# astra-vision/PaSCo

Hardware: AMD Instinct MI355X
Metric: scenes/sec (256x256x32, ~10% occ) PaSCo MIMO-3 (higher is better)
Workload: dtype f32 (conv products as 3 x f16 split MFMA, fp32 accumulate)

## Files before the change

pasco_amd/build.py:

```python
from __future__ import annotations

import os
import subprocess
import sys
from concurrent.futures import ThreadPoolExecutor

CSRC = os.path.join(os.path.dirname(os.path.abspath(__file__)), "csrc")
LIB_PATH = os.path.join(CSRC, "libpascohip.so")
SOURCES = ["coords.hip", "conv.hip", "conv_f16x3.hip", "conv_dma.hip", "conv_lin.hip", "conv_wide.hip", "conv_grid.hip", "conv_win.hip", "conv_wop.hip", "rows.hip", "attn.hip", "input.hip", "panop.hip", "eval.hip", "frame.hip", "label.hip"]
HEADERS = ["ph_common.h", "conv_h2_common.h", os.path.join("..", "..", "include", "pasco_hip.h"),
           os.path.join("..", "..", "include", "pasco_eval.h"),
           os.path.join("..", "..", "include", "pasco_frame.h"),
           os.path.join("..", "..", "include", "pasco_label.h")]
HIPCC = os.environ.get("HIPCC", "/opt/rocm/bin/hipcc")
FLAGS = ["--offload-arch=gfx950", "-O3", "-std=c++17", "-fPIC", "-Wall", "-Wno-unused-function"]


def _stale(target: str, deps: list[str]) -> bool:
    if not os.path.exists(target):
        return True
    t = os.path.getmtime(target)
    return any(os.path.getmtime(d) > t for d in deps if os.path.exists(d))


DEV_LIB_PATH = os.path.join(CSRC, "libpascohip_dev.so")


def build_hip(force: bool = False, verbose: bool = True, dev: bool = False) -> str:
    srcs = [s for s in SOURCES if os.path.exists(os.path.join(CSRC, s))]
    hdrs = [os.path.join(CSRC, h) for h in HEADERS]
    objs = []
    jobs = []
    lib_path = DEV_LIB_PATH if dev else LIB_PATH
    for s in srcs:
        src = os.path.join(CSRC, s)
        obj = os.path.join(CSRC, s.replace(".hip", ".dev.o" if dev else ".o"))
        objs.append(obj)
        if force or _stale(obj, [src] + hdrs):
            jobs.append([HIPCC, *FLAGS, *(["-DPH_DEV"] if dev else []), "-c", src, "-o", obj])

    def run(cmd):
        if verbose:
            print("[build]", " ".join(cmd), flush=True)
        r = subprocess.run(cmd, capture_output=True, text=True)
        if r.returncode != 0:
            sys.stderr.write(r.stdout + r.stderr)
            raise RuntimeError("hipcc failed: " + " ".join(cmd))
        if verbose and r.stderr.strip():
            sys.stderr.write(r.stderr)

    if jobs:
        with ThreadPoolExecutor(max_workers=min(4, len(jobs))) as ex:
            list(ex.map(run, jobs))
    if force or jobs or _stale(lib_path, objs):
        run([HIPCC, "--offload-arch=gfx950", "-shared", "-fPIC", "-o", lib_path, *objs])
    return lib_path


if __name__ == "__main__":
    print(build_hip(force="--force" in sys.argv, dev="--dev" in sys.argv))
```

pasco_amd/csrc/coords.hip:

```cpp
#include <stdarg.h>

#include "ph_common.h"

static thread_local char g_err[512] = "";

void ph_set_error(const char *fmt, ...) {
  va_list ap;
  va_start(ap, fmt);
  vsnprintf(g_err, sizeof(g_err), fmt, ap);
  va_end(ap);
}

extern "C" int ph_abi_version(void) { return PH_ABI_VERSION; }
extern "C" int ph_conv_desc_size(void) { return (int)sizeof(ph_conv_desc); }
extern "C" const char *ph_last_error(void) { return g_err; }

constexpr int CP_THREADS = 256;
constexpr int CP_ROUNDS = 8;
constexpr int CP_TILE = CP_THREADS * CP_ROUNDS;

extern "C" int64_t ph_workspace_bytes(int64_t n) {
  if (n < 0) n = 0;
  int64_t nb = n / CP_TILE + 2;
  return 9 * n + (int64_t)PH_MAX_KVOL * nb * 4 + 4096;
}

template <class Pred>
__global__ void __launch_bounds__(CP_THREADS)
    k_compact_count(Pred pred, int64_t n, int32_t *__restrict__ block_counts) {
  const int seg = blockIdx.y;
  const int nb = gridDim.x;
  const int64_t base = (int64_t)blockIdx.x * CP_TILE;
  int cnt = 0;
#pragma unroll
  for (int r = 0; r < CP_ROUNDS; ++r) {
    int64_t i = base + r * CP_THREADS + threadIdx.x;
    bool p = (i < n) && pred(seg, i);
    cnt += __popcll(__ballot(p));
  }
  __shared__ int wcnt[CP_THREADS / PH_WAVE];
  const int wave = threadIdx.x >> 6, lane = threadIdx.x & 63;
  if (lane == 0) wcnt[wave] = cnt;
  __syncthreads();
  if (threadIdx.x == 0) block_counts[(int64_t)seg * nb + blockIdx.x] = wcnt[0] + wcnt[1] + wcnt[2] + wcnt[3];
}

__global__ void __launch_bounds__(256)
    k_compact_scan(int32_t *__restrict__ block_counts, int nb, int32_t *__restrict__ totals) {
  const int seg = blockIdx.x;
  int32_t *c = block_counts + (int64_t)seg * nb;
  __shared__ int wsum[4];
  const int lane = threadIdx.x & 63, wave = threadIdx.x >> 6;
  int carry = 0;
  for (int base = 0; base < nb; base += 256) {
    int i = base + threadIdx.x;
    int v = (i < nb) ? c[i] : 0;
    int x = v;
#pragma unroll
    for (int d = 1; d < 64; d <<= 1) {
      int y = __shfl_up(x, d);
      if (lane >= d) x += y;
    }
    if (lane == 63) wsum[wave] = x;
    __syncthreads();
    int woff = 0;
    for (int w = 0; w < wave; ++w) woff += wsum[w];
    int tot = wsum[0] + wsum[1] + wsum[2] + wsum[3];
    if (i < nb) c[i] = carry + woff + x - v;
    carry += tot;
    __syncthreads();
  }
  if (threadIdx.x == 0) totals[seg] = carry;
}

template <class Pred, class Emit>
__global__ void __launch_bounds__(CP_THREADS)
    k_compact_scatter(Pred pred, Emit emit, int64_t n, const int32_t *__restrict__ block_offsets) {
  const int seg = blockIdx.y;
  const int nb = gridDim.x;
  const int64_t base = (int64_t)blockIdx.x * CP_TILE;
  __shared__ int wcnt[CP_THREADS / PH_WAVE];
  const int wave = threadIdx.x >> 6, lane = threadIdx.x & 63;
  int running = block_offsets[(int64_t)seg * nb + blockIdx.x];
#pragma unroll 1
  for (int r = 0; r < CP_ROUNDS; ++r) {
    int64_t i = base + r * CP_THREADS + threadIdx.x;
    bool p = (i < n) && pred(seg, i);
    unsigned long long b = __ballot(p);
    int wtot = __popcll(b);
    int wpre = __popcll(b & ((1ull << lane) - 1ull));
    if (lane == 0) wcnt[wave] = wtot;
    __syncthreads();
    int woff = 0;
    for (int w = 0; w < wave; ++w) woff += wcnt[w];
    int tot = wcnt[0] + wcnt[1] + wcnt[2] + wcnt[3];
    if (i < n) emit(seg, i, p ? running + woff + wpre : -1);
    running += tot;
    __syncthreads();
  }
}

template <class Pred, class Emit>
static int compact_run(Pred pred, Emit emit, int64_t n, int segs, int32_t *totals, void *ws,
                       int64_t ws_bytes, hipStream_t st) {
  int64_t nb = (n + CP_TILE - 1) / CP_TILE;
  if (nb < 1) nb = 1;
  PH_REQUIRE(ws_bytes >= (int64_t)segs * nb * 4, "compaction workspace too small (%lld < %lld)",
             (long long)ws_bytes, (long long)(segs * nb * 4));
  int32_t *block_counts = (int32_t *)ws;
  dim3 grid((unsigned)nb, (unsigned)segs);
  hipLaunchKernelGGL(k_compact_count<Pred>, grid, dim3(CP_THREADS), 0, st, pred, n, block_counts);
  PH_LAUNCH_CHECK();
  hipLaunchKernelGGL(k_compact_scan, dim3(segs), dim3(256), 0, st, block_counts, (int)nb, totals);
  PH_LAUNCH_CHECK();
  hipLaunchKernelGGL((k_compact_scatter<Pred, Emit>), grid, dim3(CP_THREADS), 0, st, pred, emit, n,
                     block_counts);
  PH_LAUNCH_CHECK();
  return 0;
}

struct PredFlag {
  const uint8_t *flags;
  __device__ bool operator()(int, int64_t i) const { return flags[i] != 0; }
};
struct EmitRows {
  int32_t *keep_rows;
  int32_t *rank_of;
  __device__ void operator()(int, int64_t i, int rank) const {
    if (rank >= 0) keep_rows[rank] = (int32_t)i;
    if (rank_of) rank_of[i] = rank;
  }
};

int ph_compact_flags(const uint8_t *flags, int64_t n, int32_t *keep_rows, int32_t *rank_of,
                     int32_t *n_keep, void *ws, int64_t ws_bytes, hipStream_t st) {
  return compact_run(PredFlag{flags}, EmitRows{keep_rows, rank_of}, n, 1, n_keep, ws, ws_bytes, st);
}

extern "C" int ph_mask_compact(const uint8_t *mask, int64_t n, int32_t *keep_rows, int32_t *n_keep,
                               void *ws, int64_t ws_bytes, ph_stream_t stream) {
  PH_REQUIRE(n >= 0 && n < 0x7FFFFFFF, "mask_compact: bad n");
  if (n == 0) {
    PH_CHECK_HIP(hipMemsetAsync(n_keep, 0, 4, ph_stream(stream)));
    return 0;
  }
  return ph_compact_flags(mask, n, keep_rows, nullptr, n_keep, ws, ws_bytes, ph_stream(stream));
}

__global__ void __launch_bounds__(256)
    k_insert(const int4 *__restrict__ coords, int64_t n, unsigned long long *__restrict__ tkeys,
             int32_t *__restrict__ tvals, uint64_t mask, int32_t *__restrict__ row_slot, int32_t *__restrict__ status) {
  int64_t i = (int64_t)blockIdx.x * blockDim.x + threadIdx.x;
  if (i >= n) return;
  int4 c = coords[i];
  if (!ph_packable(c.x, c.y, c.z, c.w)) {
    if (status != nullptr) atomicOr(status, 2);
    if (row_slot) row_slot[i] = -1;
    return;
  }
  uint64_t key = ph_pack(c.x, c.y, c.z, c.w);
  uint64_t slot = ph_hash(key) & mask;
  for (;;) {
    unsigned long long prev = atomicCAS(&tkeys[slot], (unsigned long long)PH_EMPTY_KEY,
                                        (unsigned long long)key);
    if (prev == PH_EMPTY_KEY || prev == key) break;
    slot = (slot + 1) & mask;
  }
  atomicMin((unsigned int *)&tvals[slot], (unsigned int)i);
  if (row_slot) row_slot[i] = (int32_t)slot;
}

struct PredFirst {
  const int32_t *tvals;
  const int32_t *row_slot;
  __device__ bool operator()(int, int64_t i) const {
    const int32_t s = row_slot[i];
    return s >= 0 && tvals[s] == (int32_t)i;
  }
};

__global__ void __launch_bounds__(256)
    k_assign_rank(int64_t n, const int32_t *__restrict__ rank_of,
                  const int32_t *__restrict__ row_slot, int32_t *__restrict__ tvals) {
  int64_t i = (int64_t)blockIdx.x * blockDim.x + threadIdx.x;
  if (i >= n) return;
  int r = rank_of[i];
  if (r >= 0) tvals[row_slot[i]] = r;
}

__global__ void __launch_bounds__(256)
    k_row2uniq(int64_t n, const int32_t *__restrict__ row_slot, const int32_t *__restrict__ tvals,
               int32_t *__restrict__ row2uniq) {
  int64_t i = (int64_t)blockIdx.x * blockDim.x + threadIdx.x;
  if (i >= n) return;
  const int32_t s = row_slot[i];
  row2uniq[i] = s >= 0 ? tvals[s] : -1;
}

static inline unsigned nblk(int64_t n, int t) { return (unsigned)((n + t - 1) / t); }

extern "C" int ph_map_insert(const int32_t *coords, int64_t n, uint64_t *tkeys, int32_t *tvals,
                             int64_t cap, int32_t *row2uniq, int32_t *uniq_rows, int32_t *n_uniq,
                             void *ws, int64_t ws_bytes, int32_t *status, ph_stream_t stream) {
  hipStream_t st = ph_stream(stream);
  PH_REQUIRE(n >= 0 && n < 0x3FFFFFFF, "map_insert: bad n=%lld", (long long)n);
  PH_REQUIRE(ph_is_pow2(cap) && cap >= 2 * n && cap >= 2, "map_insert: cap=%lld must be pow2 >= 2n",
             (long long)cap);
  if ((const char *)tvals == (const char *)tkeys + (size_t)cap * 8) {
    PH_CHECK_HIP(hipMemsetAsync(tkeys, 0xFF, (size_t)cap * 12, st));
  } else {
    PH_CHECK_HIP(hipMemsetAsync(tkeys, 0xFF, (size_t)cap * 8, st));
    PH_CHECK_HIP(hipMemsetAsync(tvals, 0xFF, (size_t)cap * 4, st));
  }
  if (n == 0) {
    if (n_uniq) PH_CHECK_HIP(hipMemsetAsync(n_uniq, 0, 4, st));
    return 0;
  }
  const uint64_t mask = (uint64_t)cap - 1;
  if (uniq_rows == nullptr) {
    hipLaunchKernelGGL(k_insert, dim3(nblk(n, 256)), dim3(256), 0, st, (const int4 *)coords, n,
                       (unsigned long long *)tkeys, tvals, mask, (int32_t *)nullptr, status);
    PH_LAUNCH_CHECK();
    return 0;
  }
  PH_REQUIRE(row2uniq && n_uniq, "map_insert: row2uniq / n_uniq required with uniq_rows");
  PH_REQUIRE(ws_bytes >= ph_workspace_bytes(n), "map_insert: workspace too small");
  int32_t *row_slot = (int32_t *)ws;
  int32_t *rank_of = row_slot + n;
  char *rest = (char *)(rank_of + n);
  int64_t rest_bytes = ws_bytes - 8 * n;
  hipLaunchKernelGGL(k_insert, dim3(nblk(n, 256)), dim3(256), 0, st, (const int4 *)coords, n,
                     (unsigned long long *)tkeys, tvals, mask, row_slot, status);
  PH_LAUNCH_CHECK();
  int rc = compact_run(PredFirst{tvals, row_slot}, EmitRows{uniq_rows, rank_of}, n, 1, n_uniq, rest,
                       rest_bytes, st);
  if (rc) return rc;
  hipLaunchKernelGGL(k_assign_rank, dim3(nblk(n, 256)), dim3(256), 0, st, n, rank_of, row_slot, tvals);
  PH_LAUNCH_CHECK();
  hipLaunchKernelGGL(k_row2uniq, dim3(nblk(n, 256)), dim3(256), 0, st, n, row_slot, tvals, row2uniq);
  PH_LAUNCH_CHECK();
  return 0;
}

__global__ void __launch_bounds__(256)
    k_find(const int4 *__restrict__ q, int64_t n, const uint64_t *__restrict__ tkeys,
           const int32_t *__restrict__ tvals, uint64_t mask, int32_t *__restrict__ out) {
  int64_t i = (int64_t)blockIdx.x * blockDim.x + threadIdx.x;
  if (i >= n) return;
  int4 c = q[i];
  out[i] = ph_packable(c.x, c.y, c.z, c.w) ? ph_find(tkeys, tvals, mask, ph_pack(c.x, c.y, c.z, c.w)) : -1;
}

extern "C" int ph_map_find(const int32_t *query, int64_t n, const uint64_t *tkeys,
                           const int32_t *tvals, int64_t cap, int32_t *out_rows,
                           ph_stream_t stream) {
  PH_REQUIRE(ph_is_pow2(cap), "map_find: cap must be pow2");
  if (n == 0) return 0;
  hipLaunchKernelGGL(k_find, dim3(nblk(n, 256)), dim3(256), 0, ph_stream(stream),
                     (const int4 *)query, n, tkeys, tvals, (uint64_t)cap - 1, out_rows);
  PH_LAUNCH_CHECK();
  return 0;
}

__device__ __forceinline__ int floor_to(int v, int ts) {
  int q = v / ts;
  if ((v % ts) != 0 && ((v < 0) != (ts < 0))) --q;
  return q * ts;
}

__global__ void __launch_bounds__(256)
    k_coords_floor(const int4 *__restrict__ in, int64_t n, int ts, int4 *__restrict__ out) {
  int64_t i = (int64_t)blockIdx.x * blockDim.x + threadIdx.x;
  if (i >= n) return;
  int4 c = in[i];
  out[i] = make_int4(c.x, floor_to(c.y, ts), floor_to(c.z, ts), floor_to(c.w, ts));
}

extern "C" int ph_coords_floor(const int32_t *coords, int64_t n, int32_t ts, int32_t *out,
                               ph_stream_t stream) {
  PH_REQUIRE(ts > 0, "coords_floor: ts must be > 0");
  if (n == 0) return 0;
  hipLaunchKernelGGL(k_coords_floor, dim3(nblk(n, 256)), dim3(256), 0, ph_stream(stream),
                     (const int4 *)coords, n, ts, (int4 *)out);
  PH_LAUNCH_CHECK();
  return 0;
}

__global__ void __launch_bounds__(256)
    k_coords_expand(const int4 *__restrict__ in, int64_t n, int ts, int4 *__restrict__ out) {
  int64_t t = (int64_t)blockIdx.x * blockDim.x + threadIdx.x;
  if (t >= n * 8) return;
  int64_t i = t >> 3;
  int k = (int)(t & 7);
  int4 c = in[i];
  out[t] = make_int4(c.x, c.y + (k & 1) * ts, c.z + ((k >> 1) & 1) * ts, c.w + ((k >> 2) & 1) * ts);
}

extern "C" int ph_coords_expand(const int32_t *coords, int64_t n, int32_t ts_out, int32_t *out,
                                ph_stream_t stream) {
  PH_REQUIRE(ts_out > 0, "coords_expand: ts_out must be > 0");
  if (n == 0) return 0;
  hipLaunchKernelGGL(k_coords_expand, dim3(nblk(n * 8, 256)), dim3(256), 0, ph_stream(stream),
                     (const int4 *)coords, n, ts_out, (int4 *)out);
  PH_LAUNCH_CHECK();
  return 0;
}

struct NbrOffsets {
  int32_t d[PH_MAX_KVOL][3];
};

__global__ void __launch_bounds__(256)
    k_nbr_build(const int4 *__restrict__ out_coords, int64_t n_out,
                const uint64_t *__restrict__ tkeys, const int32_t *__restrict__ tvals,
                uint64_t mask, NbrOffsets off, int32_t *__restrict__ nbr) {
  const int k = blockIdx.y;
  int64_t o = (int64_t)blockIdx.x * blockDim.x + threadIdx.x;
  if (o >= n_out) return;
  int4 c = out_coords[o];
  const int x = c.y + off.d[k][0], y = c.z + off.d[k][1], z = c.w + off.d[k][2];
  nbr[(int64_t)k * n_out + o] = ph_packable(c.x, x, y, z) ? ph_find(tkeys, tvals, mask, ph_pack(c.x, x, y, z)) : -1;
}

extern "C" int ph_nbr_build(const int32_t *out_coords, int64_t n_out, const uint64_t *in_tkeys,
                            const int32_t *in_tvals, int64_t in_cap, const int32_t *h_offsets,
                            int32_t kvol, int32_t *nbr, ph_stream_t stream) {
  PH_REQUIRE(kvol >= 1 && kvol <= PH_MAX_KVOL, "nbr_build: kvol=%d out of range", kvol);
  PH_REQUIRE(ph_is_pow2(in_cap), "nbr_build: cap must be pow2");
  if (n_out == 0) return 0;
  NbrOffsets off;
  memset(&off, 0, sizeof(off));
  memcpy(off.d, h_offsets, sizeof(int32_t) * 3 * kvol);
  dim3 grid(nblk(n_out, 256), (unsigned)kvol);
  hipLaunchKernelGGL(k_nbr_build, grid, dim3(256), 0, ph_stream(stream), (const int4 *)out_coords,
                     n_out, in_tkeys, in_tvals, (uint64_t)in_cap - 1, off, nbr);
  PH_LAUNCH_CHECK();
  return 0;
}

__global__ void __launch_bounds__(256)
    k_nbr_build_same(const int4 *__restrict__ coords, int64_t n, const uint64_t *__restrict__ tkeys,
                     const int32_t *__restrict__ tvals, uint64_t mask, NbrOffsets off, int kvol, int32_t *__restrict__ nbr) {
  const int k = blockIdx.y;
  int64_t o = (int64_t)blockIdx.x * blockDim.x + threadIdx.x;
  if (o >= n) return;
  if (k == kvol / 2) {
    nbr[(int64_t)k * n + o] = (int32_t)o;
    return;
  }
  int4 c = coords[o];
  const int x = c.y + off.d[k][0], y = c.z + off.d[k][1], z = c.w + off.d[k][2];
  const int j = ph_packable(c.x, x, y, z) ? ph_find(tkeys, tvals, mask, ph_pack(c.x, x, y, z)) : -1;
  nbr[(int64_t)k * n + o] = j;
  if (j >= 0) nbr[(int64_t)(kvol - 1 - k) * n + j] = (int32_t)o;
}

extern "C" int ph_nbr_build_same(const int32_t *coords, int64_t n, const uint64_t *tkeys, const int32_t *tvals, int64_t cap,
                                 const int32_t *h_offsets, int32_t kvol, int32_t *nbr, ph_stream_t stream) {
  PH_REQUIRE(kvol >= 1 && kvol <= PH_MAX_KVOL && (kvol & 1), "nbr_build_same: odd kernel volume <= %d expected, got %d", PH_MAX_KVOL, kvol);
  PH_REQUIRE(ph_is_pow2(cap), "nbr_build_same: cap must be pow2");
  for (int k = 0; k < kvol; ++k)
    for (int a = 0; a < 3; ++a)
      PH_REQUIRE(h_offsets[3 * k + a] == -h_offsets[3 * (kvol - 1 - k) + a], "nbr_build_same: offsets are not symmetric");
  if (n == 0) return 0;
  hipStream_t st = ph_stream(stream);
  NbrOffsets off;
  memset(&off, 0, sizeof(off));
  memcpy(off.d, h_offsets, sizeof(int32_t) * 3 * kvol);
  const int half = kvol / 2;
  if (half > 0)
    PH_CHECK_HIP(hipMemsetAsync(nbr + (int64_t)(half + 1) * n, 0xFF, (size_t)half * (size_t)n * 4, st));
  dim3 grid(nblk(n, 256), (unsigned)(half + 1));
  hipLaunchKernelGGL(k_nbr_build_same, grid, dim3(256), 0, st, (const int4 *)coords, n, tkeys, tvals, (uint64_t)cap - 1, off,
                     kvol, nbr);
  PH_LAUNCH_CHECK();
  return 0;
}

struct PredNbr {
  const int32_t *nbr;
  int64_t n_out;
  __device__ bool operator()(int seg, int64_t i) const { return nbr[(int64_t)seg * n_out + i] >= 0; }
};
struct EmitPairs {
  const int32_t *nbr;
  int64_t n_out;
  int32_t *pairs_in;
  int32_t *pairs_out;
  __device__ void operator()(int seg, int64_t i, int rank) const {
    if (rank < 0) return;
    int64_t base = (int64_t)seg * n_out;
    pairs_in[base + rank] = nbr[base + i];
    pairs_out[base + rank] = (int32_t)i;
  }
};

extern "C" int ph_kmap_compact(const int32_t *nbr, int32_t kvol, int64_t n_out, int32_t *pairs_in,
                               int32_t *pairs_out, int32_t *counts, void *ws, int64_t ws_bytes,
                               ph_stream_t stream) {
  PH_REQUIRE(kvol >= 1 && kvol <= PH_MAX_KVOL, "kmap_compact: kvol=%d out of range", kvol);
  if (n_out == 0) {
    PH_CHECK_HIP(hipMemsetAsync(counts, 0, 4 * kvol, ph_stream(stream)));
    return 0;
  }
  return compact_run(PredNbr{nbr, n_out}, EmitPairs{nbr, n_out, pairs_in, pairs_out}, n_out, kvol,
                     counts, ws, ws_bytes, ph_stream(stream));
}


__global__ void __launch_bounds__(256)
    k_rowlist_pack(const int32_t *__restrict__ pairs_in, const int32_t *__restrict__ pairs_out, const int32_t *__restrict__ counts,
                   int kvol, int64_t n_out, int32_t *__restrict__ rl_in, int32_t *__restrict__ rl_out,
                   int32_t *__restrict__ tile_k, int64_t cap, int64_t tcap, int32_t *__restrict__ status) {
  __shared__ int64_t off[PH_MAX_KVOL + 1];
  if (threadIdx.x == 0) {
    int64_t o = 0, pairs = 0;
    for (int k = 0; k < kvol; ++k) {
      off[k] = o;
      o += ((int64_t)counts[k] + 127) / 128 * 128;
      pairs += counts[k];
    }
    off[kvol] = o;
    if (status != nullptr && blockIdx.x == 0 && pairs != n_out) atomicOr(status, 32);
  }
  __syncthreads();
  const int64_t stride = (int64_t)gridDim.x * blockDim.x;
  for (int64_t i = (int64_t)blockIdx.x * blockDim.x + threadIdx.x; i < cap; i += stride) {
    int k = 0;
    while (k < kvol && i >= off[k + 1]) ++k;
    int vi = -1, vo = -1;
    if (k < kvol) {
      const int64_t j = i - off[k];
      if (j < counts[k]) {
        vi = pairs_in[(int64_t)k * n_out + j];
        vo = pairs_out[(int64_t)k * n_out + j];
      }
    }
    rl_in[i] = vi;
    rl_out[i] = vo;
    if ((i & 127) == 0 && (i >> 7) < tcap) tile_k[i >> 7] = k < kvol ? k : -1;
  }
  for (int64_t t = cap / 128 + (int64_t)blockIdx.x * blockDim.x + threadIdx.x; t < tcap; t += stride) tile_k[t] = -1;
}

extern "C" int ph_rowlist_pack(const int32_t *pairs_in, const int32_t *pairs_out, const int32_t *counts, int32_t kvol,
                               int64_t n_out, int32_t *rl_in, int32_t *rl_out, int32_t *tile_k, int64_t cap, int64_t tcap,
                               int32_t *status, ph_stream_t stream) {
  PH_REQUIRE(kvol >= 1 && kvol <= PH_MAX_KVOL, "rowlist_pack: kvol=%d out of range", kvol);
  PH_REQUIRE(cap % 128 == 0 && cap >= n_out + (int64_t)kvol * 127 - (kvol * 127) % 128 && tcap * 128 >= cap,
             "rowlist_pack: list capacity %lld too small for %lld rows and %d offsets", (long long)cap, (long long)n_out, kvol);
  if (cap == 0) return 0;
  int64_t blocks = (cap + 255) / 256;
  if (blocks > 4096) blocks = 4096;
  hipLaunchKernelGGL(k_rowlist_pack, dim3((unsigned)blocks), dim3(256), 0, ph_stream(stream), pairs_in, pairs_out, counts, kvol,
                     n_out, rl_in, rl_out, tile_k, cap, tcap, status);
  PH_LAUNCH_CHECK();
  return 0;
}
```

pasco_amd/csrc/rows.hip:

```cpp
#include "ph_common.h"

static inline unsigned nblk(int64_t n, int t) { return (unsigned)((n + t - 1) / t); }

template <typename T>
__global__ void __launch_bounds__(256)
    k_gather_rows(const T *__restrict__ src, int c, const int32_t *__restrict__ rows, int64_t n_out,
                  T *__restrict__ dst) {
  int64_t t = (int64_t)blockIdx.x * blockDim.x + threadIdx.x;
  if (t >= n_out * c) return;
  int64_t j = t / c;
  int ch = (int)(t - j * c);
  int r = rows[j];
  T v;
  memset(&v, 0, sizeof(T));
  if (r >= 0) v = src[(int64_t)r * c + ch];
  dst[t] = v;
}

extern "C" int ph_gather_rows(const void *src, int32_t c, const int32_t *rows, int64_t n_out,
                              void *dst, ph_stream_t stream) {
  PH_REQUIRE(c > 0, "gather_rows: c must be > 0");
  if (n_out == 0) return 0;
  hipStream_t st = ph_stream(stream);
  if (c % 4 == 0 && (((uintptr_t)src | (uintptr_t)dst) & 15) == 0) {
    int c4 = c / 4;
    hipLaunchKernelGGL(k_gather_rows<float4>, dim3(nblk(n_out * c4, 256)), dim3(256), 0, st,
                       (const float4 *)src, c4, rows, n_out, (float4 *)dst);
  } else {
    hipLaunchKernelGGL(k_gather_rows<float>, dim3(nblk(n_out * c, 256)), dim3(256), 0, st,
                       (const float *)src, c, rows, n_out, (float *)dst);
  }
  PH_LAUNCH_CHECK();
  return 0;
}

__global__ void __launch_bounds__(256)
    k_scatter_add_rows(const float *__restrict__ src, int c, const int32_t *__restrict__ rows,
                       int64_t n_src, float *__restrict__ dst) {
  int64_t t = (int64_t)blockIdx.x * blockDim.x + threadIdx.x;
  if (t >= n_src * c) return;
  int64_t i = t / c;
  int ch = (int)(t - i * c);
  int r = rows[i];
  if (r >= 0) dst[(int64_t)r * c + ch] += src[t];
}

extern "C" int ph_scatter_add_rows(const float *src, int32_t c, const int32_t *rows, int64_t n_src,
                                   float *dst, ph_stream_t stream) {
  PH_REQUIRE(c > 0, "scatter_add_rows: c must be > 0");
  if (n_src == 0) return 0;
  hipLaunchKernelGGL(k_scatter_add_rows, dim3(nblk(n_src * c, 256)), dim3(256), 0,
                     ph_stream(stream), src, c, rows, n_src, dst);
  PH_LAUNCH_CHECK();
  return 0;
}

struct KeepSrcs {
  const void *p[8];
};
__global__ void __launch_bounds__(256)
    k_keep_mask(KeepSrcs srcs, int n_src, int kind, const int4 *__restrict__ coords, int64_t n, const int32_t *__restrict__ lo,
                const int32_t *__restrict__ hi, uint8_t *__restrict__ out, int32_t *__restrict__ any) {
  const int64_t r = (int64_t)blockIdx.x * blockDim.x + threadIdx.x;
  bool k = n_src == 0;
  if (r < n) {
    for (int i = 0; i < n_src; ++i)
      k = k || (kind == 1 ? reinterpret_cast<const int32_t *>(srcs.p[i])[r] >= 0 : reinterpret_cast<const uint8_t *>(srcs.p[i])[r] != 0);
  }
  if (any != nullptr && __ballot(k) != 0ull && (threadIdx.x & 63) == 0) {
    if (__hip_atomic_load(any, __ATOMIC_RELAXED, __HIP_MEMORY_SCOPE_AGENT) == 0) atomicOr(any, 1);
  }
  if (r >= n) return;
  bool inside = true;
  if (lo != nullptr) {
    const int4 c = coords[r];
    inside = c.y >= lo[0] && c.z >= lo[1] && c.w >= lo[2] && c.y <= hi[0] && c.z <= hi[1] && c.w <= hi[2];
  }
  out[r] = (k && inside) ? 1 : 0;
}
__global__ void __launch_bounds__(256)
    k_keep_fallback(const int4 *__restrict__ coords, int64_t n, int64_t fallback, const int32_t *__restrict__ lo,
                    const int32_t *__restrict__ hi, uint8_t *__restrict__ out, const int32_t *__restrict__ any) {
  if (*any != 0) return;
  const int64_t r = (int64_t)blockIdx.x * blockDim.x + threadIdx.x;
  if (r >= n || r >= fallback) return;
  bool inside = true;
  if (lo != nullptr) {
    const int4 c = coords[r];
    inside = c.y >= lo[0] && c.z >= lo[1] && c.w >= lo[2] && c.y <= hi[0] && c.z <= hi[1] && c.w <= hi[2];
  }
  out[r] = inside ? 1 : 0;
}

extern "C" int ph_keep_mask(const void *const *srcs, int32_t n_src, int32_t kind, const int32_t *coords, int64_t n,
                            const int32_t *lo, const int32_t *hi, int64_t fallback_rows, uint8_t *out, int32_t *any_word,
                            ph_stream_t stream) {
  PH_REQUIRE(n_src >= 0 && n_src <= 8 && (kind == 0 || kind == 1) && n >= 0 && fallback_rows >= 0, "keep_mask: bad arguments");
  PH_REQUIRE((lo == nullptr) == (hi == nullptr) && (lo == nullptr || coords != nullptr), "keep_mask: bounds need lo, hi and coords");
  PH_REQUIRE(fallback_rows == 0 || any_word != nullptr, "keep_mask: the fallback needs the scratch word");
  if (n == 0) return 0;
  KeepSrcs ks;
  for (int i = 0; i < 8; ++i) ks.p[i] = i < n_src ? srcs[i] : nullptr;
  hipStream_t st = ph_stream(stream);
  int32_t *any = fallback_rows > 0 ? any_word : nullptr;
  if (any) PH_CHECK_HIP(hipMemsetAsync(any, 0, sizeof(int32_t), st));
  hipLaunchKernelGGL(k_keep_mask, dim3(nblk(n, 256)), dim3(256), 0, st, ks, n_src, kind, (const int4 *)coords, n, lo, hi, out, any);
  PH_LAUNCH_CHECK();
  if (any) {
    const int64_t m = n < fallback_rows ? n : fallback_rows;
    hipLaunchKernelGGL(k_keep_fallback, dim3(nblk(m, 256)), dim3(256), 0, st, (const int4 *)coords, n, fallback_rows, lo, hi, out,
                       any);
    PH_LAUNCH_CHECK();
  }
  return 0;
}

__global__ void __launch_bounds__(256)
    k_maxpool(const float *__restrict__ in, int c, const int32_t *__restrict__ nbr, int kvol,
              int64_t n_out, float *__restrict__ out) {
  int64_t t = (int64_t)blockIdx.x * blockDim.x + threadIdx.x;
  if (t >= n_out * c) return;
  int64_t o = t / c;
  int ch = (int)(t - o * c);
  float m = 0.f;
  bool any = false;
  for (int k = 0; k < kvol; ++k) {
    int r = nbr[(int64_t)k * n_out + o];
    if (r >= 0) {
      float v = in[(int64_t)r * c + ch];
      m = any ? fmaxf(m, v) : v;
      any = true;
    }
  }
  out[t] = m;
}

extern "C" int ph_maxpool_fwd(const float *in, int32_t c, const int32_t *nbr, int32_t kvol,
                              int64_t n_out, float *out, ph_stream_t stream) {
  PH_REQUIRE(c > 0 && kvol >= 1 && kvol <= PH_MAX_KVOL, "maxpool_fwd: bad shape");
  if (n_out == 0) return 0;
  hipLaunchKernelGGL(k_maxpool, dim3(nblk(n_out * c, 256)), dim3(256), 0, ph_stream(stream), in, c,
                     nbr, kvol, n_out, out);
  PH_LAUNCH_CHECK();
  return 0;
}

struct Dims4 {
  int b, x, y, z;
};

__device__ __forceinline__ int floor_div(int v, int ts) {
  int q = v / ts;
  if ((v % ts) != 0 && ((v < 0) != (ts < 0))) --q;
  return q;
}

__global__ void __launch_bounds__(256)
    k_to_dense(const float *__restrict__ feats, const int4 *__restrict__ coords, int64_t n, int c,
               int mx, int my, int mz, int ts, Dims4 d, float *__restrict__ dense) {
  int64_t t = (int64_t)blockIdx.x * blockDim.x + threadIdx.x;
  if (t >= n * c) return;
  int64_t i = t / c;
  int ch = (int)(t - i * c);
  int4 p = coords[i];
  int x = floor_div(p.y - mx, ts), y = floor_div(p.z - my, ts), z = floor_div(p.w - mz, ts);
  if (x < 0) x += d.x;
  if (y < 0) y += d.y;
  if (z < 0) z += d.z;
  if (p.x < 0 || p.x >= d.b || x < 0 || x >= d.x || y < 0 || y >= d.y || z < 0 || z >= d.z) return;
  int64_t site = ((int64_t)x * d.y + y) * d.z + z;
  dense[((int64_t)p.x * c + ch) * ((int64_t)d.x * d.y * d.z) + site] = feats[t];
}

extern "C" int ph_to_dense(const float *feats, const int32_t *coords, int64_t n, int32_t c,
                           const int32_t *h_min3, int32_t ts, const int32_t *h_dims4, float *dense,
                           ph_stream_t stream) {
  PH_REQUIRE(c > 0 && ts > 0, "to_dense: bad c/ts");
  if (n == 0) return 0;
  Dims4 d{h_dims4[0], h_dims4[1], h_dims4[2], h_dims4[3]};
  hipLaunchKernelGGL(k_to_dense, dim3(nblk(n * c, 256)), dim3(256), 0, ph_stream(stream), feats,
                     (const int4 *)coords, n, c, h_min3[0], h_min3[1], h_min3[2], ts, d, dense);
  PH_LAUNCH_CHECK();
  return 0;
}

__global__ void __launch_bounds__(256)
    k_site_flags(const float *__restrict__ dense, int c, int64_t nsite_per_b, int64_t nsites,
                 uint8_t *__restrict__ flags) {
  int64_t s = (int64_t)blockIdx.x * blockDim.x + threadIdx.x;
  if (s >= nsites) return;
  int64_t b = s / nsite_per_b;
  int64_t site = s - b * nsite_per_b;
  const float *p = dense + b * c * nsite_per_b + site;
  bool any = false;
  for (int ch = 0; ch < c; ++ch) any |= (p[(int64_t)ch * nsite_per_b] != 0.f);
  flags[s] = any ? 1 : 0;
}

__global__ void __launch_bounds__(256)
    k_sites_to_coords(const int32_t *__restrict__ keep_rows, const int32_t *__restrict__ n_rows,
                      Dims4 d, int4 *__restrict__ out_coords) {
  int64_t j = (int64_t)blockIdx.x * blockDim.x + threadIdx.x;
  if (j >= *n_rows) return;
  int64_t s = keep_rows[j];
  int z = (int)(s % d.z);
  s /= d.z;
  int y = (int)(s % d.y);
  s /= d.y;
  int x = (int)(s % d.x);
  s /= d.x;
  out_coords[j] = make_int4((int)s, x, y, z);
}

extern "C" int ph_to_sparse_coords(const float *dense, int32_t c, const int32_t *h_dims4,
                                   int32_t *out_coords, int32_t *n_rows, void *ws,
                                   int64_t ws_bytes, ph_stream_t stream) {
  Dims4 d{h_dims4[0], h_dims4[1], h_dims4[2], h_dims4[3]};
  int64_t per_b = (int64_t)d.x * d.y * d.z;
  int64_t nsites = per_b * d.b;
  PH_REQUIRE(c > 0 && nsites < 0x7FFFFF00, "to_sparse_coords: bad shape");
  hipStream_t st = ph_stream(stream);
  if (nsites == 0) {
    PH_CHECK_HIP(hipMemsetAsync(n_rows, 0, 4, st));
    return 0;
  }
  PH_REQUIRE(ws_bytes >= ph_workspace_bytes(nsites), "to_sparse_coords: workspace too small");
  uint8_t *flags = (uint8_t *)ws;
  int64_t fpad = (nsites + 15) & ~(int64_t)15;
  int32_t *keep_rows = (int32_t *)(flags + fpad);
  char *rest = (char *)(keep_rows + nsites);
  int64_t rest_bytes = ws_bytes - fpad - 4 * nsites;
  hipLaunchKernelGGL(k_site_flags, dim3(nblk(nsites, 256)), dim3(256), 0, st, dense, c, per_b, nsites,
                     flags);
  PH_LAUNCH_CHECK();
  int rc = ph_compact_flags(flags, nsites, keep_rows, nullptr, n_rows, rest, rest_bytes, st);
  if (rc) return rc;
  hipLaunchKernelGGL(k_sites_to_coords, dim3(nblk(nsites, 256)), dim3(256), 0, st, keep_rows, n_rows, d,
                     (int4 *)out_coords);
  PH_LAUNCH_CHECK();
  return 0;
}

__global__ void __launch_bounds__(256)
    k_dense_gather(const float *__restrict__ dense, int c, Dims4 d, const int4 *__restrict__ sc,
                   int64_t n, float *__restrict__ feats) {
  int64_t t = (int64_t)blockIdx.x * blockDim.x + threadIdx.x;
  if (t >= n * c) return;
  int64_t i = t / c;
  int ch = (int)(t - i * c);
  int4 p = sc[i];
  float v = 0.f;
  if (p.x >= 0 && p.x < d.b && p.y >= 0 && p.y < d.x && p.z >= 0 && p.z < d.y && p.w >= 0 && p.w < d.z) {
    int64_t per_b = (int64_t)d.x * d.y * d.z;
    int64_t site = ((int64_t)p.y * d.y + p.z) * d.z + p.w;
    v = dense[((int64_t)p.x * c + ch) * per_b + site];
  }
  feats[t] = v;
}

extern "C" int ph_dense_gather(const float *dense, int32_t c, const int32_t *h_dims4,
                               const int32_t *site_coords, int64_t n, float *feats,
                               ph_stream_t stream) {
  PH_REQUIRE(c > 0, "dense_gather: bad c");
  if (n == 0) return 0;
  Dims4 d{h_dims4[0], h_dims4[1], h_dims4[2], h_dims4[3]};
  hipLaunchKernelGGL(k_dense_gather, dim3(nblk(n * c, 256)), dim3(256), 0, ph_stream(stream), dense, c,
                     d, (const int4 *)site_coords, n, feats);
  PH_LAUNCH_CHECK();
  return 0;
}

__global__ void __launch_bounds__(256) k_sine_pe(const int32_t *__restrict__ coords, int64_t n, int cstride, int coff, int f,
                                                  const float *__restrict__ dim_t, float scale,
                                                  const float *__restrict__ table, int tab_lo, int tab_n,
                                                  float *__restrict__ out) {
  const int64_t t = (int64_t)blockIdx.x * blockDim.x + threadIdx.x;
  const int w = 3 * f;
  if (t >= n * w) return;
  const int64_t row = t / w;
  const int col = (int)(t - row * w);
  const int axis = col / f;
  const int j = col - axis * f;
  const int half = f >> 1;
  const int ci = coords[row * cstride + coff + axis];
  const unsigned ti = (unsigned)(ci - tab_lo);
  float v;
  if (table != nullptr && ti < (unsigned)tab_n) {
    v = table[(int64_t)ti * f + j];
  } else {
    float c = (float)ci;
    c = c / (c + 1e-6f) * scale;
    if (j < half) v = sinf(c / dim_t[2 * j]);
    else v = cosf(c / dim_t[2 * (j - half) + 1]);
  }
  out[t] = v;
}

extern "C" int ph_sine_pe(const int32_t *coords, int64_t n, int32_t cstride, int32_t coff, int32_t f,
                          const float *dim_t, float scale, const float *table, int32_t tab_lo, int32_t tab_n,
                          float *out, ph_stream_t stream) {
  PH_REQUIRE(n >= 0 && f > 0 && f % 2 == 0 && cstride >= 3 && coff >= 0 && coff + 3 <= cstride, "sine_pe: bad shape");
  PH_REQUIRE(table == nullptr || tab_n > 0, "sine_pe: empty table");
  if (n == 0) return 0;
  PH_REQUIRE(coords && dim_t && out, "sine_pe: null buffer");
  hipLaunchKernelGGL(k_sine_pe, dim3(nblk(n * 3 * f, 256)), dim3(256), 0, ph_stream(stream), coords, n, cstride, coff, f,
                     dim_t, scale, table, tab_lo, tab_n, out);
  PH_LAUNCH_CHECK();
  return 0;
}


template <int C, bool VEC>
__global__ void __launch_bounds__(256) k_sem_ensemble(ph_sem_ens_desc d) {
  const int64_t s = (int64_t)blockIdx.x * blockDim.x + threadIdx.x;
  if (s >= d.n_sites) return;
  float mean[C];
#pragma unroll
  for (int ch = 0; ch < C; ++ch) mean[ch] = 0.f;
  for (int i = 0; i < d.m; ++i) {
    float p[C];
    const int r = d.rows[i][s];
    if (r >= 0) {
      const float *x = d.logits[i] + (int64_t)r * C;
      if (VEC) {
#pragma unroll
        for (int q = 0; q < C / 4; ++q) {
          const float4 v = reinterpret_cast<const float4 *>(x)[q];
          p[4 * q] = v.x; p[4 * q + 1] = v.y; p[4 * q + 2] = v.z; p[4 * q + 3] = v.w;
        }
      } else {
#pragma unroll
        for (int ch = 0; ch < C; ++ch) p[ch] = x[ch];
      }
      float mx = p[0];
#pragma unroll
      for (int ch = 1; ch < C; ++ch) mx = fmaxf(mx, p[ch]);
      float sum = 0.f;
#pragma unroll
      for (int ch = 0; ch < C; ++ch) {
        p[ch] = expf(p[ch] - mx);
        sum += p[ch];
      }
#pragma unroll
      for (int ch = 0; ch < C; ++ch) p[ch] = p[ch] / sum;
    } else {
#pragma unroll
      for (int ch = 0; ch < C; ++ch) p[ch] = ch == 0 ? 1.f : 0.f;
    }
    float best = p[0];
#pragma unroll
    for (int ch = 0; ch < C; ++ch) {
      mean[ch] += p[ch];
      best = fmaxf(best, p[ch]);
    }
    float *o = d.out[i] + s * C;
    if (VEC) {
#pragma unroll
      for (int q = 0; q < C / 4; ++q) reinterpret_cast<float4 *>(o)[q] = make_float4(p[4 * q], p[4 * q + 1], p[4 * q + 2], p[4 * q + 3]);
    } else {
#pragma unroll
      for (int ch = 0; ch < C; ++ch) o[ch] = p[ch];
    }
    if (d.conf[i]) d.conf[i][s] = best;
  }
  const float inv_m = (float)d.m;
  float best = 0.f;
#pragma unroll
  for (int ch = 0; ch < C; ++ch) {
    mean[ch] = mean[ch] / inv_m;
    best = ch == 0 ? mean[ch] : fmaxf(best, mean[ch]);
  }
  float *o = d.out[d.m] + s * C;
  if (VEC) {
#pragma unroll
    for (int q = 0; q < C / 4; ++q) reinterpret_cast<float4 *>(o)[q] = make_float4(mean[4 * q], mean[4 * q + 1], mean[4 * q + 2], mean[4 * q + 3]);
  } else {
#pragma unroll
    for (int ch = 0; ch < C; ++ch) o[ch] = mean[ch];
  }
  if (d.conf[d.m]) d.conf[d.m][s] = best;
}

extern "C" int ph_sem_ensemble(const ph_sem_ens_desc *desc, ph_stream_t stream) {
  PH_REQUIRE(desc != nullptr && desc->m >= 1 && desc->m <= 8, "sem_ensemble: 1 <= m <= 8");
  PH_REQUIRE(desc->c == 20 || desc->c == 19, "sem_ensemble: serves 20 (SemanticKITTI) or 19 (SSCBench-KITTI360) classes, got %d", desc->c);
  if (desc->n_sites == 0) return 0;
  for (int i = 0; i < desc->m; ++i) PH_REQUIRE(desc->logits[i] && desc->rows[i] && desc->out[i], "sem_ensemble: null buffer");
  PH_REQUIRE(desc->out[desc->m] != nullptr, "sem_ensemble: null mean buffer");
  hipStream_t st = ph_stream(stream);
  const dim3 grid((unsigned)((desc->n_sites + 255) / 256));
  bool al = true;
  for (int i = 0; i <= desc->m; ++i) al = al && (((uintptr_t)desc->out[i]) & 15) == 0;
  for (int i = 0; i < desc->m; ++i) al = al && (((uintptr_t)desc->logits[i]) & 15) == 0;
  if (desc->c == 20 && al)
    hipLaunchKernelGGL((k_sem_ensemble<20, true>), grid, dim3(256), 0, st, *desc);
  else if (desc->c == 20)
    hipLaunchKernelGGL((k_sem_ensemble<20, false>), grid, dim3(256), 0, st, *desc);
  else
    hipLaunchKernelGGL((k_sem_ensemble<19, false>), grid, dim3(256), 0, st, *desc);
  PH_LAUNCH_CHECK();
  return 0;
}


__global__ void __launch_bounds__(256)
    k_ens_resample(const float *__restrict__ logits, int q, const int32_t *__restrict__ rows, const int32_t *__restrict__ sel,
                   int64_t u, float *__restrict__ out, uint8_t *__restrict__ flag) {
  const int lane = threadIdx.x & 63;
  const int64_t nwaves = (int64_t)gridDim.x * 4;
  for (int64_t s = (int64_t)blockIdx.x * 4 + (threadIdx.x >> 6); s < u; s += nwaves) {
    const int r = rows[sel[s]];
    float v0 = 0.f, v1 = 0.f;
    if (r >= 0) {
      const float *x = logits + (int64_t)r * q;
      if (lane < q) v0 = 1.f / (1.f + expf(-x[lane]));
      if (lane + 64 < q) v1 = 1.f / (1.f + expf(-x[lane + 64]));
    }
    float *o = out + s * q;
    if (lane < q) o[lane] = v0;
    if (lane + 64 < q) o[lane + 64] = v1;
    const unsigned long long any = __ballot(v0 != 0.f || v1 != 0.f);
    if (lane == 0) flag[s] = any != 0ull ? 1 : 0;
  }
}

__global__ void __launch_bounds__(256)
    k_ens_merge(float *__restrict__ anchor, const float *__restrict__ m, const int32_t *__restrict__ perm, int64_t u, int q,
                float fi) {
#pragma clang fp contract(off)
  const int lane = threadIdx.x & 63;
  const int p0 = lane < q ? perm[lane] : 0, p1 = lane + 64 < q ? perm[lane + 64] : 0;
  const int64_t nwaves = (int64_t)gridDim.x * 4;
  const float den = fi + 1.f;
  for (int64_t s = (int64_t)blockIdx.x * 4 + (threadIdx.x >> 6); s < u; s += nwaves) {
    float *a = anchor + s * q;
    const float *b = m + s * q;
    if (lane < q) {
      const float t = a[lane] * fi;
      a[lane] = (t + b[p0]) / den;
    }
    if (lane + 64 < q) {
      const float t = a[lane + 64] * fi;
      a[lane + 64] = (t + b[p1]) / den;
    }
  }
}

__global__ void __launch_bounds__(256)
    k_ens_finish(const float *__restrict__ anchor, int q, const int32_t *__restrict__ keep, int qk, const float *__restrict__ sem,
                 int c, const int32_t *__restrict__ sel, int64_t u, float *__restrict__ out, uint8_t *__restrict__ flag) {
  const int lane = threadIdx.x & 63;
  const int k0 = lane < qk ? keep[lane] : 0, k1 = lane + 64 < qk ? keep[lane + 64] : 0;
  const int64_t nwaves = (int64_t)gridDim.x * 4;
  for (int64_t s = (int64_t)blockIdx.x * 4 + (threadIdx.x >> 6); s < u; s += nwaves) {
    const float *sr = sem + (int64_t)sel[s] * c;
    const float p0 = sr[0];
    const bool larger = lane >= 1 && lane < c && sr[lane] > p0;
    const float nz = __ballot(larger) != 0ull ? 1.f : 0.f;
    const float *a = anchor + s * q;
    float v0 = 0.f, v1 = 0.f;
    if (lane < qk) v0 = a[k0] * nz;
    if (lane + 64 < qk) v1 = a[k1] * nz;
    float *o = out + s * qk;
    if (lane < qk) o[lane] = v0;
    if (lane + 64 < qk) o[lane + 64] = v1;
    const unsigned long long any = __ballot(v0 != 0.f || v1 != 0.f);
    if (lane == 0) flag[s] = any != 0ull ? 1 : 0;
  }
}

static unsigned ens_grid(int64_t u) {
  int64_t g = (u + 3) / 4;
  if (g > 16384) g = 16384;
  return (unsigned)(g < 1 ? 1 : g);
}

extern "C" int ph_ens_resample(const float *logits, int64_t n, int32_t q, const int32_t *rows, const int32_t *sel, int64_t u,
                               float *out, uint8_t *flag, ph_stream_t stream) {
  PH_REQUIRE(q >= 1 && q <= 128 && n >= 0 && u >= 0, "ens_resample: bad shape");
  if (u == 0) return 0;
  PH_REQUIRE(logits && rows && sel && out && flag, "ens_resample: null buffer");
  hipLaunchKernelGGL(k_ens_resample, dim3(ens_grid(u)), dim3(256), 0, ph_stream(stream), logits, q, rows, sel, u, out, flag);
  PH_LAUNCH_CHECK();
  return 0;
}

extern "C" int ph_ens_merge(float *anchor, const float *m, const int32_t *perm, int64_t u, int32_t q, int32_t i,
                            ph_stream_t stream) {
  PH_REQUIRE(q >= 1 && q <= 128 && u >= 0 && i >= 1, "ens_merge: bad shape");
  if (u == 0) return 0;
  PH_REQUIRE(anchor && m && perm, "ens_merge: null buffer");
  hipLaunchKernelGGL(k_ens_merge, dim3(ens_grid(u)), dim3(256), 0, ph_stream(stream), anchor, m, perm, u, q, (float)i);
  PH_LAUNCH_CHECK();
  return 0;
}

extern "C" int ph_ens_finish(const float *anchor, int64_t u, int32_t q, const int32_t *keep, int32_t qk, const float *sem,
                             int32_t c, const int32_t *sel, float *out, uint8_t *flag, ph_stream_t stream) {
  PH_REQUIRE(q >= 1 && q <= 128 && qk >= 0 && qk <= q && c >= 1 && c <= 64 && u >= 0, "ens_finish: bad shape");
  if (u == 0) return 0;
  PH_REQUIRE(anchor && sem && sel && flag && (qk == 0 || (keep && out)), "ens_finish: null buffer");
  hipLaunchKernelGGL(k_ens_finish, dim3(ens_grid(u)), dim3(256), 0, ph_stream(stream), anchor, q, keep, qk, sem, c, sel, u, out,
                     flag);
  PH_LAUNCH_CHECK();
  return 0;
}

__global__ void __launch_bounds__(256)
    k_project_canonical(const float *__restrict__ T, int X, int Y, int Z, double res, float mb0, float mb1, float mb2,
                        int4 *__restrict__ out) {
#pragma clang fp contract(off)
  const int64_t i = (int64_t)blockIdx.x * blockDim.x + threadIdx.x;
  const int64_t n = (int64_t)X * Y * Z;
  if (i >= n) return;
  const int z = (int)(i % Z), y = (int)((i / Z) % Y), x = (int)(i / ((int64_t)Y * Z));
  const float mb[3] = {mb0, mb1, mb2};
  const int c[3] = {x, y, z};
  float p[3];
#pragma unroll
  for (int a = 0; a < 3; ++a) {
    const double m = (double)c[a] * res;
    const double h = m + res / 2;
    p[a] = (float)(h + (double)mb[a]);
  }
  const float resf = (float)res, halff = (float)(res / 2);
  int q[3];
#pragma unroll
  for (int r = 0; r < 3; ++r) {
    const float t0 = T[r * 4 + 0] * p[0];
    const float t1 = T[r * 4 + 1] * p[1];
    float v = t0 + t1;
    const float t2 = T[r * 4 + 2] * p[2];
    v = v + t2;
    v = v + T[r * 4 + 3];
    v = v - mb[r];
    v = v - halff;
    v = v / resf;
    q[r] = (int)rintf(v);
  }
  out[i] = make_int4(0, q[0], q[1], q[2]);
}

extern "C" int ph_project_canonical(const float *T, int32_t X, int32_t Y, int32_t Z, double resolution, const float *h_min_bound,
                                    int32_t *out_coords, ph_stream_t stream) {
  PH_REQUIRE(X >= 1 && Y >= 1 && Z >= 1 && resolution > 0, "project_canonical: bad grid");
  PH_REQUIRE(T && h_min_bound && out_coords, "project_canonical: null buffer");
  const int64_t n = (int64_t)X * Y * Z;
  hipLaunchKernelGGL(k_project_canonical, dim3((unsigned)((n + 255) / 256)), dim3(256), 0, ph_stream(stream), T, X, Y, Z,
                     resolution, h_min_bound[0], h_min_bound[1], h_min_bound[2], (int4 *)out_coords);
  PH_LAUNCH_CHECK();
  return 0;
}
```

pasco_amd/graph/decoder.py:

```python
from __future__ import annotations

import os
from collections import defaultdict
from typing import Dict, List, Optional

import torch
import torch.nn as nn

from .. import me as ME
from . import fused
from .blocks import BasicGenerativeDeconvolutionBlock, ResidualBlock, SpatialDropout, run_sequential
from .fused import ACT_NONE, ACT_RELU


def _corner(v, coords: torch.Tensor) -> torch.Tensor:
    if torch.is_tensor(v):
        stream = torch.cuda.current_stream(coords.device).cuda_stream if coords.device.type == "cuda" else 0
        key = (coords.dtype, coords.device, stream, v._version)
        cache = getattr(v, "_ph_corner", None)
        if cache is not None and key in cache:
            return cache[key]
        out = v.to(device=coords.device, dtype=coords.dtype).reshape(1, 3)
        try:
            if cache is None or len(cache) > 8:
                cache = {}
                v._ph_corner = cache
            cache[key] = out
        except AttributeError:
            pass
        return out
    return torch.as_tensor(v, device=coords.device).to(coords.dtype).reshape(1, 3)


def inside_bounds(coords: torch.Tensor, lo, hi) -> torch.Tensor:
    lo, hi = _corner(lo, coords), _corner(hi, coords)
    xyz = coords[:, 1:]
    return ((xyz >= lo) & (xyz <= hi)).all(dim=1)


def box_mask(mgr, coords: torch.Tensor, lo, hi) -> torch.Tensor:
    if fused.fusion() and coords.dtype == torch.int32 and coords.dim() == 2 and coords.shape[1] == 4:
        try:
            be = mgr.backend()
        except Exception:
            be = None
        if be is not None and be.has("keep_mask") and os.environ.get("PASCO_KEEP_FUSED", "1") != "0":
            lo_t, hi_t = _corner(lo, coords).reshape(3).contiguous(), _corner(hi, coords).reshape(3).contiguous()
            return be.keep_mask([], coords.contiguous(), lo_t, hi_t)
    return inside_bounds(coords, lo, hi)


_FIRST_ROWS = {}


def _first_rows(n: int, device, k: int = 1000) -> torch.Tensor:
    stream = torch.cuda.current_stream(device).cuda_stream if torch.device(device).type == "cuda" else 0
    key = (n, str(device), k, stream)
    hit = _FIRST_ROWS.get(key)
    if hit is None:
        if len(_FIRST_ROWS) > 64:
            _FIRST_ROWS.clear()
        hit = torch.arange(n, device=device) < k
        _FIRST_ROWS[key] = hit
    return hit


def batch_sparse_tensor(tensors: List[ME.SparseTensor], n_max: Optional[int] = None):
    n_max = max([t.F.shape[0] for t in tensors] + ([n_max] if n_max is not None else []))
    f0, c0 = tensors[0].F, tensors[0].C
    bf = f0.new_empty((len(tensors), n_max, f0.shape[1]))
    bc = c0.new_empty((len(tensors), n_max, c0.shape[1]))
    for i, t in enumerate(tensors):
        n = t.F.shape[0]
        bf[i, :n] = t.F
        bc[i, :n] = t.C
        if n < n_max:
            bf[i, n:].zero_()
            bc[i, n:].zero_()
    return bf, bc


class DecoderBlock(nn.Module):
    def __init__(self, in_channels, out_channels, n_heads, compl_head_dim, heavy_decoder=True, dropout=0.0):
        super().__init__()
        self.upsample = BasicGenerativeDeconvolutionBlock(in_channels, out_channels, ks=2, stride=2)
        self.resize = nn.Sequential(
            ME.MinkowskiBatchNorm(out_channels + 3),
            ME.MinkowskiConvolution(out_channels + 3, out_channels, kernel_size=1, bias=True, dimension=3),
        )
        n_res = 7 if heavy_decoder else 3
        layers = [ResidualBlock(out_channels, out_channels) for _ in range(n_res)]
        if heavy_decoder:
            layers.append(SpatialDropout(p=dropout))
        self.process = nn.Sequential(*layers)
        self.n_heads = n_heads
        self.completion_heads = nn.ModuleDict({
            str(i): nn.Sequential(ME.MinkowskiConvolution(out_channels, compl_head_dim, kernel_size=1, bias=True,
                                                          dimension=3))
            for i in range(n_heads)})

    def forward(self, x: ME.SparseTensor, shortcut: ME.SparseTensor, global_min, global_max):
        mgr = x.coordinate_manager
        up = self.upsample.net[0]
        out_key = mgr.expand_pruned(x.coordinate_map_key, up.stride, lambda kids: box_mask(mgr, kids, global_min, global_max))
        nbr = mgr.kernel_map(x.coordinate_map_key, out_key, up.kernel_size, up.dilation, transposed=True)
        y_in = None
        if self._resize_applies(x, out_key):
            ukey, _, b2o = mgr.union(out_key, shortcut.coordinate_map_key)
            n_un, n_dec = mgr.size(ukey), mgr.size(out_key)
            buf = torch.empty((n_un, self.resize[1].out_channels), dtype=torch.float32, device=x.F.device)
            dec = self._resize_absorbed(x, out_key, nbr, out=buf[:n_dec])
            if dec is not None and dec.F.data_ptr() == buf.data_ptr():
                if n_un > n_dec:
                    buf[n_dec:].zero_()
                mgr.backend().scatter_add_rows(shortcut.F.contiguous(), b2o.contiguous(), buf)
                y_in = ME.SparseTensor(buf, coordinate_map_key=ukey, coordinate_manager=mgr)
        else:
            dec = None
        if y_in is None and dec is None:
            dec = self.upsample(x, out_key=out_key, nbr=nbr)
            ts = dec.tensor_stride[0]
            feats = torch.cat([dec.F, dec.C[:, 1:].float() / ts], dim=1)
            dec = ME.SparseTensor(feats, coordinate_map_key=out_key, coordinate_manager=mgr)
            dec = fused.conv(dec, self.resize[1], pro_bn=self.resize[0], pro_act=ACT_NONE)
        if y_in is None:
            y_in = dec + shortcut
        y = run_sequential(self.process, y_in)
        logits = [fused.conv(y, self.completion_heads[str(i)][0]) for i in range(self.n_heads)]
        return y, logits


    RESIZE_LO, RESIZE_ROWS = -1024, 5120

    def _resize_applies(self, x, out_key) -> bool:
        mgr = x.coordinate_manager
        conv = self.resize[1]
        c_in, c_out = conv.in_channels - 3, conv.out_channels
        be = mgr.backend()
        return bool(fused.fusion() and fused.conv_precision() == "f16x3" and fused._PRESPLIT and fused._kernel_device(x.F.device)
                    and mgr.size(out_key) >= fused.MIN_ROWS_LINEAR and c_in % 32 == 0 and be.split_supported(c_in, c_out)
                    and os.environ.get("PASCO_RESIZE_ABSORB", "1") != "0")

    def _resize_absorbed(self, x, out_key, nbr, out=None):
        mgr = x.coordinate_manager
        n_out = mgr.size(out_key)
        conv, bn = self.resize[1], self.resize[0]
        c_out = conv.out_channels
        c_in = conv.in_channels - 3
        be = mgr.backend()
        if not self._resize_applies(x, out_key):
            return None
        dec = self.upsample(x, out_key=out_key, nbr=nbr, emit_next=(None, ACT_NONE), split_only=True)
        if not isinstance(dec, fused.SplitRows):
            return self._resize_plain(dec, out_key)
        ts = out_key.tensor_stride[0]
        w = conv.kernel
        ver = (w._version, w.data_ptr(), conv.bias._version if conv.bias is not None else -1, ts) + tuple(
            (t._version, t.data_ptr()) for t in (bn.bn.running_mean, bn.bn.running_var, bn.bn.weight, bn.bn.bias) if t is not None)
        hit = self.__dict__.get("_ph_resize")
        if hit is None or hit[0] != ver:
            with torch.no_grad():
                s_, b_ = fused.fold_bn(bn)
                s64, b64, w64 = s_.double(), b_.double(), w.detach().reshape(c_in + 3, c_out).double()
                wf = (s64[:c_in, None] * w64[:c_in]).t().contiguous().float()
                bias = b64[:c_in] @ w64[:c_in]
                if conv.bias is not None:
                    bias = bias + conv.bias.detach().reshape(-1).double()
                idx = torch.arange(self.RESIZE_ROWS, device=w.device, dtype=torch.float64) + self.RESIZE_LO
                tab = torch.stack([((idx / ts) * s64[c_in + a] + b64[c_in + a])[:, None] * w64[c_in + a][None, :]
                                   for a in range(3)]).float().contiguous()
            hit = (ver, wf, bias.float().contiguous(), tab)
            fused.publish(tab)
            self.__dict__["_ph_resize"] = hit
        _, wf, bias, tab = hit
        coords = mgr.get_coordinates(out_key)
        out = fused.linear_rows(None, wf, bias, self, "resize", in_split=dec.split,
                                axis=(tab, coords.contiguous(), self.RESIZE_LO), out=out)
        return ME.SparseTensor(out, coordinate_map_key=out_key, coordinate_manager=mgr)

    def _resize_plain(self, dec, out_key):
        mgr = dec.coordinate_manager
        ts = dec.tensor_stride[0]
        feats = torch.cat([dec.F, dec.C[:, 1:].float() / ts], dim=1)
        dec = ME.SparseTensor(feats, coordinate_map_key=out_key, coordinate_manager=mgr)
        return fused.conv(dec, self.resize[1], pro_bn=self.resize[0], pro_act=ACT_NONE)


class DecoderGenerativeSepConvV2(nn.Module):
    def __init__(self, f, n_classes, transformer_predictor, n_infers, heavy_decoder=True, dropouts=(0.0, 0.0, 0.0)):
        super().__init__()
        dec_ch = list(f[::-1])
        self.n_infers = n_infers
        self.n_classes = n_classes
        self.transformer_predictor = transformer_predictor
        self.dec_blocks = nn.ModuleList()
        self.voxel_feats = nn.ModuleDict()
        for i in range(len(dec_ch) - 1):
            scale = 2 ** (len(dec_ch) - 2 - i)
            self.dec_blocks.append(DecoderBlock(dec_ch[i], dec_ch[i + 1], n_heads=n_infers, compl_head_dim=n_classes,
                                                heavy_decoder=heavy_decoder, dropout=dropouts[i]))
            c = dec_ch[i + 1]
            for j in range(n_infers):
                self.voxel_feats[f"scale{scale}_infer{j}"] = nn.Sequential(
                    ME.MinkowskiConvolution(c, c, kernel_size=3, bias=False, dimension=3),
                    ME.MinkowskiBatchNorm(c),
                    ME.MinkowskiReLU(),
                    ME.MinkowskiConvolution(c, c, kernel_size=3, bias=True, dimension=3),
                )
        self.pruning = ME.MinkowskiPruning()

    @staticmethod
    def _occupied(logits: ME.SparseTensor) -> torch.Tensor:
        return logits.F.argmax(dim=-1) != 0

    @staticmethod
    def _keep_sources(keep_override, scale, i, x, logits):
        if keep_override is not None:
            if hasattr(keep_override, "member_rows"):
                return keep_override.member_rows(scale, i, x.C)
            return keep_override.member(scale, i, x.C)
        return DecoderGenerativeSepConvV2._occupied(logits)

    @staticmethod
    def _fused_keep(x):
        if not fused.fusion() or x.C.dtype != torch.int32 or len(x.C.shape) != 2 or x.C.shape[1] != 4:
            return None
        try:
            be = x.coordinate_manager.backend()
        except Exception:
            return None
        return be if be.has("keep_mask") and os.environ.get("PASCO_KEEP_FUSED", "1") != "0" else None

    def _keep_completion(self, x, scale, sem_logits, keep_override):
        srcs = [self._keep_sources(keep_override, scale, i, x, sem_logits[i] if sem_logits is not None else None)
                for i in range(self.n_infers)]
        be = self._fused_keep(x)
        if be is not None and len(srcs) <= 8 and len({s.dtype for s in srcs}) == 1:
            return be.keep_mask([s.contiguous() for s in srcs])
        keeps = [s >= 0 if s.dtype == torch.int32 else s for s in srcs]
        keep = keeps[0]
        for k in keeps[1:]:
            keep = keep | k
        return keep

    def predict_panop(self, xs, sem_logits_at_scales, min_Cs, max_Cs, keep_override=None, subnets=None):
        xs_infers = defaultdict(list)
        sem_logits_pruneds = []

        def keep_mask(i, scale, x):
            logits = sem_logits_at_scales[scale][i]
            src = self._keep_sources(keep_override, scale, i, x, logits)
            be = self._fused_keep(x)
            if be is not None:
                lo, hi = _corner(min_Cs[i], x.C).reshape(3), _corner(max_Cs[i], x.C).reshape(3)
                return be.keep_mask([src.contiguous()], x.C.contiguous(), lo.contiguous(), hi.contiguous(), fallback_rows=1000)
            keep = src >= 0 if src.dtype == torch.int32 else src
            first = _first_rows(keep.shape[0], keep.device)
            keep = torch.where(keep.any(), keep, first)
            return keep & inside_bounds(x.C, min_Cs[i], max_Cs[i])

        pad_to = {s: None for s in xs}
        if subnets is not None:
            for scale, x in xs.items():
                pad_to[scale] = max(int(keep_mask(i, scale, x).sum()) for i in range(self.n_infers))
        todo = [(i, scale, x, keep_mask(i, scale, x)) for i in (range(self.n_infers) if subnets is None else subnets)
                for scale, x in xs.items()]
        mgrs = {id(x.coordinate_manager) for _, _, x, _ in todo}
        if len(mgrs) == 1 and todo:
            mgr = todo[0][2].coordinate_manager
            pruned = mgr.prune_batch([(x.coordinate_map_key, keep) for _, _, x, keep in todo])
        else:
            pruned = [x.coordinate_manager.prune(x.coordinate_map_key, keep) for _, _, x, keep in todo]
        infer_ids = list(range(self.n_infers) if subnets is None else subnets)
        n_rows = {(i, scale): x.coordinate_manager.size(out_key) for (i, scale, x, keep), (out_key, rows) in zip(todo, pruned)}
        batch_f, batch_c = {}, {}
        for scale, x in xs.items():
            n_max = max([n_rows[(i, scale)] for i in infer_ids] + ([pad_to[scale]] if pad_to[scale] is not None else []))
            batch_f[scale] = x.F.new_empty((len(infer_ids), n_max, x.F.shape[1]))
            batch_c[scale] = x.C.new_zeros((len(infer_ids), n_max, x.C.shape[1]))
        sem_F = None
        if 1 in xs:
            l0 = sem_logits_at_scales[1][infer_ids[0]].F
            sem_F = l0.new_empty((len(infer_ids), batch_f[1].shape[1], l0.shape[1]))
        for (i, scale, x, keep), (out_key, rows) in zip(todo, pruned):
            mgr = x.coordinate_manager
            be = mgr.backend()
            if scale == 1:
                logits = sem_logits_at_scales[scale][i]
                slot1, n1_ = infer_ids.index(i), n_rows[(i, scale)]
                dst = sem_F[slot1, :n1_]
                be.gather_rows(logits.F.contiguous(), rows, out=dst)
                if n1_ < sem_F.shape[1]:
                    sem_F[slot1, n1_:].zero_()
                sem_logits_pruneds.append(ME.SparseTensor(dst, coordinate_map_key=out_key, coordinate_manager=mgr))
            xi = fused.gathered_split(x, rows, out_key)
            if xi is None:
                xi = ME.SparseTensor(be.gather_rows(x.F.contiguous(), rows), coordinate_map_key=out_key, coordinate_manager=mgr)
            vf = self.voxel_feats[f"scale{scale}_infer{i}"]
            h = fused.conv(xi, vf[0], epi_bn=vf[1], epi_act=ACT_RELU, emit_next=(None, ACT_NONE), split_only=True)
            slot = infer_ids.index(i)
            n = n_rows[(i, scale)]
            y = fused.conv(h, vf[3], out=batch_f[scale][slot, :n])
            batch_c[scale][slot, :n] = y.C
            if n < batch_f[scale].shape[1]:
                batch_f[scale][slot, n:].zero_()
            xs_infers[scale].append(y)
        batched = {s: (batch_f[s], batch_c[s]) for s in xs_infers}
        batched["_meta"] = {"lens": {"fine": [int(t.F.shape[0]) for t in xs_infers[1]],
                                     "level": {s: [int(t.F.shape[0]) for t in v] for s, v in xs_infers.items()}}}
        if sem_F is None:
            sem_F, sem_C = batch_sparse_tensor(sem_logits_pruneds, pad_to[1])
        else:
            sem_C = batch_c[1]
        keep_pad = (sem_F != 0).any(-1) | (sem_C != 0).any(-1)
        panop = self.transformer_predictor(batched, (sem_F, sem_C), min_Cs, max_Cs, keep_pad, subnets=subnets,
                                           sem_tensors=sem_logits_pruneds)
        return panop, sem_logits_pruneds

    def forward(self, x, features, global_min_coords, global_max_coords, min_Cs, max_Cs,
                is_predict_panop=True, keep_override=None, subnets=None):
        assert not self.training, "inference only"
        skips = features[::-1]
        sem_logits_at_scales: Dict[int, list] = {}
        xs: Dict[int, ME.SparseTensor] = {}
        for i, block in enumerate(self.dec_blocks):
            scale = 2 ** (len(self.dec_blocks) - 1 - i)
            x, sem_logits = block(x, skips[i], global_min_coords, global_max_coords)
            keep = self._keep_completion(x, scale, sem_logits, keep_override)
            mgr = x.coordinate_manager
            out_key, rows = mgr.prune(x.coordinate_map_key, keep)
            be = mgr.backend()
            x = ME.SparseTensor(be.gather_rows(x.F, rows), coordinate_map_key=out_key, coordinate_manager=mgr)
            sem_logits = [ME.SparseTensor(be.gather_rows(l.F, rows), coordinate_map_key=out_key,
                                          coordinate_manager=mgr) for l in sem_logits]
            xs[scale] = x
            sem_logits_at_scales[scale] = sem_logits
        ret = {"sem_logits_at_scales": sem_logits_at_scales}
        if is_predict_panop:
            panop, pruned = self.predict_panop(xs, sem_logits_at_scales, min_Cs, max_Cs, keep_override, subnets)
            ret["panop_predictions"] = panop
            ret["sem_logits_pruneds"] = pruned
        return ret
```

pasco_amd/graph/fused.py:

```python
from __future__ import annotations

import contextlib
import os
import threading
from typing import Optional, Tuple

import torch
import torch.nn as nn

from ..me import SparseTensor
from ..me.backend import ACT_LEAKY, ACT_NONE, ACT_RELU
from ..me.modules import MinkowskiBatchNorm, _ConvBase

_CONV_PRECISION = "f16x3"
_PRESPLIT = True
_FUSION = True
MIN_ROWS_LINEAR = 16384
MIN_ROWS_WINDOWS = 16384
_WINDOWS_WIDE = os.environ.get("PASCO_CONV_WIN", "1") == "2"


def _kernel_device(device) -> bool:
    if device.type == "cuda":
        return True
    from ..me import backend
    cb = backend._checker_backend
    return cb is not None and cb.checker_split


def set_conv_precision(mode: str) -> None:
    global _CONV_PRECISION, _PRESPLIT
    assert mode in ("f32", "f16x3", "f16x3-inline")
    _PRESPLIT = mode != "f16x3-inline"
    _CONV_PRECISION = "f32" if mode == "f32" else "f16x3"


_TLS = threading.local()


def conv_precision() -> str:
    return getattr(_TLS, "precision", None) or _CONV_PRECISION


@contextlib.contextmanager
def precision_override(mode: str):
    assert mode in ("f32", "f16x3")
    prev = getattr(_TLS, "precision", None)
    _TLS.precision = mode
    try:
        yield
    finally:
        _TLS.precision = prev


def optimistic() -> bool:
    return bool(getattr(_TLS, "optimistic", False))


def optimistic_word(device):
    if not optimistic():
        return None
    from ..me.backend import backend_for
    try:
        return backend_for(device).optimistic_word(device)
    except RuntimeError:
        return None


@contextlib.contextmanager
def optimistic_override(on: bool):
    prev = getattr(_TLS, "optimistic", None)
    _TLS.optimistic = bool(on)
    try:
        yield
    finally:
        _TLS.optimistic = prev


def set_fusion(on: bool) -> None:
    global _FUSION
    _FUSION = bool(on)


def fusion() -> bool:
    return _FUSION


def _act_rows(F: torch.Tensor, act: int, slope: float) -> torch.Tensor:
    if act == ACT_RELU:
        return torch.relu(F)
    if act == ACT_LEAKY:
        return torch.nn.functional.leaky_relu(F, slope)
    return F


def _module_act(y: SparseTensor, act: int, slope: float) -> SparseTensor:
    if act == ACT_NONE:
        return y
    from ..me.modules import MinkowskiLeakyReLU, MinkowskiReLU
    mod = MinkowskiReLU() if act == ACT_RELU else MinkowskiLeakyReLU(slope)
    return mod(y)


def _conv_unfused(x, mod, pro_bn, pro_act, epi_bn, epi_act, epi2_bn, residual, res_act, slope, out_key, nbr):
    mgr = x.coordinate_manager
    same = lambda t, feats: SparseTensor(feats, coordinate_map_key=t.coordinate_map_key, coordinate_manager=mgr)
    bn_of = lambda bn, t: bn(t) if isinstance(bn, MinkowskiBatchNorm) else same(t, bn(t.F))
    y = x
    if pro_bn is not None:
        y = bn_of(pro_bn, y)
    y = _module_act(y, pro_act, slope)
    if out_key is None:
        y = mod(y)
    else:
        raw, pending = y.take_prologue()
        y = SparseTensor(mod.conv_rows(mgr.backend(), raw, nbr, mgr.size(out_key), mgr=mgr, prologue=pending),
                         coordinate_map_key=out_key, coordinate_manager=mgr)
    if epi_bn is not None:
        y = bn_of(epi_bn, y)
    y = _module_act(y, epi_act, slope)
    if epi2_bn is not None:
        y = bn_of(epi2_bn, y)
    if residual is not None:
        y = same(y, y.F + residual)
    return _module_act(y, res_act, slope)


def publish(t):
    dev = t.device if torch.is_tensor(t) else t
    if dev.type == "cuda" and not torch.cuda.is_current_stream_capturing():
        torch.cuda.current_stream(dev).synchronize()
    return t


def _split_of(w, be):
    return be.split_weight_rows(w) if _PRESPLIT else be.split_weight_f16(w)


def split_weight(mod, be):
    w = mod.kernel
    ver = (w._version, w.device, _PRESPLIT)
    hit = getattr(mod, "_ph_split", None)
    if hit is None or hit[0] != ver:
        hit = (ver, _split_of(w, be))
        publish(w.device)
        object.__setattr__(mod, "_ph_split", hit)
    return hit[1]


def split_input(x: SparseTensor, be, ps, pb, pro_act, slope):
    F = x.F if x.F.is_contiguous() else x.F.contiguous()
    key = _split_key(F, ps, pb, pro_act, slope)
    cache = x.__dict__.setdefault("_ph_in_split", {})
    hit = cache.get(key)
    if hit is None:
        hit = be.split_rows(F, pro_scale=ps, pro_shift=pb, pro_act=pro_act, slope=slope)
        cache[key] = hit
    return hit


def gathered_split(x: SparseTensor, rows: torch.Tensor, out_key):
    mgr = x.coordinate_manager
    be = mgr.backend()
    c = x.F.shape[1]
    if not (_FUSION and _PRESPLIT and conv_precision() == "f16x3" and be.split_supported(c, c) and x.F.shape[0] > 0):
        return None
    op = split_input(x, be, None, None, ACT_NONE, 0.01)
    n, cpad = op.shape[0], op.shape[1] * 32
    got = be.gather_rows(op.view(torch.float32).view(n, cpad), rows)
    return SplitRows(got.view(torch.float16).view(got.shape[0], cpad // 32, 2, 32), c, out_key, mgr)


def split_rows_2d(x2d: torch.Tensor):
    if not (_FUSION and _kernel_device(x2d.device) and conv_precision() == "f16x3" and _PRESPLIT and x2d.shape[1] % 8 == 0):
        return None
    from ..me.backend import backend_for
    return backend_for(x2d.device).split_rows(x2d.contiguous())


def linear_rows(x2d: Optional[torch.Tensor], weight: torch.Tensor, bias, cache_owner, cache_key: str,
                min_rows: Optional[int] = None, in_split=None, residual: Optional[torch.Tensor] = None,
                emit: bool = False, want_out: bool = True, axis=None, out: Optional[torch.Tensor] = None):
    cout, cin = weight.shape
    n = x2d.shape[0] if x2d is not None else in_split.shape[0]
    dev = x2d.device if x2d is not None else in_split.device
    be = None
    min_rows = MIN_ROWS_LINEAR if min_rows is None else min_rows
    if _FUSION and _kernel_device(dev) and n >= min_rows and conv_precision() == "f16x3":
        from ..me.backend import backend_for
        be = backend_for(dev)
        if not be.split_supported(cin, cout):
            be = None
    if be is None:
        assert x2d is not None, "linear_rows: a pre-split operand needs the split path"
        y = torch.nn.functional.linear(x2d, weight, bias)
        y = y if residual is None else y + residual
        if axis is not None:
            y = y + axis_rows(axis)
        if out is not None:
            out.copy_(y)
            y = out
        return (y, None) if emit else y
    ver = (weight._version, weight.device, weight.data_ptr(), _PRESPLIT)
    hit = cache_owner.__dict__.get("_ph_lin_" + cache_key)
    if hit is None or hit[0] != ver:
        wt = weight.detach().t().contiguous()
        hit = (ver, wt, _split_of(wt, be), bias.detach().contiguous() if bias is not None else None)
        publish(wt)
        cache_owner.__dict__["_ph_lin_" + cache_key] = hit
    _, wt, split, b = hit
    do_emit = emit and _PRESPLIT and cout % 32 == 0
    out = be.conv_fwd(None if (x2d is None) else x2d.contiguous(), wt, None, n,
                      xshape=(n, cin) if x2d is None else None, bias=b, split=split,
                      in_split=in_split if _PRESPLIT else None,
                      residual=None if residual is None else residual.contiguous(),
                      emit_split=(None, None, ACT_NONE) if do_emit else None, want_out=want_out or not do_emit,
                      axis=axis, out=out)
    if not emit:
        return out
    return out if do_emit else (out, None)


def axis_rows(axis) -> torch.Tensor:
    tab, coords, lo = axis
    idx = (coords[:, 1:4].long() - lo).clamp(0, tab.shape[1] - 1)
    return tab[0][idx[:, 0]] + tab[1][idx[:, 1]] + tab[2][idx[:, 2]]


def linear_bn_act(x2d: Optional[torch.Tensor], lin: nn.Linear, *, pro_bn=None, epi_bn=None, epi_act: int = ACT_NONE,
                  min_rows: Optional[int] = None, in_split=None, emit: bool = False, emit_into: Optional[torch.Tensor] = None,
                  out: Optional[torch.Tensor] = None):
    cin, cout = lin.in_features, lin.out_features
    n = x2d.shape[0] if x2d is not None else in_split.shape[0]
    dev = x2d.device if x2d is not None else in_split.device
    min_rows = MIN_ROWS_LINEAR if min_rows is None else min_rows
    if not (_FUSION and _kernel_device(dev) and n >= min_rows):
        assert x2d is not None
        y = x2d if pro_bn is None else pro_bn(x2d)
        y = lin(y)
        y = y if epi_bn is None else epi_bn(y)
        y = torch.relu(y) if epi_act == ACT_RELU else y
        return (y, None) if emit else y
    from ..me.backend import backend_for
    be = backend_for(dev)
    ps = pb = es = eb = None
    if pro_bn is not None:
        ps, pb = fold_bn(pro_bn)
    if epi_bn is not None:
        es, eb = fold_bn(epi_bn)
    w = lin.weight
    ver = (w._version, w.device, w.data_ptr(), _PRESPLIT, conv_precision())
    hit = lin.__dict__.get("_ph_lin_w")
    if hit is None or hit[0] != ver:
        wt = w.detach().t().contiguous()
        split = _split_of(wt, be) if (conv_precision() == "f16x3" and be.split_supported(cin, cout)) else None
        hit = (ver, wt, split, lin.bias.detach().contiguous() if lin.bias is not None else None)
        publish(wt)
        lin.__dict__["_ph_lin_w"] = hit
    _, wt, split, b = hit
    do_emit = emit and split is not None and _PRESPLIT and cout % 32 == 0
    assert x2d is not None or (split is not None and _PRESPLIT), "a pre-split operand needs the split path"
    out = be.conv_fwd(None if x2d is None else x2d.contiguous(), wt, None, n, xshape=(n, cin) if x2d is None else None,
                      bias=b, pro_scale=ps, pro_shift=pb, epi_scale=es, epi_shift=eb, epi_act=epi_act, split=split,
                      in_split=in_split if (split is not None and _PRESPLIT) else None,
                      emit_split=(None, None, ACT_NONE) if do_emit else None, want_out=not do_emit,
                      in_split_has_prologue=True, out_split=emit_into if do_emit else None, out=None if do_emit else out)
    if not emit:
        return out
    return out if do_emit else (out, None)


def prepare_batched_weights(w: torch.Tensor):
    from ..me.backend import backend_for
    be = backend_for(w.device)
    B, Q, D = w.shape
    w = w.detach()
    e = 13 - torch.frexp(w.abs().amax())[1]
    e = e.to(torch.int32).clamp(-100, 100)
    up = ((e + 127) << 23).view(torch.float32)
    down = ((127 - e) << 23).view(torch.float32)
    w_split = be.split_rows((w * up).reshape(B * Q, D).contiguous(), exp2=0)
    unscale = (torch.ones(Q, device=w.device) * down).contiguous()
    return w_split, unscale


def batched_rows_matmul(x: Optional[torch.Tensor], w: Optional[torch.Tensor], x_split: torch.Tensor, shape=None,
                        prepared=None, bias=None, axis=None) -> torch.Tensor:
    from ..me.backend import backend_for
    dev = x_split.device
    be = backend_for(dev)
    B, P, D = x.shape if x is not None else shape
    w_split, unscale = prepared if prepared is not None else prepare_batched_weights(w)
    Q = unscale.numel()
    out = torch.empty((B, P, Q), dtype=torch.float32, device=dev)
    xs = x_split.reshape(B, P, -1)
    ws = w_split.reshape(B, Q, -1)
    for b in range(B):
        be.conv_fwd(None, None, None, P, xshape=(P, D), wshape=(1, D, Q), split=(ws[b], 1.0), in_split=xs[b],
                    epi_scale=unscale, out=out[b], epi2_shift=None if bias is None else bias[b],
                    axis=None if axis is None else (axis[0][b], axis[1][b], axis[2]))
    return out


def fold_bn(bn) -> Tuple[torch.Tensor, torch.Tensor]:
    m = bn.bn if isinstance(bn, MinkowskiBatchNorm) else bn
    assert isinstance(m, nn.modules.batchnorm._BatchNorm)
    assert not m.training, "fused graph serves inference (module.eval()) only"
    bufs, pars = m._buffers, m._parameters
    rm, rv, w, b = bufs["running_mean"], bufs["running_var"], pars.get("weight"), pars.get("bias")
    ver = (rm._version, rv._version, w._version if w is not None else -1, b._version if b is not None else -1, rm.device)
    hit = m.__dict__.get("_ph_folded")
    if hit is not None and hit[0] == ver:
        return hit[1], hit[2]
    with torch.no_grad():
        inv = torch.rsqrt(m.running_var.float() + m.eps)
        scale = inv * (m.weight.float() if m.weight is not None else 1.0)
        shift = (m.bias.float() if m.bias is not None else 0.0) - m.running_mean.float() * scale
        scale, shift = scale.contiguous(), shift.contiguous()
    publish(scale)
    m._ph_folded = (ver, scale, shift)
    return scale, shift


class SplitRows:

    def __init__(self, split: torch.Tensor, channels: int, coordinate_map_key, coordinate_manager):
        self.split = split
        self.channels = channels
        self.coordinate_map_key = coordinate_map_key
        self.coordinate_manager = coordinate_manager


def _split_key(F, ps, pb, pro_act, slope):
    return (F.data_ptr(), F._version, None if ps is None else ps.data_ptr(), None if pb is None else pb.data_ptr(),
            pro_act, float(slope) if pro_act == ACT_LEAKY else 0.0)


def conv(x: SparseTensor, mod: _ConvBase, *, pro_bn=None, pro_act: int = ACT_NONE, epi_bn=None,
         epi_act: int = ACT_NONE, epi2_bn=None, residual: Optional[torch.Tensor] = None,
         res_act: int = ACT_NONE, slope: float = 0.01, out_key=None, nbr=None, emit_next=None,
         split_only: bool = False, one_pair: bool = False, out: Optional[torch.Tensor] = None):
    mgr = x.coordinate_manager
    if not _FUSION:
        assert not isinstance(x, SplitRows)
        y = _conv_unfused(x, mod, pro_bn, pro_act, epi_bn, epi_act, epi2_bn, residual, res_act, slope, out_key, nbr)
        if out is not None:
            out.copy_(y.F)
            y = SparseTensor(out, coordinate_map_key=y.coordinate_map_key, coordinate_manager=mgr)
        return y
    if out_key is None:
        out_key, nbr = mod._maps(x)
    n_out = mgr.size(out_key)
    ps = pb = es = eb = e2s = e2b = None
    if pro_bn is not None:
        ps, pb = fold_bn(pro_bn)
    if epi_bn is not None:
        es, eb = fold_bn(epi_bn)
    if epi2_bn is not None:
        e2s, e2b = fold_bn(epi2_bn)
    bias = mod.bias.detach().reshape(-1) if mod.bias is not None else None
    be = mgr.backend()
    split = in_split = None
    x_rows = None
    if isinstance(x, SplitRows):
        assert pro_bn is None and pro_act == ACT_NONE, "a pre-split input already carries its prologue"
        split, in_split = split_weight(mod, be), x.split
        xshape = (in_split.shape[0], x.channels)
    else:
        x_rows = x.F if x.F.is_contiguous() else x.F.contiguous()
        xshape = None
        if conv_precision() == "f16x3" and be.split_supported(mod.in_channels, mod.out_channels):
            split = split_weight(mod, be)
            if _PRESPLIT and n_out > 0:
                in_split = split_input(x, be, ps, pb, pro_act, slope)
    emit = None
    if emit_next is not None and in_split is not None and mod.out_channels % 32 == 0:
        nbn, nact = emit_next
        ns, nb = fold_bn(nbn) if nbn is not None else (None, None)
        emit = (ns, nb, nact)
    only = split_only and emit is not None and n_out > 0
    win = None
    if in_split is not None and nbr is not None and nbr.shape[0] == 27 and n_out >= MIN_ROWS_WINDOWS and \
            be.device_type == "cuda" and (33 <= mod.out_channels <= 64 or _WINDOWS_WIDE):
        win = mgr.kernel_windows(nbr)
    rowlist = None
    if one_pair and in_split is not None and nbr is not None and nbr.shape[0] <= 8 and n_out >= MIN_ROWS_LINEAR and \
            be.device_type == "cuda" and os.environ.get("PASCO_CONV_RL", "1") != "0":
        rowlist = mgr.kernel_rowlist(nbr)
    if out is not None:
        assert not only and out.is_contiguous() and tuple(out.shape) == (n_out, mod.out_channels) and out.dtype == torch.float32
    out = be.conv_fwd(
        x_rows, mod.kernel.detach(), nbr, n_out, xshape=xshape, bias=bias,
        pro_scale=ps, pro_shift=pb, pro_act=pro_act, epi_scale=es, epi_shift=eb, epi_act=epi_act,
        epi2_scale=e2s, epi2_shift=e2b, residual=residual, res_act=res_act, slope=slope, split=split,
        in_split=in_split, emit_split=emit, want_out=not only, win=win, in_split_has_prologue=True, rowlist=rowlist,
        out=out if n_out > 0 else None)
    if emit is None:
        return SparseTensor(out, coordinate_map_key=out_key, coordinate_manager=mgr)
    out, out_split = out
    if only:
        assert emit[0] is None and emit[1] is None and emit[2] == ACT_NONE, "split_only serves a plain next operand"
        return SplitRows(out_split, mod.out_channels, out_key, mgr)
    y = SparseTensor(out, coordinate_map_key=out_key, coordinate_manager=mgr)
    y.__dict__.setdefault("_ph_in_split", {})[_split_key(y.F, emit[0], emit[1], emit[2], slope)] = out_split
    return y


__all__ = ["fold_bn", "conv", "set_conv_precision", "conv_precision", "precision_override", "optimistic", "optimistic_override", "set_fusion", "fusion", "linear_rows", "split_rows_2d", "gathered_split", "batched_rows_matmul", "prepare_batched_weights", "linear_bn_act", "ACT_NONE", "ACT_RELU", "ACT_LEAKY"]
```

pasco_amd/me/backend.py:

```python
from __future__ import annotations

import contextlib
import ctypes as C
import os
import threading
from typing import Dict, Optional

import torch

_HERE = os.path.dirname(os.path.abspath(__file__))
HIP_LIB_PATH = os.path.join(os.path.dirname(_HERE), "csrc", "libpascohip.so")

ACT_NONE, ACT_RELU, ACT_LEAKY = 0, 1, 2
ABI_VERSION = 5


class StatusError(RuntimeError):

    def __init__(self, bits: int, message: str):
        super().__init__(message)
        self.bits = bits


class F16RangeError(StatusError):
    """ONLY bit 0 was raised: an activation left the f16 range of the split-precision convolutions.  The result of the
    step is unusable, the exact-fp32 path (fused.set_conv_precision("f32")) serves the same graph."""
MAX_KVOL = 64
SPLIT_ACT_EXP2 = 5

_vp = C.c_void_p
_i64 = C.c_int64
_i32 = C.c_int32


class ConvDesc(C.Structure):

    _fields_ = [
        ("in_", _vp), ("weight", _vp), ("nbr", _vp), ("out", _vp),
        ("n_in", _i64), ("n_out", _i64),
        ("cin", _i32), ("cout", _i32), ("kvol", _i32), ("pro_act", _i32),
        ("pro_scale", _vp), ("pro_shift", _vp), ("bias", _vp),
        ("epi_scale", _vp), ("epi_shift", _vp),
        ("epi_act", _i32), ("epi_slope", C.c_float),
        ("residual", _vp), ("res_act", _i32), ("split_exp2", _i32),
        ("epi2_scale", _vp), ("epi2_shift", _vp),
        ("mma_mode", _i32), ("w_unscale", C.c_float), ("w_f16_hi", _vp), ("w_f16_lo", _vp),
        ("splitk_ws", _vp), ("splitk_ws_bytes", _i64), ("status", _vp),
        ("in_split", _vp), ("w_split", _vp),
        ("out_split", _vp), ("osp_scale", _vp), ("osp_shift", _vp), ("osp_act", _i32), ("route", _i32),
        ("win_rows", _vp), ("win_cnt", _vp), ("win_slots", _vp), ("win_stats", _vp),
        ("axis_table", _vp), ("axis_coords", _vp), ("axis_lo", _i32), ("axis_rows", _i32),
        ("rl_in", _vp), ("rl_out", _vp), ("rl_tile_k", _vp), ("rl_rows", _i64), ("rl_tiles", _i32),
        ("exact_if", _vp), ("w_frag", _vp),
        ("grid_dims", _i32 * 4), ("grid_kernel", _i32 * 3), ("reserved3", _i32),
    ]


class SemEnsDesc(C.Structure):

    _fields_ = [("m", _i32), ("c", _i32), ("n_sites", _i64), ("logits", _vp * 8), ("rows", _vp * 8),
                ("out", _vp * 9), ("conf", _vp * 9)]


_SIGNATURES = {
    "abi_version": [],
    "conv_desc_size": [],
    "last_error": [],
    "workspace_bytes": [_i64],
    "map_insert": [_vp, _i64, _vp, _vp, _i64, _vp, _vp, _vp, _vp, _i64, _vp, _vp],
    "map_find": [_vp, _i64, _vp, _vp, _i64, _vp, _vp],
    "coords_floor": [_vp, _i64, _i32, _vp, _vp],
    "coords_expand": [_vp, _i64, _i32, _vp, _vp],
    "nbr_build": [_vp, _i64, _vp, _vp, _i64, _vp, _i32, _vp, _vp],
    "nbr_build_same": [_vp, _i64, _vp, _vp, _i64, _vp, _i32, _vp, _vp],
    "kmap_compact": [_vp, _i32, _i64, _vp, _vp, _vp, _vp, _i64, _vp],
    "rowlist_pack": [_vp, _vp, _vp, _i32, _i64, _vp, _vp, _vp, _i64, _i64, _vp, _vp],
    "conv_fwd": [C.POINTER(ConvDesc), _vp],
    "conv_last_config": [_vp],
    "win_build": [_vp, _i32, _i64, _vp, _vp, _vp, _vp, _vp],
    "sem_ensemble": [C.POINTER(SemEnsDesc), _vp],
    "split_rows": [_vp, _i64, _i32, _vp, _vp, _i32, C.c_float, _i32, _vp, _vp, _vp],
    "maxpool_fwd": [_vp, _i32, _vp, _i32, _i64, _vp, _vp],
    "mask_compact": [_vp, _i64, _vp, _vp, _vp, _i64, _vp],
    "gather_rows": [_vp, _i32, _vp, _i64, _vp, _vp],
    "scatter_add_rows": [_vp, _i32, _vp, _i64, _vp, _vp],
    "to_dense": [_vp, _vp, _i64, _i32, _vp, _i32, _vp, _vp, _vp],
    "to_sparse_coords": [_vp, _i32, _vp, _vp, _vp, _vp, _i64, _vp],
    "dense_gather": [_vp, _i32, _vp, _vp, _i64, _vp, _vp],
    "sine_pe": [_vp, _i64, _i32, _i32, _i32, _vp, C.c_float, _vp, _i32, _i32, _vp, _vp],
    "attn_workspace_bytes": [_i64, _i32, _i32, _i32, _i32],
    "attn_mask_pack": [_vp, _i64, _i32, _i32, _i32, _vp, _vp, _vp],
    "bits_orpool": [_vp, _vp, _i32, _i64, _vp, _vp],
    "bits_or_reduce": [_vp, _i64, _i32, _vp, _vp],
    "attn_cross_fwd": [_vp, _vp, _vp, _vp, _vp, _vp, _i64, _i32, _i32, _i32, _i32, _vp, _i64, _vp],
    "bits_block_or": [_vp, _i64, _i64, _i32, _vp, _vp, _i64, _vp, _vp, _vp, _vp, _vp, _vp],
    "project_canonical": [_vp, _i32, _i32, _i32, C.c_double, _vp, _vp, _vp],
    "ens_resample": [_vp, _i64, _i32, _vp, _vp, _i64, _vp, _vp, _vp],
    "ens_merge": [_vp, _vp, _vp, _i64, _i32, _i32, _vp],
    "ens_finish": [_vp, _i64, _i32, _vp, _i32, _vp, _i32, _vp, _vp, _vp, _vp],
    "attn_cross_split": [_vp, _vp, _vp, _i32, _vp, _vp, _vp, _i64, _i32, _i32, _i32, _i32, _vp, _i64, _vp, _vp],
    "attn_cross_feat": [_vp, _vp, _vp, _i32, _i32, _vp, _vp, _vp, _i64, _i32, _i32, _i32, _vp, _i64, _vp, _vp],
    "pos_aug": [_vp, _i64, _vp, _i32, _i32, _i32, _vp, _vp, _vp],
    "keep_mask": [_vp, _i32, _i32, _vp, _i64, _vp, _vp, _i64, _vp, _vp, _vp],
    "points_bounds": [_vp, _i64, _vp, _vp],
    "points_mark": [_vp, _i64, _vp, _vp, _vp, _vp, _vp],
    "mask_compact_rank": [_vp, _i64, _vp, _vp, _vp, _vp, _i64, _vp],
    "points_link": [_vp, _i64, _vp, _i32, _vp, _vp, _vp, _vp, _vp, _vp],
    "cells_max": [_vp, _i32, _vp, _vp, _i64, _i32, _vp, _vp, _vp, _vp, _vp, _vp, _vp],
    "panop_queries": [_vp, _i32, _i32, C.c_float, _vp, _vp, _vp],
    "panop_argmax": [_vp, _i64, _i32, _vp, C.c_float, _vp, _vp, _vp, _vp, _vp, _vp],
    "panop_write": [_i64, _vp, _vp, _vp, _vp, _vp, _vp, _vp, C.c_double, C.c_uint64, _vp, _vp, _vp, _vp, _vp, _vp, _vp],
}
_RESTYPES = {"last_error": C.c_char_p, "workspace_bytes": _i64, "attn_workspace_bytes": _i64}
_OPTIONAL = {}

EXPORTED_SYMBOLS = tuple(_SIGNATURES.keys())


def _ptr(t: Optional[torch.Tensor]) -> Optional[int]:
    if t is None:
        return None
    return t.data_ptr()


STATUS_MAGNITUDE = 0x40
ROUTE_WIN_ALWAYS, ROUTE_WIN_NEVER, ROUTE_WIDE_ALWAYS, ROUTE_WIDE_NEVER, ROUTE_LIN_NEVER, ROUTE_GRID_NEVER = 0x1, 0x2, 0x4, 0x8, 0x10, 0x20


class CBackend:

    def __init__(self, path: str, prefix: str, device_type: str):
        if not os.path.exists(path):
            raise RuntimeError(
                f"{path} not found - build it first (python -m pasco_amd.build); "
                "pasco_amd has no CPU fallback")
        self.path = path
        self.prefix = prefix
        self.device_type = device_type
        self._serves_cuda = device_type == "cuda"
        self.lib = C.CDLL(path)
        self.fn: Dict[str, object] = {}
        ver = getattr(self.lib, prefix + "abi_version", None)
        v = int(ver()) if ver is not None else -1
        if v != ABI_VERSION:
            raise RuntimeError(f"{path}: C-ABI version {v}, this binding expects {ABI_VERSION} - rebuild the library "
                               "(python -m pasco_amd.build --force; oracle: python -m oracle.build)")
        dsz = getattr(self.lib, prefix + "conv_desc_size", None)
        if dsz is None or int(dsz()) != C.sizeof(ConvDesc):
            raise RuntimeError(f"{path}: sizeof(ph_conv_desc) = {None if dsz is None else int(dsz())}, the binding's mirror has "
                               f"{C.sizeof(ConvDesc)} bytes - rebuild the library against include/pasco_hip.h")
        for name, argtypes in _SIGNATURES.items():
            f = getattr(self.lib, prefix + name)
            f.argtypes = argtypes
            f.restype = _RESTYPES.get(name, C.c_int)
            self.fn[name] = f
        for name, argtypes in _OPTIONAL.items():
            f = getattr(self.lib, prefix + name, None)
            if f is not None:
                f.argtypes = argtypes
                f.restype = C.c_int
                self.fn[name] = f
        self._ws: Dict[torch.device, torch.Tensor] = {}
        self._status_ptrs: Dict[tuple, int] = {}
        self._tls = threading.local()
        self.checker_split = False

    def routing(self, bits: int):
        import contextlib

        @contextlib.contextmanager
        def cm():
            old = getattr(self._tls, "route", 0)
            self._tls.route = int(bits)
            try:
                yield self
            finally:
                self._tls.route = old
        return cm()

    def set_route(self, bits: int) -> int:
        old = getattr(self._tls, "route", 0)
        self._tls.route = int(bits)
        return old

    def has(self, name: str) -> bool:
        return name in self.fn

    def _check(self, rc: int, name: str):
        if rc != 0:
            msg = self.fn["last_error"]()
            raise RuntimeError(f"{self.prefix}{name} failed ({rc}): {msg.decode() if msg else ''}")

    def stream(self, device: torch.device) -> Optional[int]:
        if device.type == "cuda":
            idx = device.index
            if idx is None:
                idx = torch.cuda.current_device()
            return _raw_stream(idx)
        return None

    def _stream_key(self, device: torch.device):
        if device.type == "cuda" and device.index is None:
            device = torch.device("cuda", torch.cuda.current_device())
        return (device, self.stream(device) or 0)

    def release_stream(self, stream) -> int:
        handle = int(getattr(stream, "cuda_stream", stream) or 0)
        dev = getattr(stream, "device", None)
        if dev is None and torch.cuda.is_available():
            dev = torch.device("cuda", torch.cuda.current_device())
        drop = [k for k in self._ws
                if isinstance(k, tuple) and len(k) == 3 and isinstance(k[0], str) and isinstance(k[1], torch.device)
                and k[2] == handle and (dev is None or k[1] == dev)]
        for k in drop:
            del self._ws[k]
        for k in [k for k in self._status_ptrs if k[2] == handle and (dev is None or k[1] == dev.index)]:
            del self._status_ptrs[k]
        return len(drop)

    def workspace(self, n: int, device: torch.device) -> torch.Tensor:
        need = int(self.fn["workspace_bytes"](int(n)))
        key = ("ws",) + self._stream_key(device)
        ws = self._ws.get(key)
        if ws is None or ws.numel() < need:
            ws = torch.empty(max(need, 1 << 20), dtype=torch.uint8, device=device)
            self._ws[key] = ws
        return ws

    def _chk(self, t: torch.Tensor, dtype, name: str):
        if t.dtype is dtype and t.is_cuda == self._serves_cuda and t.is_contiguous():
            return
        if t.dtype != dtype:
            raise TypeError(f"{name}: expected {dtype}, got {t.dtype}")
        if not t.is_contiguous():
            raise ValueError(f"{name}: tensor must be contiguous")
        if t.device.type != self.device_type:
            raise ValueError(f"{name}: tensor on {t.device}, backend serves {self.device_type}")

    @staticmethod
    def table_capacity(n: int) -> int:
        cap = 16
        while cap < 2 * n:
            cap <<= 1
        return cap

    def map_insert(self, coords: torch.Tensor, dedup: bool = True):
        tkeys, tvals, row2uniq, uniq_rows, n_uniq = self.map_insert_launch(coords, dedup)
        if not dedup:
            return tkeys, tvals, None, None, coords.shape[0]
        nu = int(n_uniq.item())
        return tkeys, tvals, row2uniq, uniq_rows[:nu], nu

    def map_insert_launch(self, coords: torch.Tensor, dedup: bool = True, n_uniq: Optional[torch.Tensor] = None):
        self._chk(coords, torch.int32, "coords")
        n = coords.shape[0]
        dev = coords.device
        cap = self.table_capacity(n)
        table = torch.empty(cap + cap // 2, dtype=torch.int64, device=dev)
        tkeys = table[:cap]
        tvals = table[cap:].view(torch.int32)
        ws = torch.empty(int(self.fn["workspace_bytes"](int(n))), dtype=torch.uint8, device=dev)
        if dedup:
            m = max(n, 1)
            m4 = (m + 3) // 4 * 4
            rows2 = torch.empty(2 * m4 + 1, dtype=torch.int32, device=dev)
            row2uniq, uniq_rows = rows2[:m], rows2[m4:m4 + m]
            if n_uniq is None:
                n_uniq = rows2[2 * m4:]
            rc = self.fn["map_insert"](_ptr(coords), n, _ptr(tkeys), _ptr(tvals), cap, _ptr(row2uniq),
                                       _ptr(uniq_rows), n_uniq.data_ptr(), _ptr(ws), ws.numel(), self.status_ptr(dev),
                                       self.stream(dev))
            self._check(rc, "map_insert")
            return tkeys, tvals, row2uniq[:n], uniq_rows, n_uniq
        rc = self.fn["map_insert"](_ptr(coords), n, _ptr(tkeys), _ptr(tvals), cap, None, None, None,
                                   _ptr(ws), ws.numel(), self.status_ptr(dev), self.stream(dev))
        self._check(rc, "map_insert")
        return tkeys, tvals, None, None, None

    def map_find(self, query: torch.Tensor, tkeys: torch.Tensor, tvals: torch.Tensor) -> torch.Tensor:
        self._chk(query, torch.int32, "query")
        n = query.shape[0]
        out = torch.empty(n, dtype=torch.int32, device=query.device)
        rc = self.fn["map_find"](_ptr(query), n, _ptr(tkeys), _ptr(tvals), tkeys.numel(), _ptr(out),
                                 self.stream(query.device))
        self._check(rc, "map_find")
        return out

    def coords_floor(self, coords: torch.Tensor, ts: int) -> torch.Tensor:
        self._chk(coords, torch.int32, "coords")
        out = torch.empty_like(coords)
        rc = self.fn["coords_floor"](_ptr(coords), coords.shape[0], int(ts), _ptr(out),
                                     self.stream(coords.device))
        self._check(rc, "coords_floor")
        return out

    def coords_expand(self, coords: torch.Tensor, ts_out: int) -> torch.Tensor:
        self._chk(coords, torch.int32, "coords")
        n = coords.shape[0]
        out = torch.empty((n * 8, 4), dtype=torch.int32, device=coords.device)
        rc = self.fn["coords_expand"](_ptr(coords), n, int(ts_out), _ptr(out), self.stream(coords.device))
        self._check(rc, "coords_expand")
        return out

    def nbr_build(self, out_coords: torch.Tensor, tkeys: torch.Tensor, tvals: torch.Tensor,
                  offsets, same_map: bool = False) -> torch.Tensor:
        self._chk(out_coords, torch.int32, "out_coords")
        kvol = len(offsets)
        if not 1 <= kvol <= MAX_KVOL:
            raise ValueError(f"kernel volume {kvol} not supported (max {MAX_KVOL})")
        n_out = out_coords.shape[0]
        flat = (_i32 * (3 * kvol))(*[int(v) for o in offsets for v in o])
        nbr = torch.empty((kvol, n_out), dtype=torch.int32, device=out_coords.device)
        name = "nbr_build_same" if same_map else "nbr_build"
        rc = self.fn[name](_ptr(out_coords), n_out, _ptr(tkeys), _ptr(tvals), tkeys.numel(),
                           C.cast(flat, _vp), kvol, _ptr(nbr), self.stream(out_coords.device))
        self._check(rc, name)
        return nbr

    def rowlist_build(self, nbr: torch.Tensor) -> dict:
        self._chk(nbr, torch.int32, "nbr")
        kvol, n_out = nbr.shape
        pin, pout, counts = self.kmap_compact(nbr)
        cap = (n_out + kvol * 127 + 127) // 128 * 128
        tcap = cap // 128
        dev = nbr.device
        rl_in = torch.empty(cap, dtype=torch.int32, device=dev)
        rl_out = torch.empty(cap, dtype=torch.int32, device=dev)
        tile_k = torch.empty(tcap, dtype=torch.int32, device=dev)
        rc = self.fn["rowlist_pack"](_ptr(pin), _ptr(pout), _ptr(counts), kvol, n_out, _ptr(rl_in), _ptr(rl_out), _ptr(tile_k),
                                     cap, tcap, self.status_ptr(dev), self.stream(dev))
        self._check(rc, "rowlist_pack")
        return {"in": rl_in, "out": rl_out, "tile_k": tile_k}

    def win_build(self, nbr: torch.Tensor) -> dict:
        self._chk(nbr, torch.int32, "nbr")
        kvol, n_out = nbr.shape
        if kvol != 27:
            raise ValueError("win_build serves 3x3x3 kernel maps")
        dev = nbr.device
        t = (n_out + 127) // 128
        win = {"rows": torch.empty((max(t, 1), 27 * 128), dtype=torch.int32, device=dev),
               "cnt": torch.empty(max(t, 1), dtype=torch.int32, device=dev) if n_out > 0 else torch.zeros(1, dtype=torch.int32, device=dev),
               "slots": torch.empty((max(t, 1), 27, 128), dtype=torch.int16, device=dev),
               "stats": torch.empty(4, dtype=torch.int32, device=dev) if n_out > 0 else torch.zeros(4, dtype=torch.int32, device=dev),
               "n_out": n_out}
        rc = self.fn["win_build"](_ptr(nbr), kvol, n_out, _ptr(win["rows"]), _ptr(win["cnt"]), _ptr(win["slots"]),
                                  _ptr(win["stats"]), self.stream(dev))
        self._check(rc, "win_build")
        return win

    def kmap_compact(self, nbr: torch.Tensor):
        self._chk(nbr, torch.int32, "nbr")
        kvol, n_out = nbr.shape
        dev = nbr.device
        pin = torch.empty_like(nbr)
        pout = torch.empty_like(nbr)
        counts = torch.empty(kvol, dtype=torch.int32, device=dev)
        ws = self.workspace(n_out, dev)
        rc = self.fn["kmap_compact"](_ptr(nbr), kvol, n_out, _ptr(pin), _ptr(pout), _ptr(counts),
                                     _ptr(ws), ws.numel(), self.stream(dev))
        self._check(rc, "kmap_compact")
        return pin, pout, counts

    def conv_fwd(self, x: Optional[torch.Tensor], weight: Optional[torch.Tensor], nbr: Optional[torch.Tensor],
                 n_out: int, *, wshape=None, xshape=None, bias=None, pro_scale=None, pro_shift=None, pro_act=ACT_NONE, epi_scale=None,
                 epi_shift=None, epi_act=ACT_NONE, slope=0.01, residual=None, res_act=ACT_NONE,
                 epi2_scale=None, epi2_shift=None, split=None, in_split: Optional[torch.Tensor] = None,
                 emit_split=None, want_out: bool = True,
                 out: Optional[torch.Tensor] = None, win=None, in_split_has_prologue: bool = False, axis=None,
                 rowlist=None, out_split: Optional[torch.Tensor] = None, status: Optional[torch.Tensor] = None,
                 exact_if: Optional[torch.Tensor] = None, grid=None):
        if x is None:
            if xshape is None or in_split is None or split is None or len(split) != 2 or not self.split_capable():
                raise ValueError("conv: x=None needs xshape, in_split and a mode-2 split on the device backend")
            if pro_scale is not None or pro_shift is not None or pro_act != ACT_NONE:
                raise ValueError("conv: a pre-split input already carries its prologue")
            x = torch.empty((xshape[0], xshape[1]), dtype=torch.float32, device="meta")
            dev = in_split.device
        else:
            self._chk(x, torch.float32, "in")
            dev = x.device
        if weight is None:
            if wshape is None or split is None or len(split) != 2 or not self.split_capable():
                raise ValueError("conv: weight=None needs wshape and a mode-2 split on the device backend")
            kvol, cin, cout = wshape
        else:
            self._chk(weight, torch.float32, "weight")
            if weight.dim() == 2:
                kvol, (cin, cout) = 1, weight.shape
            else:
                kvol, cin, cout = weight.shape
        if x.shape[1] != cin:
            raise ValueError(f"conv: input has {x.shape[1]} channels, kernel expects {cin}")
        if nbr is not None:
            self._chk(nbr, torch.int32, "nbr")
            if tuple(nbr.shape) != (kvol, n_out):
                raise ValueError(f"conv: nbr shape {tuple(nbr.shape)} != {(kvol, n_out)}")
        emit = emit_split is not None and split is not None and len(split) == 2 and cout % 32 == 0
        if emit_split is not None and not emit:
            raise ValueError("conv: emit_split needs a mode-2 split and cout % 32 == 0")
        if out is None and (want_out or not emit):
            out = torch.empty((n_out, cout), dtype=torch.float32, device=dev)
        if emit and out_split is not None:
            if out_split.dtype != torch.float16 or not out_split.is_contiguous() or out_split.numel() != n_out * 2 * cout:
                raise ValueError("conv: out_split must be contiguous f16 [n_out, cout / 32, 2, 32]")
        else:
            out_split = torch.empty((n_out, cout // 32, 2, 32), dtype=torch.float16, device=dev) if emit else None
        if n_out == 0:
            return (out, out_split) if emit else out
        d = ConvDesc()
        d.route = getattr(self._tls, "route", 0)
        if emit:
            osc, osh, oact = emit_split
            for name, t in (("osp_scale", osc), ("osp_shift", osh)):
                if t is not None:
                    self._chk(t, torch.float32, name)
                    if t.numel() != cout:
                        raise ValueError(f"conv: {name} has {t.numel()} entries, expected {cout}")
            d.out_split, d.osp_scale, d.osp_shift, d.osp_act = _ptr(out_split), _ptr(osc), _ptr(osh), int(oact)
        d.in_, d.weight, d.nbr, d.out = (None if x.is_meta else _ptr(x)), _ptr(weight), _ptr(nbr), _ptr(out)
        d.n_in, d.n_out, d.cin, d.cout, d.kvol = x.shape[0], n_out, cin, cout, kvol
        d.pro_act, d.epi_act, d.res_act, d.epi_slope = pro_act, epi_act, res_act, float(slope)
        for name, t, c in (("pro_scale", pro_scale, cin), ("pro_shift", pro_shift, cin),
                           ("bias", bias, cout), ("epi_scale", epi_scale, cout),
                           ("epi_shift", epi_shift, cout), ("epi2_scale", epi2_scale, cout),
                           ("epi2_shift", epi2_shift, cout)):
            if t is not None:
                self._chk(t, torch.float32, name)
                if t.numel() != c:
                    raise ValueError(f"conv: {name} has {t.numel()} entries, expected {c}")
            setattr(d, name, _ptr(t))
        if residual is not None:
            self._chk(residual, torch.float32, "residual")
            if tuple(residual.shape) != (n_out, cout):
                raise ValueError("conv: residual shape mismatch")
        d.residual = _ptr(residual)
        if axis is not None:
            tab, acoords, lo = axis
            self._chk(tab, torch.float32, "axis table")
            self._chk(acoords, torch.int32, "axis coords")
            if tab.dim() != 3 or tab.shape[0] != 3 or tab.shape[2] != cout or tuple(acoords.shape) != (n_out, 4):
                raise ValueError("conv: axis = (table [3, T, cout], coords [n_out, 4], lo)")
            if self.device_type == "cuda" and (split is None or len(split) != 2):
                raise ValueError("conv: the axis-table residual is served by the pre-split (mode 2) path")
            d.axis_table, d.axis_coords, d.axis_lo, d.axis_rows = _ptr(tab), _ptr(acoords), int(lo), int(tab.shape[1])
        if split is not None:
            if len(split) == 2:
                w_split, unscale = split
                if in_split is None:
                    in_split = self.split_rows(x, pro_scale=pro_scale, pro_shift=pro_shift, pro_act=pro_act, slope=slope)
                elif not x.is_meta and (pro_scale is not None or pro_shift is not None or pro_act != ACT_NONE) and \
                        not in_split_has_prologue:
                    raise ValueError("conv: in_split given together with a prologue - pass in_split_has_prologue=True if "
                                     "the operand was built with split_rows(x, pro_scale=..., pro_shift=..., pro_act=...), "
                                     "else drop in_split")
                cpad = (cin + 31) // 32 * 32
                if in_split.dtype != torch.float16 or in_split.numel() != x.shape[0] * 2 * cpad:
                    raise ValueError("conv: in_split does not match the input rows")
                if w_split.numel() != kvol * cout * 2 * cpad:
                    raise ValueError("conv: w_split does not match the kernel")
                d.mma_mode, d.in_split, d.w_split = 2, _ptr(in_split), _ptr(w_split)
                if grid is not None and nbr is not None:
                    gd, gk = grid
                    if len(gd) != 4 or len(gk) != 3 or gd[0] * gd[1] * gd[2] * gd[3] != n_out or x.shape[0] != n_out or \
                            gk[0] * gk[1] * gk[2] != kvol or any(k % 2 == 0 for k in gk):
                        raise ValueError("conv: grid = ((B, X, Y, Z), (kx, ky, kz)) must describe the whole map (odd kernel sizes)")
                    for q in range(4):
                        d.grid_dims[q] = int(gd[q])
                    for q in range(3):
                        d.grid_kernel[q] = int(gk[q])
                if rowlist is not None and nbr is not None:
                    d.rl_in, d.rl_out, d.rl_tile_k = _ptr(rowlist["in"]), _ptr(rowlist["out"]), _ptr(rowlist["tile_k"])
                    d.rl_rows, d.rl_tiles = int(rowlist["in"].numel()), int(rowlist["tile_k"].numel())
                if win is not None and kvol == 27 and nbr is not None:
                    d.win_rows, d.win_cnt, d.win_slots, d.win_stats = (_ptr(win["rows"]), _ptr(win["cnt"]),
                                                                       _ptr(win["slots"]), _ptr(win["stats"]))
                    if 32 < cout <= 64 and self._serves_cuda:
                        d.w_frag = _ptr(self.weight_fragments(w_split, kvol, cout, cpad))
            else:
                w_hi, w_lo, unscale = split
                d.mma_mode, d.w_f16_hi, d.w_f16_lo = 1, _ptr(w_hi), _ptr(w_lo)
            d.split_exp2 = SPLIT_ACT_EXP2
            d.w_unscale = float(unscale) * 2.0 ** (-SPLIT_ACT_EXP2)
            d.status = self.status_ptr(dev) if status is None else status.data_ptr()
            if kvol > 1 or n_out * cout <= (1 << 23):
                need = 12 * n_out * cout * 4 if n_out * cout <= (1 << 23) else 512 * 128 * 128 * 4
                key = ("splitk",) + self._stream_key(dev)
                sk = self._ws.get(key)
                if sk is None or sk.numel() < need:
                    sk = torch.empty(need, dtype=torch.uint8, device=dev)
                    self._ws[key] = sk
                d.splitk_ws, d.splitk_ws_bytes = _ptr(sk), sk.numel()
        if exact_if is not None:
            if split is not None:
                raise ValueError("conv: exact_if guards an exact fp32 launch (no split)")
            d.exact_if = exact_if.data_ptr()
        rc = self.fn["conv_fwd"](C.byref(d), self.stream(dev))
        self._check(rc, "conv_fwd")
        return (out, out_split) if emit else out

    @staticmethod
    def grid_offsets(kernel_size) -> list:
        kx, ky, kz = (int(k) for k in kernel_size)
        return [(x, y, z) for z in range(-(kz // 2), kz // 2 + 1) for x in range(-(kx // 2), kx // 2 + 1)
                for y in range(-(ky // 2), ky // 2 + 1)]

    def conv_last_config(self) -> dict:
        buf = (_i32 * 8)()
        self._check(self.fn["conv_last_config"](C.cast(buf, _vp)), "conv_last_config")
        names = ("mma_mode", "bm", "bn", "kc", "ksplit", "emit", "kernel", "waves")
        return dict(zip(names, [int(v) for v in buf]))

    def status_word(self, device) -> torch.Tensor:
        return self._status_pair(device)[0:1]

    def status_ptr(self, device) -> int:
        pinned = getattr(self._tls, "status_pin", None)
        if pinned is not None:
            return pinned.data_ptr()
        idx = device.index
        if idx is None and device.type == "cuda":
            idx = torch.cuda.current_device()
        k = (device.type, idx, _raw_stream(idx) if device.type == "cuda" else 0)
        hit = self._status_ptrs.get(k)
        if hit is None:
            hit = self._status_pair(device).data_ptr()
            self._status_ptrs[k] = hit
        return hit

    def optimistic_word(self, device) -> torch.Tensor:
        return self._status_pair(device)[1:2]

    def _status_pair(self, device) -> torch.Tensor:
        pinned = getattr(self._tls, "status_pin", None)
        if pinned is not None:
            return pinned
        key = ("status",) + self._stream_key(torch.device(device))
        t = self._ws.get(key)
        if t is None:
            t = torch.zeros(2, dtype=torch.int32, device=device)
            self._ws[key] = t
        return t

    @contextlib.contextmanager
    def pin_status(self, device):
        prev = getattr(self._tls, "status_pin", None)
        self._tls.status_pin = None
        self._tls.status_pin = self._status_pair(device)
        try:
            yield
        finally:
            self._tls.status_pin = prev

    STATUS_TEXT = {
        1: "an activation outside the f16 range in a split-precision convolution / attention operand (rerun with "
           "pasco_amd.graph.fused.set_conv_precision('f32'); PascoNet.forward does so by itself)",
        2: "a coordinate outside the packable range (batch index 0..1023, coordinates -131072..131071, not all four at their "
           "maximum) was inserted into a coordinate map; the row was left out of the map",
        32: "a kernel map handed over as one-pair-per-output-row (fused.conv(..., one_pair=True): row lists of a generative "
            "transposed convolution) has another number of pairs than rows: output rows would stay unwritten (PASCO_CONV_RL=0)",
        16: "an optimistic shortcut of the graph did not hold (a fast path taken without the host read that would justify it: "
            "attention-mask block lookups with a coordinate outside its subnet's box, kept rows that are not the leading rows, "
            "an all-zero bottleneck site); PASCO_OPTIMISTIC=0 takes the checked paths; PascoNet.forward redoes the step by itself",
        8: "the fused input stage met a merged row that is entirely zero or a point outside its box (ME.to_sparse drops such a "
           "row: the stage has to run on its general path, PASCO_INPUT_FUSED=0; PascoNet.forward redoes it by itself)",
        4: "a coordinate outside the rows of a per-axis table residual (ph_conv_desc.axis_table) was clamped to the table's "
           "edge; the materialised forms are selected with PASCO_RESIZE_ABSORB=0 PASCO_PE_TABLE=0 PASCO_HEAD_ABSORB=0",
    }

    def check_status(self, device) -> None:
        t = self._ws.get(("status",) + self._stream_key(torch.device(device)))
        if t is None:
            return
        snap = t.clone()
        t.zero_()
        v, opt = snap.tolist()
        v &= ~STATUS_MAGNITUDE
        if opt != 0:
            v |= 16
        if v == 0:
            return
        msgs = [self.STATUS_TEXT[b] for b in (1, 2, 4, 8, 16, 32) if v & b]
        if v & ~63:
            msgs.append(f"unknown status bits {v & ~63:#x}")
        text = f"pasco_amd: device status {v:#x}: " + "; ".join(msgs)
        raise (F16RangeError if v == 1 else StatusError)(v, text)

    @staticmethod
    def split_weight_f16(weight: torch.Tensor, exponent=None):
        w = weight.detach().float()
        if w.dim() == 2:
            w = w[None]
        if exponent is not None:
            e = int(exponent)
        else:
            wmax = float(w.abs().max())
            e = 0 if wmax == 0.0 else 13 - int(torch.frexp(torch.tensor(wmax))[1])
        scaled = (w * float(2.0 ** e)).transpose(1, 2).contiguous()
        hi = scaled.to(torch.float16)
        lo = (scaled - hi.float()).to(torch.float16)
        return hi.contiguous(), lo.contiguous(), float(2.0 ** (-e))

    def split_rows(self, x: torch.Tensor, *, pro_scale=None, pro_shift=None, pro_act=ACT_NONE, slope=0.01,
                   out: Optional[torch.Tensor] = None, exp2: Optional[int] = None,
                   status: Optional[torch.Tensor] = None) -> torch.Tensor:
        exp2 = SPLIT_ACT_EXP2 if exp2 is None else int(exp2)
        self._chk(x, torch.float32, "in")
        n, c = x.shape
        if c % 8 != 0:
            raise ValueError("split_rows: needs c % 8 == 0")
        cpad = (c + 31) // 32 * 32
        if out is None:
            out = torch.empty((n, cpad // 32, 2, 32), dtype=torch.float16, device=x.device)
        for name, t in (("pro_scale", pro_scale), ("pro_shift", pro_shift)):
            if t is not None:
                self._chk(t, torch.float32, name)
                if t.numel() != c:
                    raise ValueError(f"split_rows: {name} has {t.numel()} entries, expected {c}")
        rc = self.fn["split_rows"](_ptr(x), n, c, _ptr(pro_scale), _ptr(pro_shift), pro_act, float(slope), exp2, _ptr(out),
                                   self.status_ptr(x.device) if status is None else status.data_ptr(), self.stream(x.device))
        self._check(rc, "split_rows")
        return out

    def split_weight_rows(self, weight: torch.Tensor, exponent=None):
        w = weight.detach().float()
        if w.dim() == 2:
            w = w[None]
        if exponent is not None:
            e = int(exponent)
        else:
            wmax = float(w.abs().max())
            e = 0 if wmax == 0.0 else 13 - int(torch.frexp(torch.tensor(wmax))[1])
        k, cin, cout = w.shape
        rows = (w * float(2.0 ** e)).transpose(1, 2).contiguous().view(k * cout, cin)
        return self.split_rows(rows, exp2=0), float(2.0 ** (-e))

    @staticmethod
    def weight_fragments(w_split: torch.Tensor, kvol: int, cout: int, cpad: int) -> torch.Tensor:
        hit = getattr(w_split, "_ph_wfrag", None)
        if hit is not None and hit[0] == (kvol, cout, cpad):
            return hit[1]
        g = cpad // 32
        ws = w_split.view(kvol, cout, g, 2, 2, 2, 8)
        rows = torch.arange(64, device=w_split.device).clamp_(max=cout - 1)
        ws = ws.index_select(1, rows).view(kvol, 2, 32, g, 2, 2, 2, 8)
        frag = ws.permute(0, 3, 5, 1, 4, 6, 2, 7).contiguous()
        frag = frag.view(kvol, 2 * g, 2, 2, 64, 8)
        try:
            w_split._ph_wfrag = ((kvol, cout, cpad), frag)
        except AttributeError:
            pass
        return frag

    def split_capable(self) -> bool:
        return self.device_type == "cuda" or self.checker_split

    def split_supported(self, cin: int, cout: int) -> bool:
        return self.split_capable() and cin % 8 == 0 and cout % 4 == 0

    def maxpool_fwd(self, x: torch.Tensor, nbr: torch.Tensor) -> torch.Tensor:
        self._chk(x, torch.float32, "in")
        self._chk(nbr, torch.int32, "nbr")
        kvol, n_out = nbr.shape
        out = torch.empty((n_out, x.shape[1]), dtype=torch.float32, device=x.device)
        rc = self.fn["maxpool_fwd"](_ptr(x), x.shape[1], _ptr(nbr), kvol, n_out, _ptr(out),
                                    self.stream(x.device))
        self._check(rc, "maxpool_fwd")
        return out

    def mask_compact(self, mask: torch.Tensor) -> torch.Tensor:
        if mask.dtype == torch.bool:
            mask = mask.view(torch.uint8)
        self._chk(mask, torch.uint8, "mask")
        n = mask.shape[0]
        dev = mask.device
        buf = torch.empty(max(n, 1) + 1, dtype=torch.int32, device=dev)
        keep, cnt = buf[:-1], buf[-1:]
        ws = self.workspace(n, dev)
        rc = self.fn["mask_compact"](_ptr(mask), n, _ptr(keep), cnt.data_ptr(), _ptr(ws), ws.numel(),
                                     self.stream(dev))
        self._check(rc, "mask_compact")
        return keep[: int(cnt.item())]

    MAX_INPUT_SITES = 1 << 27

    def pooled_merge(self, h: torch.Tensor, xyz: torch.Tensor, starts, bounds=None):
        self._chk(h, torch.float32, "h")
        self._chk(xyz, torch.int64, "xyz")
        n, c = h.shape
        m = len(starts) - 1
        if not (c % 4 == 0 and 1 <= m <= 8 and tuple(xyz.shape) == (n, 3)):
            raise ValueError("pooled_merge: h [P, C] with C % 4 == 0, xyz int64 [P, 3], at most 8 subnets")
        dev = h.device
        st = self.stream(dev)
        if bounds is None:
            b6 = torch.empty(6, dtype=torch.int32, device=dev)
            self._check(self.fn["points_bounds"](_ptr(xyz), n, _ptr(b6), st), "points_bounds")
            b6 = b6.tolist()
            lo, hi = b6[:3], b6[3:]
        else:
            lo, hi = [int(v) for v in bounds[0]], [int(v) for v in bounds[1]]
        dims = [hi[a] - lo[a] + 1 for a in range(3)]
        nsites = dims[0] * dims[1] * dims[2]
        if n == 0 or min(dims) <= 0 or nsites > self.MAX_INPUT_SITES:
            return None
        hlo, hdim = (_i32 * 3)(*lo), (_i32 * 3)(*dims)
        hst = (_i64 * (m + 1))(*[int(v) for v in starts])
        flags = torch.zeros(nsites, dtype=torch.uint8, device=dev)
        status = self.status_ptr(dev)
        self._check(self.fn["points_mark"](_ptr(xyz), n, C.cast(hlo, _vp), C.cast(hdim, _vp), _ptr(flags), status, st),
                    "points_mark")
        sites = torch.empty(min(n, nsites), dtype=torch.int32, device=dev)
        rank = torch.empty(nsites, dtype=torch.int32, device=dev)
        cnt = torch.empty(1, dtype=torch.int32, device=dev)
        ws = self.workspace(nsites, dev)
        self._check(self.fn["mask_compact_rank"](_ptr(flags), nsites, _ptr(sites), _ptr(rank), _ptr(cnt), _ptr(ws), ws.numel(),
                                                 st), "mask_compact_rank")
        v = int(cnt.item())
        head = torch.full((max(v * m, 1),), -1, dtype=torch.int32, device=dev)
        nxt = torch.empty(n, dtype=torch.int32, device=dev)
        self._check(self.fn["points_link"](_ptr(xyz), n, C.cast(hst, _vp), m, C.cast(hlo, _vp), C.cast(hdim, _vp), _ptr(rank),
                                           _ptr(head), _ptr(nxt), st), "points_link")
        out = torch.empty((v, m * c), dtype=torch.float32, device=dev)
        coords = torch.empty((v, 4), dtype=torch.int32, device=dev)
        self._check(self.fn["cells_max"](_ptr(h), c, _ptr(head), _ptr(nxt), v, m, _ptr(sites), C.cast(hlo, _vp), C.cast(hdim, _vp),
                                         _ptr(out), _ptr(coords), status, st), "cells_max")
        return coords, out

    def mask_compact_many(self, masks) -> list:
        masks = [m.view(torch.uint8) if m.dtype == torch.bool else m for m in masks]
        if not masks:
            return []
        dev = masks[0].device
        cnts = torch.empty(len(masks), dtype=torch.int32, device=dev)
        keeps = []
        for j, mask in enumerate(masks):
            self._chk(mask, torch.uint8, "mask")
            n = mask.shape[0]
            keep = torch.empty(max(n, 1), dtype=torch.int32, device=dev)
            ws = torch.empty(int(self.fn["workspace_bytes"](int(n))), dtype=torch.uint8, device=dev)
            rc = self.fn["mask_compact"](_ptr(mask), n, _ptr(keep), cnts[j:j + 1].data_ptr(), _ptr(ws), ws.numel(),
                                         self.stream(dev))
            self._check(rc, "mask_compact")
            keeps.append(keep)
        return [k[:c] for k, c in zip(keeps, cnts.tolist())]

    def gather_rows(self, src: torch.Tensor, rows: torch.Tensor, out: Optional[torch.Tensor] = None) -> torch.Tensor:
        if src.element_size() != 4:
            raise TypeError("gather_rows serves 4-byte element types")
        if not src.is_contiguous():
            raise ValueError("gather_rows: src must be contiguous")
        self._chk(rows, torch.int32, "rows")
        c = src.shape[1]
        if out is None:
            out = torch.empty((rows.shape[0], c), dtype=src.dtype, device=src.device)
        elif out.shape != (rows.shape[0], c) or out.dtype != src.dtype or not out.is_contiguous() or out.device != src.device:
            raise ValueError("gather_rows: out must be contiguous [M, C] of src's dtype")
        rc = self.fn["gather_rows"](_ptr(src), c, _ptr(rows), rows.shape[0], _ptr(out),
                                    self.stream(src.device))
        self._check(rc, "gather_rows")
        return out

    def scatter_add_rows(self, src: torch.Tensor, rows: torch.Tensor, dst: torch.Tensor) -> torch.Tensor:
        self._chk(src, torch.float32, "src")
        self._chk(dst, torch.float32, "dst")
        self._chk(rows, torch.int32, "rows")
        rc = self.fn["scatter_add_rows"](_ptr(src), src.shape[1], _ptr(rows), src.shape[0], _ptr(dst),
                                         self.stream(src.device))
        self._check(rc, "scatter_add_rows")
        return dst

    def sem_ensemble(self, logits, rows, want_conf: bool = True):
        m = len(logits)
        c = logits[0].shape[1]
        n = rows[0].shape[0]
        dev = logits[0].device
        d = SemEnsDesc()
        d.m, d.c, d.n_sites = m, c, n
        outs = [torch.empty((n, c), dtype=torch.float32, device=dev) for _ in range(m + 1)]
        confs = [torch.empty(n, dtype=torch.float32, device=dev) for _ in range(m + 1)] if want_conf else None
        for i in range(m):
            self._chk(logits[i], torch.float32, "logits")
            self._chk(rows[i], torch.int32, "rows")
            if logits[i].shape[1] != c or rows[i].shape[0] != n:
                raise ValueError("sem_ensemble: shape mismatch between subnets")
            d.logits[i], d.rows[i] = _ptr(logits[i]), _ptr(rows[i])
        for i in range(m + 1):
            d.out[i] = _ptr(outs[i])
            d.conf[i] = _ptr(confs[i]) if want_conf else None
        rc = self.fn["sem_ensemble"](C.byref(d), self.stream(dev))
        self._check(rc, "sem_ensemble")
        return outs, confs

    def to_dense(self, feats, coords, min3, ts: int, dims4) -> torch.Tensor:
        self._chk(feats, torch.float32, "feats")
        self._chk(coords, torch.int32, "coords")
        c = feats.shape[1]
        b, x, y, z = [int(v) for v in dims4]
        dense = torch.zeros((b, c, x, y, z), dtype=torch.float32, device=feats.device)
        hmin = (_i32 * 3)(*[int(v) for v in min3])
        hdim = (_i32 * 4)(b, x, y, z)
        rc = self.fn["to_dense"](_ptr(feats), _ptr(coords), feats.shape[0], c, C.cast(hmin, _vp), int(ts),
                                 C.cast(hdim, _vp), _ptr(dense), self.stream(feats.device))
        self._check(rc, "to_dense")
        return dense

    def to_sparse(self, dense: torch.Tensor):
        self._chk(dense, torch.float32, "dense")
        b, c, x, y, z = dense.shape
        dev = dense.device
        nsites = b * x * y * z
        coords = torch.empty((max(nsites, 1), 4), dtype=torch.int32, device=dev)
        cnt = torch.empty(1, dtype=torch.int32, device=dev)
        ws = self.workspace(nsites, dev)
        hdim = (_i32 * 4)(b, x, y, z)
        rc = self.fn["to_sparse_coords"](_ptr(dense), c, C.cast(hdim, _vp), _ptr(coords), _ptr(cnt),
                                         _ptr(ws), ws.numel(), self.stream(dev))
        self._check(rc, "to_sparse_coords")
        n = int(cnt.item())
        coords = coords[:n].contiguous()
        feats = self.dense_gather(dense, coords)
        return coords, feats

    def dense_gather(self, dense: torch.Tensor, site_coords: torch.Tensor) -> torch.Tensor:
        self._chk(dense, torch.float32, "dense")
        self._chk(site_coords, torch.int32, "site_coords")
        b, c, x, y, z = dense.shape
        n = site_coords.shape[0]
        feats = torch.empty((n, c), dtype=torch.float32, device=dense.device)
        hdim = (_i32 * 4)(b, x, y, z)
        rc = self.fn["dense_gather"](_ptr(dense), c, C.cast(hdim, _vp), _ptr(site_coords), n, _ptr(feats),
                                     self.stream(dense.device))
        self._check(rc, "dense_gather")
        return feats


    def keep_mask(self, srcs, coords: Optional[torch.Tensor] = None, lo: Optional[torch.Tensor] = None,
                  hi: Optional[torch.Tensor] = None, fallback_rows: int = 0) -> torch.Tensor:
        srcs = list(srcs)
        if not srcs:
            if coords is None or lo is None:
                raise ValueError("keep_mask: no source and no box")
            kind, n, dev = 0, coords.shape[0], coords.device
        else:
            kind = 1 if srcs[0].dtype == torch.int32 else 0
            n = srcs[0].shape[0]
            dev = srcs[0].device
        for t in srcs:
            if t.shape != (n,) or not t.is_contiguous() or (t.dtype == torch.int32) != (kind == 1) or \
                    (kind == 0 and t.dtype not in (torch.bool, torch.uint8)):
                raise ValueError("keep_mask: sources must be contiguous [n] tensors, all int32 or all bool / uint8")
        if (lo is None) != (hi is None):
            raise ValueError("keep_mask: give both corners or neither")
        if lo is not None:
            self._chk(coords, torch.int32, "coords")
            self._chk(lo, torch.int32, "lo")
            self._chk(hi, torch.int32, "hi")
            if coords.shape != (n, 4) or lo.numel() != 3 or hi.numel() != 3:
                raise ValueError("keep_mask: coords [n, 4], corners [3]")
        out = torch.empty((n,), dtype=torch.bool, device=dev)
        ptrs = (_vp * len(srcs))(*[_ptr(t) for t in srcs])
        word = None
        if fallback_rows > 0:
            key = ("keep_any",) + self._stream_key(dev)
            word = self._ws.get(key)
            if word is None:
                word = torch.zeros(1, dtype=torch.int32, device=dev)
                self._ws[key] = word
        rc = self.fn["keep_mask"](C.cast(ptrs, _vp), len(srcs), kind, _ptr(coords) if lo is not None else None, n, _ptr(lo),
                                  _ptr(hi), int(fallback_rows), _ptr(out), _ptr(word), self.stream(dev))
        self._check(rc, "keep_mask")
        return out

    def attn_mask_pack(self, vals: torch.Tensor, b: int, n: int, positive_only: bool = False, want_any: bool = True):
        self._chk(vals, torch.float32, "vals")
        qn = vals.shape[1]
        assert vals.shape[0] == b * n
        bits = torch.empty((b, n, 4), dtype=torch.int32, device=vals.device)
        any_ = torch.empty((b, 4), dtype=torch.int32, device=vals.device) if want_any else None
        rc = self.fn["attn_mask_pack"](_ptr(vals), n, b, qn, 1 if positive_only else 0, _ptr(bits), _ptr(any_),
                                       self.stream(vals.device))
        self._check(rc, "attn_mask_pack")
        return bits, any_

    def bits_orpool(self, bits: torch.Tensor, nbr: torch.Tensor) -> torch.Tensor:
        self._chk(bits, torch.int32, "bits")
        self._chk(nbr, torch.int32, "nbr")
        kvol, n_out = nbr.shape
        out = torch.empty((n_out, 4), dtype=torch.int32, device=bits.device)
        rc = self.fn["bits_orpool"](_ptr(bits), _ptr(nbr), kvol, n_out, _ptr(out), self.stream(bits.device))
        self._check(rc, "bits_orpool")
        return out

    def bits_block_or(self, level_coords: torch.Tensor, n_per_b: int, s: int, tkeys, tvals, bits: torch.Tensor, lo=None,
                      hi=None, want_range: bool = False, range_word: Optional[torch.Tensor] = None):
        self._chk(level_coords, torch.int32, "level_coords")
        self._chk(bits, torch.int32, "bits")
        m = level_coords.shape[0]
        out = torch.empty((m, 4), dtype=torch.int32, device=bits.device)
        rng = torch.zeros(1, dtype=torch.int32, device=bits.device) if want_range else range_word
        if rng is not None:
            self._chk(lo, torch.int32, "lo")
            self._chk(hi, torch.int32, "hi")
        rc = self.fn["bits_block_or"](_ptr(level_coords), m, int(n_per_b), int(s), _ptr(tkeys), _ptr(tvals), tkeys.numel(),
                                      _ptr(bits), _ptr(lo), _ptr(hi), _ptr(out), _ptr(rng), self.stream(bits.device))
        self._check(rc, "bits_block_or")
        return (out, rng) if want_range else out

    def bits_or_reduce(self, bits: torch.Tensor) -> torch.Tensor:
        self._chk(bits, torch.int32, "bits")
        b, n, _ = bits.shape
        out = torch.empty((b, 4), dtype=torch.int32, device=bits.device)
        rc = self.fn["bits_or_reduce"](_ptr(bits), n, b, _ptr(out), self.stream(bits.device))
        self._check(rc, "bits_or_reduce")
        return out

    def sine_pe(self, coords: torch.Tensor, dim_t: torch.Tensor, scale: float, coff: int = 0,
                table: Optional[torch.Tensor] = None, tab_lo: int = 0) -> torch.Tensor:
        self._chk(coords, torch.int32, "coords")
        self._chk(dim_t, torch.float32, "dim_t")
        n, cstride = coords.shape
        f = dim_t.numel()
        tab_n = 0
        if table is not None:
            self._chk(table, torch.float32, "table")
            if table.dim() != 2 or table.shape[1] != f:
                raise ValueError("sine_pe: table must be [T, f]")
            tab_n = table.shape[0]
        out = torch.empty((n, 3 * f), dtype=torch.float32, device=coords.device)
        rc = self.fn["sine_pe"](_ptr(coords), n, cstride, coff, f, _ptr(dim_t), float(scale), _ptr(table), int(tab_lo),
                                tab_n, _ptr(out), self.stream(coords.device))
        self._check(rc, "sine_pe")
        return out

    def sine_pe_table(self, dim_t: torch.Tensor, scale: float, lo: int, hi: int) -> torch.Tensor:
        v = torch.arange(lo, hi, dtype=torch.int32, device=dim_t.device)
        c = torch.stack([v, v, v], dim=1).contiguous()
        return self.sine_pe(c, dim_t, scale)[:, : dim_t.numel()].contiguous()

    def attn_supported(self, qn: int, dh: int) -> bool:
        return qn <= 128 and (dh == 48 or self.device_type == "cpu")

    def attn_cross_fwd(self, q, k, v, bits=None, any_=None) -> torch.Tensor:
        for t, nm in ((q, "q"), (k, "k"), (v, "v")):
            self._chk(t, torch.float32, nm)
        b, h, qn, dh = q.shape
        n = k.shape[1]
        assert k.shape == (b, n, h * dh) and v.shape == k.shape
        out = torch.empty((b, qn, h * dh), dtype=torch.float32, device=q.device)
        need = int(self.fn["attn_workspace_bytes"](n, b, h, qn, dh))
        key = ("attn",) + self._stream_key(q.device)
        ws = self._ws.get(key)
        if ws is None or ws.numel() < need:
            ws = torch.empty(need, dtype=torch.uint8, device=q.device)
            self._ws[key] = ws
        rc = self.fn["attn_cross_fwd"](_ptr(q), _ptr(k), _ptr(v), _ptr(bits), _ptr(any_), _ptr(out), n, b, h, qn, dh,
                                       _ptr(ws), ws.numel(), self.stream(q.device))
        self._check(rc, "attn_cross_fwd")
        return out


    def attn_cross_split(self, q, k_split, v_split, n: int, bits=None, any_=None, exp2=None) -> torch.Tensor:
        self._chk(q, torch.float32, "q")
        b, h, qn, dh = q.shape
        d = h * dh
        for t, nm in ((k_split, "k_split"), (v_split, "v_split")):
            assert t.dtype == torch.float16 and t.is_contiguous() and t.numel() == b * n * d * 2, nm
        exp2 = SPLIT_ACT_EXP2 if exp2 is None else int(exp2)
        out = torch.empty((b, qn, d), dtype=torch.float32, device=q.device)
        need = int(self.fn["attn_workspace_bytes"](n, b, h, qn, dh))
        key = ("attn",) + self._stream_key(q.device)
        ws = self._ws.get(key)
        if ws is None or ws.numel() < need:
            ws = torch.empty(need, dtype=torch.uint8, device=q.device)
            self._ws[key] = ws
        rc = self.fn["attn_cross_split"](_ptr(q), _ptr(k_split), _ptr(v_split), exp2, _ptr(bits), _ptr(any_), _ptr(out),
                                         n, b, h, qn, dh, _ptr(ws), ws.numel(), self.status_ptr(q.device),
                                         self.stream(q.device))
        self._check(rc, "attn_cross_split")
        return out


    POS_AUG_COLS = 16

    def pos_aug(self, coords: torch.Tensor, eps: torch.Tensor, tab_lo: int, exp2: Optional[int] = None) -> torch.Tensor:
        exp2 = SPLIT_ACT_EXP2 if exp2 is None else int(exp2)
        self._chk(coords, torch.int32, "coords")
        self._chk(eps, torch.float32, "eps")
        n = coords.shape[0]
        assert coords.shape[1] == 4
        out = torch.empty((n, self.POS_AUG_COLS), dtype=torch.float16, device=coords.device)
        rc = self.fn["pos_aug"](_ptr(coords), n, _ptr(eps), int(tab_lo), eps.numel(), exp2, _ptr(out),
                                self.status_ptr(coords.device), self.stream(coords.device))
        self._check(rc, "pos_aug")
        return out

    def attn_feat_supported(self, qn: int, c: int) -> bool:
        return qn <= 128 and (c == 64 or (self.device_type == "cpu" and c % 32 == 0)) and self.has("attn_cross_feat")

    def attn_cross_feat(self, q2, x_split, aug, n: int, bits=None, any_=None, exp2=None) -> torch.Tensor:
        self._chk(q2, torch.float32, "q2")
        b, h, qn, d = q2.shape
        c = d - self.POS_AUG_COLS
        assert x_split.dtype == torch.float16 and x_split.is_contiguous() and x_split.numel() == b * n * c * 2, "x_split"
        assert aug.dtype == torch.float16 and aug.is_contiguous() and aug.numel() == b * n * self.POS_AUG_COLS, "aug"
        exp2 = SPLIT_ACT_EXP2 if exp2 is None else int(exp2)
        out = torch.empty((b, qn, h * d), dtype=torch.float32, device=q2.device)
        need = int(self.fn["attn_workspace_bytes"](n, b, h, qn, d))
        key = ("attn",) + self._stream_key(q2.device)
        ws = self._ws.get(key)
        if ws is None or ws.numel() < need:
            ws = torch.empty(need, dtype=torch.uint8, device=q2.device)
            self._ws[key] = ws
        rc = self.fn["attn_cross_feat"](_ptr(q2), _ptr(x_split), _ptr(aug), c, exp2, _ptr(bits), _ptr(any_), _ptr(out), n, b, h,
                                        qn, _ptr(ws), ws.numel(), self.status_ptr(q2.device), self.stream(q2.device))
        self._check(rc, "attn_cross_feat")
        return out

    def project_canonical(self, T: torch.Tensor, size, resolution: float, min_bound) -> torch.Tensor:
        T = T.to(dtype=torch.float32).contiguous()
        if T.device.type != self.device_type:
            raise ValueError(f"T on {T.device}, backend serves {self.device_type}")
        assert T.shape[-1] == 4 and T.shape[0] >= 3
        x, y, z = (int(v) for v in size)
        out = torch.empty((x * y * z, 4), dtype=torch.int32, device=T.device)
        mb = (C.c_float * 3)(*[float(v) for v in min_bound])
        rc = self.fn["project_canonical"](_ptr(T), x, y, z, float(resolution), C.cast(mb, _vp), _ptr(out), self.stream(T.device))
        self._check(rc, "project_canonical")
        return out

    def ens_resample(self, logits: torch.Tensor, rows: torch.Tensor, sel: torch.Tensor):
        self._chk(logits, torch.float32, "logits")
        self._chk(rows, torch.int32, "rows")
        self._chk(sel, torch.int32, "sel")
        n, q = logits.shape
        u = sel.shape[0]
        out = torch.empty((u, q), dtype=torch.float32, device=logits.device)
        flag = torch.empty((u,), dtype=torch.uint8, device=logits.device)
        rc = self.fn["ens_resample"](_ptr(logits), n, q, _ptr(rows), _ptr(sel), u, _ptr(out), _ptr(flag), self.stream(logits.device))
        self._check(rc, "ens_resample")
        return out, flag

    def ens_merge(self, anchor: torch.Tensor, m: torch.Tensor, perm: torch.Tensor, i: int) -> torch.Tensor:
        self._chk(anchor, torch.float32, "anchor")
        self._chk(m, torch.float32, "m")
        self._chk(perm, torch.int32, "perm")
        u, q = anchor.shape
        assert m.shape == anchor.shape and perm.numel() == q
        rc = self.fn["ens_merge"](_ptr(anchor), _ptr(m), _ptr(perm), u, q, int(i), self.stream(anchor.device))
        self._check(rc, "ens_merge")
        return anchor

    def ens_finish(self, anchor: torch.Tensor, keep: torch.Tensor, sem: torch.Tensor, sel: torch.Tensor):
        self._chk(anchor, torch.float32, "anchor")
        self._chk(keep, torch.int32, "keep")
        self._chk(sem, torch.float32, "sem")
        self._chk(sel, torch.int32, "sel")
        u, q = anchor.shape
        qk = keep.numel()
        out = torch.empty((u, qk), dtype=torch.float32, device=anchor.device)
        flag = torch.empty((u,), dtype=torch.uint8, device=anchor.device)
        rc = self.fn["ens_finish"](_ptr(anchor), u, q, _ptr(keep), qk, _ptr(sem), sem.shape[1], _ptr(sel), _ptr(out), _ptr(flag),
                                   self.stream(anchor.device))
        self._check(rc, "ens_finish")
        return out, flag


    PANOP_QMAX = 128

    def panoptic_rows(self, masks: torch.Tensor, qp: torch.Tensor, object_mask_threshold: float, overlap_threshold: float,
                      vox_occ_threshold: float, thing_ids, reduce_areas=None) -> dict:
        self._chk(masks, torch.float32, "masks")
        self._chk(qp, torch.float32, "qp")
        n, q = masks.shape
        c1 = qp.shape[1]
        if qp.shape[0] != q or not 1 <= q <= self.PANOP_QMAX or not 2 <= c1 <= 64:
            raise ValueError("panoptic_rows: masks [n, q], qp [q, c1] with q <= 128 queries and c1 <= 64 classes")
        dev = masks.device
        st = self.stream(dev)
        Q = self.PANOP_QMAX
        tabs = torch.zeros((4 + 1 + 5 + 2, Q), dtype=torch.int32, device=dev)
        qtab, nk, seg, areas = tabs[0:4], tabs[4, 0:1], tabs[5:10], tabs[10:12]
        self._check(self.fn["panop_queries"](_ptr(qp), q, c1, float(object_mask_threshold), qtab.data_ptr(), nk.data_ptr(),
                                             st), "panop_queries")
        per_i = torch.empty((3, max(n, 1)), dtype=torch.int32, device=dev)
        per_f = torch.empty((5, max(n, 1)), dtype=torch.float32, device=dev)
        own = torch.empty(max(n, 1), dtype=torch.uint8, device=dev)
        self._check(self.fn["panop_argmax"](_ptr(masks), n, q, qtab.data_ptr(), float(vox_occ_threshold), per_i[0].data_ptr(),
                                            _ptr(own), per_f[0].data_ptr(), per_f[1].data_ptr(), areas.data_ptr(), st),
                    "panop_argmax")
        if reduce_areas is not None:
            reduce_areas(areas)
        thing = 0
        for t in thing_ids:
            if 0 <= int(t) < 64:
                thing |= 1 << int(t)
        self._check(self.fn["panop_write"](n, per_i[0].data_ptr(), _ptr(own), per_f[0].data_ptr(), per_f[1].data_ptr(),
                                           areas.data_ptr(), qtab.data_ptr(), nk.data_ptr(), float(overlap_threshold), thing,
                                           per_i[1].data_ptr(), per_i[2].data_ptr(), per_f[2].data_ptr(), per_f[3].data_ptr(),
                                           per_f[4].data_ptr(), seg.data_ptr(), st), "panop_write")
        return {"panoptic": per_i[1, :n], "semantic": per_i[2, :n], "ins_unc": per_f[2, :n], "vox_conf": per_f[3, :n],
                "vox_unc": per_f[4, :n], "winner": per_i[0, :n], "own": own[:n], "qtab": qtab, "nk": nk, "seg": seg,
                "areas": areas, "tabs": tabs}


_raw_stream = getattr(torch._C, "_cuda_getCurrentRawStream", None)
if _raw_stream is None:
    def _raw_stream(idx: int) -> int:
        return torch.cuda.current_stream(idx).cuda_stream


_hip_backend: Optional[CBackend] = None
_checker_backend: Optional[CBackend] = None


def hip_backend() -> CBackend:
    global _hip_backend
    if _hip_backend is None:
        _hip_backend = CBackend(HIP_LIB_PATH, "ph_", "cuda")
    return _hip_backend


def register_checker_backend(backend: Optional[CBackend]) -> None:
    global _checker_backend
    _checker_backend = backend


def backend_for(device: torch.device) -> CBackend:
    device = torch.device(device)
    if device.type == "cuda":
        return hip_backend()
    if _checker_backend is not None and device.type == _checker_backend.device_type:
        return _checker_backend
    raise RuntimeError(
        f"pasco_amd serves ROCm GPU tensors only (got device '{device}'); there is no CPU path. "
        "Move tensors to cuda:N (MI355X) - tests may register a checker backend explicitly.")
```

pasco_amd/me/core.py:

```python
from __future__ import annotations

import itertools
from typing import Dict, List, Optional, Sequence, Tuple

import torch

from .backend import CBackend, backend_for

_key_counter = itertools.count()


def _triple(v) -> Tuple[int, int, int]:
    if type(v) is tuple and len(v) == 3 and type(v[0]) is int and type(v[1]) is int and type(v[2]) is int:
        return v
    if isinstance(v, torch.Tensor):
        v = v.tolist()
    if isinstance(v, (list, tuple)):
        if len(v) == 1:
            return (int(v[0]),) * 3
        assert len(v) == 3, f"expected 3 values, got {v}"
        return tuple(int(a) for a in v)
    return (int(v),) * 3


class CoordinateMapKey:

    __slots__ = ("tensor_stride", "uid")

    def __init__(self, tensor_stride, uid: Optional[int] = None):
        self.tensor_stride = _triple(tensor_stride)
        self.uid = next(_key_counter) if uid is None else uid

    def get_tensor_stride(self) -> List[int]:
        return list(self.tensor_stride)

    def get_key(self):
        return (list(self.tensor_stride), str(self.uid))

    def __hash__(self):
        return hash((self.tensor_stride, self.uid))

    def __eq__(self, other):
        return isinstance(other, CoordinateMapKey) and self.uid == other.uid and self.tensor_stride == other.tensor_stride

    def __repr__(self):
        return f"CoordinateMapKey(stride={list(self.tensor_stride)}, id={self.uid})"


class _CoordMap:
    __slots__ = ("coords", "_tkeys", "_tvals", "n", "_build")

    def __init__(self, coords, tkeys, tvals, build=None):
        self.coords = coords
        self._tkeys = tkeys
        self._tvals = tvals
        self._build = build
        self.n = coords.shape[0]

    def _table(self):
        if self._tkeys is None:
            self._tkeys, self._tvals = self._build(self.coords)
            self._build = None

    @property
    def tkeys(self):
        self._table()
        return self._tkeys

    @property
    def tvals(self):
        self._table()
        return self._tvals


def tensor_version(t: torch.Tensor) -> Optional[int]:
    try:
        return t._version
    except RuntimeError:
        return None


def kernel_offsets(kernel_size, tensor_stride, dilation=1, transposed=False) -> List[Tuple[int, int, int]]:
    kx, ky, kz = _triple(kernel_size)
    sx, sy, sz = _triple(tensor_stride)
    dx, dy, dz = _triple(dilation)
    sign = -1 if transposed else 1

    def rng(k):
        return range(-(k // 2), k // 2 + 1) if k % 2 == 1 else range(0, k)

    return [(sign * x * sx * dx, sign * y * sy * dy, sign * z * sz * dz)
            for z in rng(kz) for y in rng(ky) for x in rng(kx)]


class CoordinateManager:

    def __init__(self, D: int = 3, device=None):
        assert D == 3, "only 3 spatial dimensions are served"
        self.D = D
        self.device = torch.device(device) if device is not None else None
        self._maps: Dict[CoordinateMapKey, _CoordMap] = {}
        self._stride_cache: Dict[tuple, CoordinateMapKey] = {}
        self._kmap_cache: Dict[tuple, torch.Tensor] = {}
        self._origin: Dict[CoordinateMapKey, Tuple[CoordinateMapKey, torch.Tensor]] = {}

    def backend(self) -> CBackend:
        return backend_for(self.device)

    def _register(self, coords, tkeys, tvals, tensor_stride) -> CoordinateMapKey:
        key = CoordinateMapKey(tensor_stride)
        self._maps[key] = _CoordMap(coords, tkeys, tvals)
        return key

    def get_coordinates(self, key: CoordinateMapKey) -> torch.Tensor:
        return self._maps[key].coords

    def size(self, key: CoordinateMapKey) -> int:
        return self._maps[key].n

    def number_of_unique_batch_indices(self) -> int:
        bs = set()
        for m in self._maps.values():
            if m.n:
                bs.update(torch.unique(m.coords[:, 0]).tolist())
        return len(bs)

    def insert_and_map(self, coords: torch.Tensor, tensor_stride=1):
        if self.device is None:
            self.device = coords.device
        coords = coords.to(torch.int32).contiguous()
        be = self.backend()
        tkeys, tvals, row2uniq, uniq_rows, nu = be.map_insert(coords, dedup=True)
        if nu != coords.shape[0]:
            coords = be.gather_rows(coords, uniq_rows)
        else:
            uniq_rows = None
        key = self._register(coords, tkeys, tvals, tensor_stride)
        return key, (row2uniq, uniq_rows)

    def insert_unique(self, coords: torch.Tensor, tensor_stride) -> CoordinateMapKey:
        if self.device is None:
            self.device = coords.device
        coords = coords.to(torch.int32).contiguous()
        be = self.backend()
        if be.device_type != "cuda":
            tkeys, tvals, _, _, _ = be.map_insert(coords, dedup=False)
            return self._register(coords, tkeys, tvals, tensor_stride)
        key = self._register(coords, None, None, tensor_stride)
        self._maps[key]._build = lambda c: be.map_insert(c, dedup=False)[:2]
        return key

    def stride(self, in_key: CoordinateMapKey, stride) -> CoordinateMapKey:
        s = _triple(stride)
        assert s[0] == s[1] == s[2], "isotropic strides only"
        if s[0] == 1:
            return in_key
        ck = (in_key, s)
        if ck in self._stride_cache:
            return self._stride_cache[ck]
        m = self._maps[in_key]
        ts_out = tuple(a * b for a, b in zip(in_key.tensor_stride, s))
        be = self.backend()
        floored = be.coords_floor(m.coords, ts_out[0])
        tkeys, tvals, row2uniq, uniq_rows, nu = be.map_insert(floored, dedup=True)
        out_coords = be.gather_rows(floored, uniq_rows) if nu != floored.shape[0] else floored
        key = self._register(out_coords, tkeys, tvals, ts_out)
        self._stride_cache[ck] = key
        self._origin[key] = (in_key, row2uniq)
        return key

    def stride_chain(self, in_key: CoordinateMapKey, levels: int) -> List[CoordinateMapKey]:
        keys, todo, k = [], [], in_key
        for l in range(levels):
            nxt = self._stride_cache.get((k, (2, 2, 2)))
            if nxt is None:
                break
            keys.append(nxt)
            k = nxt
        if len(keys) == levels:
            return keys
        if keys:
            for l in range(len(keys), levels):
                keys.append(self.stride(keys[-1] if keys else in_key, 2))
            return keys
        m = self._maps[in_key]
        be = self.backend()
        ts0 = in_key.tensor_stride[0]
        cnts = torch.empty(levels, dtype=torch.int32, device=m.coords.device)
        parts = []
        for l in range(levels):
            floored = be.coords_floor(m.coords, ts0 << (l + 1))
            parts.append((floored,) + be.map_insert_launch(floored, dedup=True, n_uniq=cnts[l:l + 1]))
        counts = cnts.tolist()
        prev_key, prev_first = in_key, None
        for l, (floored, tkeys, tvals, row2uniq, uniq_rows, _) in enumerate(parts):
            nu = counts[l]
            uniq_rows = uniq_rows[:nu]
            coords = be.gather_rows(floored, uniq_rows) if nu != floored.shape[0] else floored
            ts = ts0 << (l + 1)
            key = self._register(coords, tkeys, tvals, (ts, ts, ts))
            self._stride_cache[(prev_key, (2, 2, 2))] = key
            r2u = row2uniq if prev_first is None else be.gather_rows(row2uniq.reshape(-1, 1).contiguous(), prev_first).reshape(-1)
            self._origin[key] = (prev_key, r2u)
            prev_key, prev_first = key, uniq_rows
            keys.append(key)
        return keys

    def expand(self, in_key: CoordinateMapKey, stride) -> CoordinateMapKey:
        s = _triple(stride)
        assert s == (2, 2, 2), "generative expansion is served for kernel 2 / stride 2"
        ts_in = in_key.tensor_stride
        assert all(t % 2 == 0 for t in ts_in), "cannot up-sample below tensor stride 1"
        ts_out = tuple(t // 2 for t in ts_in)
        m = self._maps[in_key]
        be = self.backend()
        children = be.coords_expand(m.coords, ts_out[0])
        tkeys, tvals, row2uniq, uniq_rows, nu = be.map_insert(children, dedup=True)
        out_coords = be.gather_rows(children, uniq_rows) if nu != children.shape[0] else children
        return self._register(out_coords, tkeys, tvals, ts_out)

    def expand_pruned(self, in_key: CoordinateMapKey, stride, keep_of) -> CoordinateMapKey:
        s = _triple(stride)
        assert s == (2, 2, 2), "generative expansion is served for kernel 2 / stride 2"
        ts_in = in_key.tensor_stride
        assert all(t % 2 == 0 for t in ts_in), "cannot up-sample below tensor stride 1"
        ts_out = tuple(t // 2 for t in ts_in)
        m = self._maps[in_key]
        be = self.backend()
        children = be.coords_expand(m.coords, ts_out[0])
        keep = be.mask_compact(keep_of(children).contiguous())
        return self.insert_unique(be.gather_rows(children, keep), ts_out)

    def prune(self, in_key: CoordinateMapKey, mask: torch.Tensor):
        m = self._maps[in_key]
        assert mask.shape[0] == m.n, f"mask has {mask.shape[0]} rows, map has {m.n}"
        last = self.__dict__.get("_last_prune")
        if last is not None and last[0] == in_key and last[1] is mask and last[2] == tensor_version(mask):
            return last[3], last[4]
        be = self.backend()
        keep = be.mask_compact(mask.contiguous())
        coords = be.gather_rows(m.coords, keep)
        out_key = self.insert_unique(coords, in_key.tensor_stride)
        self.__dict__["_last_prune"] = (in_key, mask, tensor_version(mask), out_key, keep)
        return out_key, keep

    def prune_batch(self, jobs):
        be = self.backend()
        uniq, order = {}, []
        for in_key, mask in jobs:
            m = self._maps[in_key]
            assert mask.shape[0] == m.n, f"mask has {mask.shape[0]} rows, map has {m.n}"
            k = (in_key, id(mask), tensor_version(mask))
            if k not in uniq:
                uniq[k] = len(order)
                order.append((in_key, mask))
        keeps = be.mask_compact_many([mask.contiguous() for _, mask in order])
        done = []
        for (in_key, mask), keep in zip(order, keeps):
            coords = be.gather_rows(self._maps[in_key].coords, keep)
            done.append((self.insert_unique(coords, in_key.tensor_stride), keep))
        return [done[uniq[(in_key, id(mask), tensor_version(mask))]] for in_key, mask in jobs]

    def union(self, key_a: CoordinateMapKey, key_b: CoordinateMapKey):
        assert key_a.tensor_stride == key_b.tensor_stride, "union needs equal tensor strides"
        ma, mb = self._maps[key_a], self._maps[key_b]
        be = self.backend()
        cat = torch.cat([ma.coords, mb.coords], dim=0)
        tkeys, tvals, row2uniq, uniq_rows, nu = be.map_insert(cat, dedup=True)
        coords = be.gather_rows(cat, uniq_rows) if nu != cat.shape[0] else cat
        key = self._register(coords, tkeys, tvals, key_a.tensor_stride)
        return key, row2uniq[: ma.n], row2uniq[ma.n:]

    def kernel_map(self, in_key: CoordinateMapKey, out_key: CoordinateMapKey, kernel_size,
                   dilation=1, transposed: bool = False) -> torch.Tensor:
        ks = _triple(kernel_size)
        dl = _triple(dilation)
        ck = (in_key, out_key, ks, dl, transposed)
        nbr = self._kmap_cache.get(ck)
        if nbr is None:
            base_stride = out_key.tensor_stride if transposed else in_key.tensor_stride
            offs = kernel_offsets(ks, base_stride, dl, transposed)
            mi, mo = self._maps[in_key], self._maps[out_key]
            k = len(offs)
            same = in_key == out_key and not transposed and k % 2 == 1 and k > 1 and all(
                tuple(offs[i]) == tuple(-v for v in offs[k - 1 - i]) for i in range(k // 2 + 1))
            nbr = self.backend().nbr_build(mo.coords, mi.tkeys, mi.tvals, offs, same_map=same)
            self._kmap_cache[ck] = nbr
        return nbr

    def kernel_windows(self, nbr: torch.Tensor):
        cache = self.__dict__.setdefault("_win_cache", {})
        key = nbr.data_ptr()
        hit = cache.get(key)
        if hit is None or hit[0] is not nbr:
            hit = (nbr, self.backend().win_build(nbr))
            cache[key] = hit
        return hit[1]

    def kernel_rowlist(self, nbr: torch.Tensor):
        cache = self.__dict__.setdefault("_rl_cache", {})
        key = nbr.data_ptr()
        hit = cache.get(key)
        if hit is None or hit[0] is not nbr:
            hit = (nbr, self.backend().rowlist_build(nbr))
            cache[key] = hit
        return hit[1]

    def kernel_map_coo(self, in_key, out_key, kernel_size, dilation=1, transposed=False):
        nbr = self.kernel_map(in_key, out_key, kernel_size, dilation, transposed)
        pin, pout, counts = self.backend().kmap_compact(nbr)
        counts = counts.tolist()
        return [(pin[k, :c], pout[k, :c]) for k, c in enumerate(counts)]

    def find(self, key: CoordinateMapKey, query: torch.Tensor) -> torch.Tensor:
        m = self._maps[key]
        return self.backend().map_find(query.to(torch.int32).contiguous(), m.tkeys, m.tvals)


class SparseTensor:

    def __init__(self, features: torch.Tensor, coordinates: Optional[torch.Tensor] = None,
                 tensor_stride=1, coordinate_map_key: Optional[CoordinateMapKey] = None,
                 coordinate_manager: Optional[CoordinateManager] = None, quantization_mode=None,
                 device=None, **_unused):
        assert isinstance(features, torch.Tensor), "features must be a torch.Tensor"
        assert features.dim() == 2, f"features must be [N, C], got {tuple(features.shape)}"
        if device is not None:
            features = features.to(device)
        if coordinate_map_key is None:
            assert coordinates is not None, "either coordinates or coordinate_map_key is required"
            assert coordinates.dim() == 2 and coordinates.shape[1] == 4, "coordinates must be [N, 4] (b,x,y,z)"
            assert coordinates.shape[0] == features.shape[0], "coordinates / features row mismatch"
            if coordinates.dtype in (torch.float32, torch.float64):
                coordinates = torch.floor(coordinates)
            coordinates = coordinates.to(device=features.device, dtype=torch.int32)
            if coordinate_manager is None:
                coordinate_manager = CoordinateManager(D=3, device=features.device)
            coordinate_map_key, (row2uniq, uniq_rows) = coordinate_manager.insert_and_map(
                coordinates, tensor_stride)
            if uniq_rows is not None:
                features = coordinate_manager.backend().gather_rows(features.contiguous(), uniq_rows)
            self.unique_index = uniq_rows
            self.inverse_mapping = row2uniq
        else:
            assert coordinate_manager is not None, "coordinate_map_key needs its coordinate_manager"
            n = coordinate_manager.size(coordinate_map_key)
            assert features.shape[0] == n, f"features have {features.shape[0]} rows, map has {n}"
            self.unique_index = None
            self.inverse_mapping = None
        self._F = features
        self._pending = None
        self._manager = coordinate_manager
        self.coordinate_map_key = coordinate_map_key

    @classmethod
    def deferred(cls, src: "SparseTensor", scale, shift, act: int, slope: float) -> "SparseTensor":
        assert src._pending is None
        out = cls(src._F, coordinate_map_key=src.coordinate_map_key, coordinate_manager=src._manager)
        out._pending = (scale, shift, int(act), float(slope))
        return out

    def _materialise(self) -> None:
        scale, shift, act, slope = self._pending
        y = self._F
        if scale is not None:
            y = y * scale
        if shift is not None:
            y = y + shift
        if act == 1:
            y = torch.relu(y)
        elif act == 2:
            y = torch.nn.functional.leaky_relu(y, slope)
        self._F, self._pending = y, None

    def take_prologue(self):
        return self._F, self._pending

    @property
    def F(self) -> torch.Tensor:
        if self._pending is not None:
            self._materialise()
        return self._F

    @property
    def features(self) -> torch.Tensor:
        return self.F

    @property
    def C(self) -> torch.Tensor:
        return self._manager.get_coordinates(self.coordinate_map_key)

    @property
    def coordinates(self) -> torch.Tensor:
        return self.C

    @property
    def coordinate_manager(self) -> CoordinateManager:
        return self._manager

    @property
    def tensor_stride(self) -> List[int]:
        return list(self.coordinate_map_key.tensor_stride)

    @property
    def shape(self):
        return self._F.shape

    def size(self, *a):
        return self._F.size(*a)

    @property
    def device(self):
        return self._F.device

    @property
    def dtype(self):
        return self._F.dtype

    @property
    def D(self) -> int:
        return 3

    def __len__(self):
        return self._F.shape[0]

    def __repr__(self):
        return (f"SparseTensor(N={self._F.shape[0]}, C={self._F.shape[1]}, "
                f"tensor_stride={self.tensor_stride}, device={self.device})")

    def _binary(self, other, fn_same, is_add: bool):
        if not isinstance(other, SparseTensor):
            return SparseTensor(fn_same(self.F, other), coordinate_map_key=self.coordinate_map_key,
                                coordinate_manager=self._manager)
        assert other._manager is self._manager, "binary ops need tensors of the same coordinate manager"
        if other.coordinate_map_key == self.coordinate_map_key:
            return SparseTensor(fn_same(self.F, other.F), coordinate_map_key=self.coordinate_map_key,
                                coordinate_manager=self._manager)
        assert is_add, "only + is served across different coordinate maps"
        assert self._F.shape[1] == other._F.shape[1], "channel mismatch in union add"
        be = self._manager.backend()
        key, a2o, b2o = self._manager.union(self.coordinate_map_key, other.coordinate_map_key)
        n_out = self._manager.size(key)
        na = self._F.shape[0]
        out = torch.empty((n_out, self._F.shape[1]), dtype=self._F.dtype, device=self._F.device)
        out[:na].copy_(self.F)
        if n_out > na:
            out[na:].zero_()
        be.scatter_add_rows(other.F.contiguous(), b2o.contiguous(), out)
        return SparseTensor(out, coordinate_map_key=key, coordinate_manager=self._manager)

    def __add__(self, other):
        return self._binary(other, lambda a, b: a + b, True)

    def __sub__(self, other):
        return self._binary(other, lambda a, b: a - b, False)

    def __mul__(self, other):
        return self._binary(other, lambda a, b: a * b, False)

    def dense(self, shape: Optional[torch.Size] = None, min_coordinate: Optional[torch.Tensor] = None,
              contract_stride: bool = True):
        ts = self.tensor_stride
        coords = self.C
        if min_coordinate is None:
            if coords.shape[0]:
                mn = coords[:, 1:].min(dim=0)[0]
                if not bool((mn >= 0).all()):
                    raise ValueError(f"Coordinate has a negative value: {mn.tolist()}. "
                                     "Please provide min_coordinate argument")
            min3 = [0, 0, 0]
            min_ret = torch.zeros((1, 3), dtype=torch.int32)
        else:
            assert min_coordinate.numel() == 3, "min_coordinate must have 3 entries"
            min3 = [int(v) for v in min_coordinate.reshape(-1).tolist()]
            assert all(m % t == 0 for m, t in zip(min3, ts)), \
                "The minimum coordinates must be divisible by the tensor stride."
            min_ret = min_coordinate.reshape(1, 3).to(self.device)
        step = ts[0] if contract_stride else 1
        c = self._F.shape[1]
        if shape is None:
            if coords.shape[0] == 0:
                dims = (1, 1, 1, 1)
            else:
                mx = coords.max(dim=0)[0].tolist()
                dims = (mx[0] + 1, *[(mx[1 + a] - min3[a]) // step + 1 for a in range(3)])
        else:
            assert len(shape) == 5, "shape must be [B, C, X, Y, Z]"
            dims = (int(shape[0]), int(shape[2]), int(shape[3]), int(shape[4]))
        be = self._manager.backend()
        dense = be.to_dense(self.F.contiguous(), coords, min3, step, dims)
        return dense, min_ret, torch.IntTensor(ts)

    def features_at(self, batch_index: int) -> torch.Tensor:
        return self.F[self.C[:, 0] == batch_index]

    def coordinates_at(self, batch_index: int) -> torch.Tensor:
        c = self.C
        return c[c[:, 0] == batch_index][:, 1:]


class TensorField:
    pass


def to_sparse(x: torch.Tensor, format: Optional[str] = None, coordinates=None, device=None) -> SparseTensor:
    assert x.dim() == 5, "to_sparse serves [B, C, X, Y, Z] tensors"
    assert format in (None, "BCXXX"), "only the default BCXXX layout is served"
    be = backend_for(x.device)
    coords, feats = be.to_sparse(x.contiguous().float())
    mgr = CoordinateManager(D=3, device=x.device)
    key = mgr.insert_unique(coords, 1)
    return SparseTensor(feats, coordinate_map_key=key, coordinate_manager=mgr)


def batched_coordinates(coords: Sequence[torch.Tensor], dtype=torch.int32, device=None) -> torch.Tensor:
    out = []
    for b, c in enumerate(coords):
        if not isinstance(c, torch.Tensor):
            c = torch.as_tensor(c)
        c = torch.floor(c) if c.dtype.is_floating_point else c
        c = c.to(dtype)
        bcol = torch.full((c.shape[0], 1), b, dtype=dtype, device=c.device)
        out.append(torch.cat([bcol, c], dim=1))
    res = torch.cat(out, dim=0) if out else torch.zeros((0, 4), dtype=dtype)
    return res.to(device) if device is not None else res.cpu()
```

Measured before the change: 48.81.

## Derive pruned-map kernel maps from parent tables and fuse prune/compaction kernels

Adds a fused prune operation that compacts a mask and gathers the coordinates in one count/scatter pass per batch of jobs. Pruned maps remember their parent, so a same-map kernel map can be derived from the parent's cached neighbor table by restricting it through keep_rows and rank_of instead of rebuilding it with hash lookups. Compaction also drops the separate scan kernel for small inputs by having each block sum the earlier block counts itself, and it fuses rank assignment into the scatter. A multi-tensor gather kernel is added as well. The cost is extra bookkeeping, parent references that keep buffers alive, and a redundant per-block prefix sum.

```diff
diff --git a/include/pasco_map.h b/include/pasco_map.h
--- /dev/null
+++ b/include/pasco_map.h
@@ -0,0 +1,42 @@
+#ifndef PASCO_MAP_H_
+#define PASCO_MAP_H_
+
+#include <stdint.h>
+
+#ifdef __cplusplus
+extern "C" {
+#endif
+
+#define PM_ABI_VERSION 1
+#define PM_MAX_JOBS 16
+#define PM_MAX_GATHER 8
+
+typedef void *pm_stream_t;
+
+int pm_abi_version(void);
+const char *pm_last_error(void);
+
+typedef struct pm_prune_job {
+  const uint8_t *mask;
+  int64_t n;
+  const int32_t *parent_coords;
+  int32_t *keep_rows;
+  int32_t *rank_of;
+  int32_t *out_coords;
+} pm_prune_job;
+
+int64_t pm_prune_workspace_bytes(int64_t n);
+
+int pm_prune_rows(const pm_prune_job *h_jobs, int32_t n_jobs, int32_t *n_keep, void *ws, int64_t ws_bytes,
+                  pm_stream_t stream);
+
+int pm_nbr_restrict(const int32_t *parent_nbr, int64_t n_parent, int32_t kvol, const int32_t *keep_rows,
+                    const int32_t *rank_of, int64_t n_keep, int32_t *child_nbr, pm_stream_t stream);
+
+int pm_gather_rows_multi(const void *const *h_srcs, const int32_t *h_widths, int32_t count, const int32_t *rows,
+                         int64_t n_out, void *const *h_dsts, const int64_t *h_n_pad, pm_stream_t stream);
+
+#ifdef __cplusplus
+}
+#endif
+#endif
diff --git a/pasco_amd/build.py b/pasco_amd/build.py
--- a/pasco_amd/build.py
+++ b/pasco_amd/build.py
@@ -11,7 +11,8 @@
 HEADERS = ["ph_common.h", "conv_h2_common.h", os.path.join("..", "..", "include", "pasco_hip.h"),
            os.path.join("..", "..", "include", "pasco_eval.h"),
            os.path.join("..", "..", "include", "pasco_frame.h"),
-           os.path.join("..", "..", "include", "pasco_label.h")]
+           os.path.join("..", "..", "include", "pasco_label.h"),
+           os.path.join("..", "..", "include", "pasco_map.h")]
 HIPCC = os.environ.get("HIPCC", "/opt/rocm/bin/hipcc")
 FLAGS = ["--offload-arch=gfx950", "-O3", "-std=c++17", "-fPIC", "-Wall", "-Wno-unused-function"]
 
diff --git a/pasco_amd/csrc/coords.hip b/pasco_amd/csrc/coords.hip
--- a/pasco_amd/csrc/coords.hip
+++ b/pasco_amd/csrc/coords.hip
@@ -1,6 +1,7 @@
 #include <stdarg.h>
 
 #include "ph_common.h"
+#include "../../include/pasco_map.h"
 
 static thread_local char g_err[512] = "";
 
@@ -27,7 +28,7 @@
 
 template <class Pred>
 __global__ void __launch_bounds__(CP_THREADS)
-    k_compact_count(Pred pred, int64_t n, int32_t *__restrict__ block_counts) {
+    k_compact_count(Pred pred, int64_t n, int32_t *__restrict__ block_counts, uint8_t *__restrict__ flags) {
   const int seg = blockIdx.y;
   const int nb = gridDim.x;
   const int64_t base = (int64_t)blockIdx.x * CP_TILE;
@@ -36,6 +37,7 @@
   for (int r = 0; r < CP_ROUNDS; ++r) {
     int64_t i = base + r * CP_THREADS + threadIdx.x;
     bool p = (i < n) && pred(seg, i);
+    if (Pred::kStoresVerdict && i < n) flags[(int64_t)seg * n + i] = p ? 1 : 0;
     cnt += __popcll(__ballot(p));
   }
   __shared__ int wcnt[CP_THREADS / PH_WAVE];
@@ -73,19 +75,28 @@
   if (threadIdx.x == 0) totals[seg] = carry;
 }
 
+__device__ __forceinline__ int cp_block_sum(const int32_t *__restrict__ counts, int m, int *red) {
+  int s = 0;
+  for (int i = threadIdx.x; i < m; i += CP_THREADS) s += counts[i];
+#pragma unroll
+  for (int d = 32; d >= 1; d >>= 1) s += __shfl_xor(s, d);
+  if ((threadIdx.x & 63) == 0) red[threadIdx.x >> 6] = s;
+  __syncthreads();
+  s = red[0] + red[1] + red[2] + red[3];
+  __syncthreads();
+  return s;
+}
+
 template <class Pred, class Emit>
-__global__ void __launch_bounds__(CP_THREADS)
-    k_compact_scatter(Pred pred, Emit emit, int64_t n, const int32_t *__restrict__ block_offsets) {
-  const int seg = blockIdx.y;
-  const int nb = gridDim.x;
-  const int64_t base = (int64_t)blockIdx.x * CP_TILE;
-  __shared__ int wcnt[CP_THREADS / PH_WAVE];
+__device__ __forceinline__ int cp_scatter_tile(const Pred &pred, const Emit &emit, int seg, int64_t n, int64_t base, int running,
+                                               const uint8_t *__restrict__ flags, int *wcnt) {
   const int wave = threadIdx.x >> 6, lane = threadIdx.x & 63;
-  int running = block_offsets[(int64_t)seg * nb + blockIdx.x];
 #pragma unroll 1
   for (int r = 0; r < CP_ROUNDS; ++r) {
     int64_t i = base + r * CP_THREADS + threadIdx.x;
-    bool p = (i < n) && pred(seg, i);
+    bool p;
+    if (Pred::kStoresVerdict) p = (i < n) && flags[(int64_t)seg * n + i] != 0;
+    else p = (i < n) && pred(seg, i);
     unsigned long long b = __ballot(p);
     int wtot = __popcll(b);
     int wpre = __popcll(b & ((1ull << lane) - 1ull));
@@ -98,28 +109,49 @@
     running += tot;
     __syncthreads();
   }
-}
+  return running;
+}
+
+template <class Pred, class Emit>
+__global__ void __launch_bounds__(CP_THREADS)
+    k_compact_scatter(Pred pred, Emit emit, int64_t n, const int32_t *__restrict__ block_counts, const uint8_t *__restrict__ flags,
+                      int scanned, int32_t *__restrict__ totals) {
+  const int seg = blockIdx.y;
+  const int nb = gridDim.x;
+  __shared__ int wcnt[CP_THREADS / PH_WAVE];
+  const int32_t *c = block_counts + (int64_t)seg * nb;
+  int running = scanned ? c[blockIdx.x] : cp_block_sum(c, (int)blockIdx.x, wcnt);
+  running = cp_scatter_tile(pred, emit, seg, n, (int64_t)blockIdx.x * CP_TILE, running, flags, wcnt);
+  if (!scanned && blockIdx.x == (unsigned)(nb - 1) && threadIdx.x == 0) totals[seg] = running;
+}
+
+constexpr int64_t CP_FOLD_MAX_BLOCKS = 2048;
 
 template <class Pred, class Emit>
 static int compact_run(Pred pred, Emit emit, int64_t n, int segs, int32_t *totals, void *ws,
                        int64_t ws_bytes, hipStream_t st) {
   int64_t nb = (n + CP_TILE - 1) / CP_TILE;
   if (nb < 1) nb = 1;
-  PH_REQUIRE(ws_bytes >= (int64_t)segs * nb * 4, "compaction workspace too small (%lld < %lld)",
-             (long long)ws_bytes, (long long)(segs * nb * 4));
+  const int64_t need = (int64_t)segs * nb * 4 + (Pred::kStoresVerdict ? (int64_t)segs * n : 0);
+  PH_REQUIRE(ws_bytes >= need, "compaction workspace too small (%lld < %lld)", (long long)ws_bytes, (long long)need);
   int32_t *block_counts = (int32_t *)ws;
+  uint8_t *flags = Pred::kStoresVerdict ? (uint8_t *)(block_counts + (int64_t)segs * nb) : nullptr;
   dim3 grid((unsigned)nb, (unsigned)segs);
-  hipLaunchKernelGGL(k_compact_count<Pred>, grid, dim3(CP_THREADS), 0, st, pred, n, block_counts);
-  PH_LAUNCH_CHECK();
-  hipLaunchKernelGGL(k_compact_scan, dim3(segs), dim3(256), 0, st, block_counts, (int)nb, totals);
-  PH_LAUNCH_CHECK();
+  hipLaunchKernelGGL(k_compact_count<Pred>, grid, dim3(CP_THREADS), 0, st, pred, n, block_counts, flags);
+  PH_LAUNCH_CHECK();
+  const int scanned = nb > CP_FOLD_MAX_BLOCKS;
+  if (scanned) {
+    hipLaunchKernelGGL(k_compact_scan, dim3(segs), dim3(256), 0, st, block_counts, (int)nb, totals);
+    PH_LAUNCH_CHECK();
+  }
   hipLaunchKernelGGL((k_compact_scatter<Pred, Emit>), grid, dim3(CP_THREADS), 0, st, pred, emit, n,
-                     block_counts);
+                     block_counts, flags, scanned, totals);
   PH_LAUNCH_CHECK();
   return 0;
 }
 
 struct PredFlag {
+  static constexpr bool kStoresVerdict = false;
   const uint8_t *flags;
   __device__ bool operator()(int, int64_t i) const { return flags[i] != 0; }
 };
@@ -171,6 +203,7 @@
 }
 
 struct PredFirst {
+  static constexpr bool kStoresVerdict = true;
   const int32_t *tvals;
   const int32_t *row_slot;
   __device__ bool operator()(int, int64_t i) const {
@@ -179,14 +212,16 @@
   }
 };
 
-__global__ void __launch_bounds__(256)
-    k_assign_rank(int64_t n, const int32_t *__restrict__ rank_of,
-                  const int32_t *__restrict__ row_slot, int32_t *__restrict__ tvals) {
-  int64_t i = (int64_t)blockIdx.x * blockDim.x + threadIdx.x;
-  if (i >= n) return;
-  int r = rank_of[i];
-  if (r >= 0) tvals[row_slot[i]] = r;
-}
+struct EmitFirst {
+  int32_t *uniq_rows;
+  const int32_t *row_slot;
+  int32_t *tvals;
+  __device__ void operator()(int, int64_t i, int rank) const {
+    if (rank < 0) return;
+    uniq_rows[rank] = (int32_t)i;
+    tvals[row_slot[i]] = rank;
+  }
+};
 
 __global__ void __launch_bounds__(256)
     k_row2uniq(int64_t n, const int32_t *__restrict__ row_slot, const int32_t *__restrict__ tvals,
@@ -226,17 +261,14 @@
   PH_REQUIRE(row2uniq && n_uniq, "map_insert: row2uniq / n_uniq required with uniq_rows");
   PH_REQUIRE(ws_bytes >= ph_workspace_bytes(n), "map_insert: workspace too small");
   int32_t *row_slot = (int32_t *)ws;
-  int32_t *rank_of = row_slot + n;
-  char *rest = (char *)(rank_of + n);
-  int64_t rest_bytes = ws_bytes - 8 * n;
+  char *rest = (char *)(row_slot + n);
+  int64_t rest_bytes = ws_bytes - 4 * n;
   hipLaunchKernelGGL(k_insert, dim3(nblk(n, 256)), dim3(256), 0, st, (const int4 *)coords, n,
                      (unsigned long long *)tkeys, tvals, mask, row_slot, status);
   PH_LAUNCH_CHECK();
-  int rc = compact_run(PredFirst{tvals, row_slot}, EmitRows{uniq_rows, rank_of}, n, 1, n_uniq, rest,
+  int rc = compact_run(PredFirst{tvals, row_slot}, EmitFirst{uniq_rows, row_slot, tvals}, n, 1, n_uniq, rest,
                        rest_bytes, st);
   if (rc) return rc;
-  hipLaunchKernelGGL(k_assign_rank, dim3(nblk(n, 256)), dim3(256), 0, st, n, rank_of, row_slot, tvals);
-  PH_LAUNCH_CHECK();
   hipLaunchKernelGGL(k_row2uniq, dim3(nblk(n, 256)), dim3(256), 0, st, n, row_slot, tvals, row2uniq);
   PH_LAUNCH_CHECK();
   return 0;
@@ -378,6 +410,7 @@
 }
 
 struct PredNbr {
+  static constexpr bool kStoresVerdict = false;
   const int32_t *nbr;
   int64_t n_out;
   __device__ bool operator()(int seg, int64_t i) const { return nbr[(int64_t)seg * n_out + i] >= 0; }
@@ -457,3 +490,127 @@
   PH_LAUNCH_CHECK();
   return 0;
 }
+
+extern "C" int pm_abi_version(void) { return PM_ABI_VERSION; }
+extern "C" const char *pm_last_error(void) { return g_err; }
+
+struct PmJobs {
+  const uint8_t *mask[PM_MAX_JOBS];
+  const int4 *coords[PM_MAX_JOBS];
+  int32_t *keep_rows[PM_MAX_JOBS];
+  int32_t *rank_of[PM_MAX_JOBS];
+  int4 *out_coords[PM_MAX_JOBS];
+  int32_t *counts[PM_MAX_JOBS];
+  int64_t n[PM_MAX_JOBS];
+  int32_t nb[PM_MAX_JOBS];
+};
+
+struct EmitPrune {
+  const int4 *coords;
+  int32_t *keep_rows;
+  int32_t *rank_of;
+  int4 *out_coords;
+  __device__ void operator()(int, int64_t i, int rank) const {
+    rank_of[i] = rank;
+    if (rank < 0) return;
+    keep_rows[rank] = (int32_t)i;
+    out_coords[rank] = coords[i];
+  }
+};
+
+__global__ void __launch_bounds__(CP_THREADS) k_prune_count(PmJobs jobs) {
+  const int job = blockIdx.y;
+  if ((int)blockIdx.x >= jobs.nb[job]) return;
+  const uint8_t *__restrict__ mask = jobs.mask[job];
+  const int64_t n = jobs.n[job];
+  const int64_t base = (int64_t)blockIdx.x * CP_TILE;
+  int cnt = 0;
+#pragma unroll
+  for (int r = 0; r < CP_ROUNDS; ++r) {
+    int64_t i = base + r * CP_THREADS + threadIdx.x;
+    bool p = (i < n) && mask[i] != 0;
+    cnt += __popcll(__ballot(p));
+  }
+  __shared__ int wcnt[CP_THREADS / PH_WAVE];
+  const int wave = threadIdx.x >> 6, lane = threadIdx.x & 63;
+  if (lane == 0) wcnt[wave] = cnt;
+  __syncthreads();
+  if (threadIdx.x == 0) jobs.counts[job][blockIdx.x] = wcnt[0] + wcnt[1] + wcnt[2] + wcnt[3];
+}
+
+__global__ void __launch_bounds__(CP_THREADS) k_prune_scatter(PmJobs jobs, int32_t *__restrict__ n_keep) {
+  const int job = blockIdx.y;
+  const int nb = jobs.nb[job];
+  if ((int)blockIdx.x >= nb) return;
+  __shared__ int wcnt[CP_THREADS / PH_WAVE];
+  int running = cp_block_sum(jobs.counts[job], (int)blockIdx.x, wcnt);
+  running = cp_scatter_tile(PredFlag{jobs.mask[job]}, EmitPrune{jobs.coords[job], jobs.keep_rows[job], jobs.rank_of[job], jobs.out_coords[job]},
+                            0, jobs.n[job], (int64_t)blockIdx.x * CP_TILE, running, nullptr, wcnt);
+  if ((int)blockIdx.x == nb - 1 && threadIdx.x == 0) n_keep[job] = running;
+}
+
+static inline int64_t pm_tiles(int64_t n) {
+  int64_t nb = (n + CP_TILE - 1) / CP_TILE;
+  return nb < 1 ? 1 : nb;
+}
+
+extern "C" int64_t pm_prune_workspace_bytes(int64_t n) {
+  if (n < 0) n = 0;
+  return (pm_tiles(n) * 4 + 255) / 256 * 256;
+}
+
+extern "C" int pm_prune_rows(const pm_prune_job *h_jobs, int32_t n_jobs, int32_t *n_keep, void *ws, int64_t ws_bytes,
+                             pm_stream_t stream) {
+  PH_REQUIRE(n_jobs >= 1 && n_jobs <= PM_MAX_JOBS, "prune_rows: %d jobs, 1 .. %d served", n_jobs, PM_MAX_JOBS);
+  PH_REQUIRE(h_jobs != nullptr && n_keep != nullptr, "prune_rows: null jobs / n_keep");
+  PmJobs jobs;
+  memset(&jobs, 0, sizeof(jobs));
+  int64_t used = 0, max_nb = 1;
+  for (int j = 0; j < n_jobs; ++j) {
+    const pm_prune_job &q = h_jobs[j];
+    PH_REQUIRE(q.n >= 0 && q.n < 0x7FFFFFFF, "prune_rows: job %d has bad n=%lld", j, (long long)q.n);
+    PH_REQUIRE(q.n == 0 || (q.mask && q.parent_coords && q.keep_rows && q.rank_of && q.out_coords), "prune_rows: job %d has a null pointer", j);
+    PH_REQUIRE((((uintptr_t)q.parent_coords | (uintptr_t)q.out_coords) & 15) == 0, "prune_rows: job %d: coordinates must be 16-byte aligned", j);
+    const int64_t nb = pm_tiles(q.n);
+    PH_REQUIRE(nb <= CP_FOLD_MAX_BLOCKS, "prune_rows: job %d has %lld rows, at most %lld served", j, (long long)q.n, (long long)(CP_FOLD_MAX_BLOCKS * CP_TILE));
+    jobs.mask[j] = q.mask;
+    jobs.coords[j] = (const int4 *)q.parent_coords;
+    jobs.keep_rows[j] = q.keep_rows;
+    jobs.rank_of[j] = q.rank_of;
+    jobs.out_coords[j] = (int4 *)q.out_coords;
+    jobs.counts[j] = (int32_t *)((char *)ws + used);
+    jobs.n[j] = q.n;
+    jobs.nb[j] = (int32_t)nb;
+    used += pm_prune_workspace_bytes(q.n);
+    if (nb > max_nb) max_nb = nb;
+  }
+  PH_REQUIRE(ws != nullptr && ws_bytes >= used, "prune_rows: workspace too small (%lld < %lld)", (long long)ws_bytes, (long long)used);
+  hipStream_t st = ph_stream(stream);
+  dim3 grid((unsigned)max_nb, (unsigned)n_jobs);
+  hipLaunchKernelGGL(k_prune_count, grid, dim3(CP_THREADS), 0, st, jobs);
+  PH_LAUNCH_CHECK();
+  hipLaunchKernelGGL(k_prune_scatter, grid, dim3(CP_THREADS), 0, st, jobs, n_keep);
+  PH_LAUNCH_CHECK();
+  return 0;
+}
+
+__global__ void __launch_bounds__(256)
+    k_nbr_restrict(const int32_t *__restrict__ parent_nbr, int64_t n_parent, const int32_t *__restrict__ keep_rows,
+                   const int32_t *__restrict__ rank_of, int64_t n_keep, int32_t *__restrict__ child_nbr) {
+  const int k = blockIdx.y;
+  int64_t r = (int64_t)blockIdx.x * blockDim.x + threadIdx.x;
+  if (r >= n_keep) return;
+  const int32_t j = parent_nbr[(int64_t)k * n_parent + keep_rows[r]];
+  child_nbr[(int64_t)k * n_keep + r] = j >= 0 ? rank_of[j] : -1;
+}
+
+extern "C" int pm_nbr_restrict(const int32_t *parent_nbr, int64_t n_parent, int32_t kvol, const int32_t *keep_rows,
+                               const int32_t *rank_of, int64_t n_keep, int32_t *child_nbr, pm_stream_t stream) {
+  PH_REQUIRE(kvol >= 1 && kvol <= PH_MAX_KVOL, "nbr_restrict: kvol=%d out of range", kvol);
+  PH_REQUIRE(n_keep >= 0 && n_keep <= n_parent && n_parent < 0x7FFFFFFF, "nbr_restrict: %lld kept rows of %lld", (long long)n_keep, (long long)n_parent);
+  if (n_keep == 0) return 0;
+  dim3 grid(nblk(n_keep, 256), (unsigned)kvol);
+  hipLaunchKernelGGL(k_nbr_restrict, grid, dim3(256), 0, ph_stream(stream), parent_nbr, n_parent, keep_rows, rank_of, n_keep, child_nbr);
+  PH_LAUNCH_CHECK();
+  return 0;
+}
diff --git a/pasco_amd/csrc/rows.hip b/pasco_amd/csrc/rows.hip
--- a/pasco_amd/csrc/rows.hip
+++ b/pasco_amd/csrc/rows.hip
@@ -1,4 +1,5 @@
 #include "ph_common.h"
+#include "../../include/pasco_map.h"
 
 static inline unsigned nblk(int64_t n, int t) { return (unsigned)((n + t - 1) / t); }
 
@@ -30,6 +31,61 @@
     hipLaunchKernelGGL(k_gather_rows<float>, dim3(nblk(n_out * c, 256)), dim3(256), 0, st,
                        (const float *)src, c, rows, n_out, (float *)dst);
   }
+  PH_LAUNCH_CHECK();
+  return 0;
+}
+
+struct GatherMulti {
+  const void *src[PM_MAX_GATHER];
+  void *dst[PM_MAX_GATHER];
+  int64_t n_pad[PM_MAX_GATHER];
+  int32_t c[PM_MAX_GATHER];
+  int32_t vec4[PM_MAX_GATHER];
+};
+
+template <typename T>
+__device__ __forceinline__ void gather_multi_one(const T *__restrict__ src, int c, const int32_t *__restrict__ rows, int64_t n_out,
+                                                 int64_t n_pad, T *__restrict__ dst) {
+  const int64_t stride = (int64_t)gridDim.x * blockDim.x;
+  for (int64_t t = (int64_t)blockIdx.x * blockDim.x + threadIdx.x; t < n_pad * c; t += stride) {
+    int64_t j = t / c;
+    int ch = (int)(t - j * c);
+    int r = j < n_out ? rows[j] : -1;
+    T v;
+    memset(&v, 0, sizeof(T));
+    if (r >= 0) v = src[(int64_t)r * c + ch];
+    dst[t] = v;
+  }
+}
+
+__global__ void __launch_bounds__(256) k_gather_rows_multi(GatherMulti g, const int32_t *__restrict__ rows, int64_t n_out) {
+  const int t = blockIdx.y;
+  if (g.vec4[t]) gather_multi_one<float4>((const float4 *)g.src[t], g.c[t], rows, n_out, g.n_pad[t], (float4 *)g.dst[t]);
+  else gather_multi_one<float>((const float *)g.src[t], g.c[t], rows, n_out, g.n_pad[t], (float *)g.dst[t]);
+}
+
+extern "C" int pm_gather_rows_multi(const void *const *h_srcs, const int32_t *h_widths, int32_t count, const int32_t *rows,
+                                    int64_t n_out, void *const *h_dsts, const int64_t *h_n_pad, pm_stream_t stream) {
+  PH_REQUIRE(count >= 1 && count <= PM_MAX_GATHER, "gather_rows_multi: %d tensors, 1 .. %d served", count, PM_MAX_GATHER);
+  PH_REQUIRE(n_out >= 0 && h_srcs && h_widths && h_dsts, "gather_rows_multi: bad arguments");
+  GatherMulti g;
+  memset(&g, 0, sizeof(g));
+  int64_t most = 0;
+  for (int t = 0; t < count; ++t) {
+    const int c = h_widths[t];
+    const int64_t n_pad = h_n_pad ? h_n_pad[t] : n_out;
+    PH_REQUIRE(c > 0, "gather_rows_multi: tensor %d has width %d", t, c);
+    PH_REQUIRE(n_pad >= n_out, "gather_rows_multi: tensor %d: %lld padded rows < %lld rows", t, (long long)n_pad, (long long)n_out);
+    PH_REQUIRE(n_pad == 0 || (h_dsts[t] && (n_out == 0 || h_srcs[t])), "gather_rows_multi: tensor %d has a null pointer", t);
+    g.vec4[t] = c % 4 == 0 && (((uintptr_t)h_srcs[t] | (uintptr_t)h_dsts[t]) & 15) == 0;
+    g.c[t] = g.vec4[t] ? c / 4 : c;
+    g.src[t] = h_srcs[t];
+    g.dst[t] = h_dsts[t];
+    g.n_pad[t] = n_pad;
+    if (n_pad * g.c[t] > most) most = n_pad * g.c[t];
+  }
+  if (most == 0) return 0;
+  hipLaunchKernelGGL(k_gather_rows_multi, dim3(nblk(most, 256), (unsigned)count), dim3(256), 0, ph_stream(stream), g, rows, n_out);
   PH_LAUNCH_CHECK();
   return 0;
 }
diff --git a/pasco_amd/graph/decoder.py b/pasco_amd/graph/decoder.py
--- a/pasco_amd/graph/decoder.py
+++ b/pasco_amd/graph/decoder.py
@@ -289,11 +289,12 @@
                 logits = sem_logits_at_scales[scale][i]
                 slot1, n1_ = infer_ids.index(i), n_rows[(i, scale)]
                 dst = sem_F[slot1, :n1_]
-                be.gather_rows(logits.F.contiguous(), rows, out=dst)
-                if n1_ < sem_F.shape[1]:
-                    sem_F[slot1, n1_:].zero_()
+                xi = fused.gathered_split(x, rows, out_key, also=([logits.F.contiguous()], [sem_F[slot1]]))
+                if xi is None:
+                    be.gather_rows_multi([logits.F.contiguous()], rows, [sem_F[slot1]])
                 sem_logits_pruneds.append(ME.SparseTensor(dst, coordinate_map_key=out_key, coordinate_manager=mgr))
-            xi = fused.gathered_split(x, rows, out_key)
+            else:
+                xi = fused.gathered_split(x, rows, out_key)
             if xi is None:
                 xi = ME.SparseTensor(be.gather_rows(x.F.contiguous(), rows), coordinate_map_key=out_key, coordinate_manager=mgr)
             vf = self.voxel_feats[f"scale{scale}_infer{i}"]
@@ -330,9 +331,9 @@
             mgr = x.coordinate_manager
             out_key, rows = mgr.prune(x.coordinate_map_key, keep)
             be = mgr.backend()
-            x = ME.SparseTensor(be.gather_rows(x.F, rows), coordinate_map_key=out_key, coordinate_manager=mgr)
-            sem_logits = [ME.SparseTensor(be.gather_rows(l.F, rows), coordinate_map_key=out_key,
-                                          coordinate_manager=mgr) for l in sem_logits]
+            got = be.gather_rows_multi([x.F.contiguous()] + [l.F.contiguous() for l in sem_logits], rows)
+            x = ME.SparseTensor(got[0], coordinate_map_key=out_key, coordinate_manager=mgr)
+            sem_logits = [ME.SparseTensor(f, coordinate_map_key=out_key, coordinate_manager=mgr) for f in got[1:]]
             xs[scale] = x
             sem_logits_at_scales[scale] = sem_logits
         ret = {"sem_logits_at_scales": sem_logits_at_scales}
diff --git a/pasco_amd/graph/fused.py b/pasco_amd/graph/fused.py
--- a/pasco_amd/graph/fused.py
+++ b/pasco_amd/graph/fused.py
@@ -159,7 +159,7 @@
     return hit
 
 
-def gathered_split(x: SparseTensor, rows: torch.Tensor, out_key):
+def gathered_split(x: SparseTensor, rows: torch.Tensor, out_key, also=None):
     mgr = x.coordinate_manager
     be = mgr.backend()
     c = x.F.shape[1]
@@ -167,7 +167,11 @@
         return None
     op = split_input(x, be, None, None, ACT_NONE, 0.01)
     n, cpad = op.shape[0], op.shape[1] * 32
-    got = be.gather_rows(op.view(torch.float32).view(n, cpad), rows)
+    src = op.view(torch.float32).view(n, cpad)
+    if also is not None:
+        got = be.gather_rows_multi([src] + list(also[0]), rows, [None] + list(also[1]))[0]
+    else:
+        got = be.gather_rows(src, rows)
     return SplitRows(got.view(torch.float16).view(got.shape[0], cpad // 32, 2, 32), c, out_key, mgr)
 
 
diff --git a/pasco_amd/me/backend.py b/pasco_amd/me/backend.py
--- a/pasco_amd/me/backend.py
+++ b/pasco_amd/me/backend.py
@@ -116,6 +116,22 @@
 
 EXPORTED_SYMBOLS = tuple(_SIGNATURES.keys())
 
+PM_ABI_VERSION = 1
+PM_MAX_JOBS, PM_MAX_GATHER = 16, 8
+PM_MAX_ROWS = 2048 * 2048
+
+
+class PruneJob(C.Structure):
+    _fields_ = [("mask", _vp), ("n", _i64), ("parent_coords", _vp), ("keep_rows", _vp), ("rank_of", _vp), ("out_coords", _vp)]
+
+
+_PM_SIGNATURES = {
+    "prune_workspace_bytes": ([_i64], _i64),
+    "prune_rows": ([C.POINTER(PruneJob), _i32, _vp, _vp, _i64, _vp], C.c_int),
+    "nbr_restrict": ([_vp, _i64, _i32, _vp, _vp, _i64, _vp, _vp], C.c_int),
+    "gather_rows_multi": ([C.POINTER(_vp), C.POINTER(_i32), _i32, _vp, _i64, C.POINTER(_vp), C.POINTER(_i64), _vp], C.c_int),
+}
+
 
 def _ptr(t: Optional[torch.Tensor]) -> Optional[int]:
     if t is None:
@@ -160,6 +176,18 @@
                 f.argtypes = argtypes
                 f.restype = C.c_int
                 self.fn[name] = f
+        self.pm: Dict[str, object] = {}
+        self.pm_calls: Dict[str, int] = {}
+        pmv = getattr(self.lib, "pm_abi_version", None) if prefix == "ph_" else None
+        if pmv is not None:
+            if int(pmv()) != PM_ABI_VERSION:
+                raise RuntimeError(f"{path}: pm ABI {int(pmv())}, this binding expects {PM_ABI_VERSION} - rebuild the library "
+                                   "(python -m pasco_amd.build --force)")
+            self.lib.pm_last_error.restype = C.c_char_p
+            for name, (argtypes, restype) in _PM_SIGNATURES.items():
+                f = getattr(self.lib, "pm_" + name)
+                f.argtypes, f.restype = argtypes, restype
+                self.pm[name] = f
         self._ws: Dict[torch.device, torch.Tensor] = {}
         self._status_ptrs: Dict[tuple, int] = {}
         self._tls = threading.local()
@@ -190,6 +218,14 @@
         if rc != 0:
             msg = self.fn["last_error"]()
             raise RuntimeError(f"{self.prefix}{name} failed ({rc}): {msg.decode() if msg else ''}")
+
+    def _check_pm(self, rc: int, name: str):
+        if rc != 0:
+            msg = self.lib.pm_last_error()
+            raise RuntimeError(f"pm_{name} failed ({rc}): {msg.decode() if msg else ''}")
+
+    def _count(self, name: str):
+        self.pm_calls[name] = self.pm_calls.get(name, 0) + 1
 
     def stream(self, device: torch.device) -> Optional[int]:
         if device.type == "cuda":
@@ -253,6 +289,7 @@
 
     def map_insert_launch(self, coords: torch.Tensor, dedup: bool = True, n_uniq: Optional[torch.Tensor] = None):
         self._chk(coords, torch.int32, "coords")
+        self._count("map_insert")
         n = coords.shape[0]
         dev = coords.device
         cap = self.table_capacity(n)
@@ -745,6 +782,91 @@
             keeps.append(keep)
         return [k[:c] for k, c in zip(keeps, cnts.tolist())]
 
+    def prune_rows_many(self, jobs, derived: Optional[bool] = None) -> list:
+        jobs = [((m.view(torch.uint8) if m.dtype == torch.bool else m), c) for m, c in jobs]
+        if not jobs:
+            return []
+        if derived is None:
+            derived = True
+        if not (derived and "prune_rows" in self.pm and all(m.shape[0] <= PM_MAX_ROWS for m, _ in jobs)):
+            keeps = self.mask_compact_many([m for m, _ in jobs])
+            return [(keep, None, self.gather_rows(c, keep)) for keep, (_, c) in zip(keeps, jobs)]
+        dev = jobs[0][0].device
+        st = self.stream(dev)
+        cnts = torch.empty(len(jobs), dtype=torch.int32, device=dev)
+        wsb = self.pm["prune_workspace_bytes"]
+        bufs = []
+        for lo in range(0, len(jobs), PM_MAX_JOBS):
+            part = jobs[lo:lo + PM_MAX_JOBS]
+            arr = (PruneJob * len(part))()
+            need = 0
+            for j, (mask, coords) in enumerate(part):
+                self._chk(mask, torch.uint8, "mask")
+                self._chk(coords, torch.int32, "coords")
+                n = mask.shape[0]
+                if coords.shape != (n, 4):
+                    raise ValueError(f"prune_rows: mask has {n} rows, coordinates are {tuple(coords.shape)}")
+                m4 = (max(n, 1) + 3) // 4 * 4
+                rows2 = torch.empty(2 * m4, dtype=torch.int32, device=dev)
+                out = torch.empty((max(n, 1), 4), dtype=torch.int32, device=dev)
+                arr[j] = PruneJob(_ptr(mask), n, _ptr(coords), _ptr(rows2), rows2[m4:].data_ptr(), _ptr(out))
+                bufs.append((rows2[:n], rows2[m4:m4 + n], out))
+                need += int(wsb(n))
+            key = ("pmws",) + self._stream_key(dev)
+            ws = self._ws.get(key)
+            if ws is None or ws.numel() < need:
+                ws = torch.empty(max(need, 1 << 16), dtype=torch.uint8, device=dev)
+                self._ws[key] = ws
+            self._count("prune_rows")
+            rc = self.pm["prune_rows"](arr, len(part), cnts[lo:].data_ptr(), _ptr(ws), ws.numel(), st)
+            self._check_pm(rc, "prune_rows")
+        return [(keep[:c], rank_of, out[:c]) for (keep, rank_of, out), c in zip(bufs, cnts.tolist())]
+
+    def nbr_restrict(self, parent_nbr: torch.Tensor, keep_rows: torch.Tensor, rank_of: torch.Tensor) -> torch.Tensor:
+        self._chk(parent_nbr, torch.int32, "parent_nbr")
+        self._chk(keep_rows, torch.int32, "keep_rows")
+        self._chk(rank_of, torch.int32, "rank_of")
+        kvol, n_parent = parent_nbr.shape
+        if rank_of.shape[0] != n_parent:
+            raise ValueError(f"nbr_restrict: rank_of has {rank_of.shape[0]} rows, the parent table {n_parent}")
+        n_keep = keep_rows.shape[0]
+        child = torch.empty((kvol, n_keep), dtype=torch.int32, device=parent_nbr.device)
+        self._count("nbr_restrict")
+        rc = self.pm["nbr_restrict"](_ptr(parent_nbr), n_parent, kvol, _ptr(keep_rows), _ptr(rank_of), n_keep, _ptr(child),
+                                     self.stream(parent_nbr.device))
+        self._check_pm(rc, "nbr_restrict")
+        return child
+
+    def gather_rows_multi(self, srcs, rows: torch.Tensor, outs=None) -> list:
+        self._chk(rows, torch.int32, "rows")
+        m = rows.shape[0]
+        srcs = list(srcs)
+        outs = [None] * len(srcs) if outs is None else list(outs)
+        for t, src in enumerate(srcs):
+            if src.element_size() != 4 or not src.is_contiguous() or src.dim() != 2:
+                raise ValueError("gather_rows_multi: contiguous [N, C] tensors of a 4-byte element type")
+            if outs[t] is None:
+                outs[t] = torch.empty((m, src.shape[1]), dtype=src.dtype, device=src.device)
+            o = outs[t]
+            if o.dim() != 2 or o.shape[0] < m or o.shape[1] != src.shape[1] or o.dtype != src.dtype or not o.is_contiguous() \
+                    or o.device != src.device:
+                raise ValueError("gather_rows_multi: out must be contiguous [P >= M, C] of src's dtype")
+        if "gather_rows_multi" not in self.pm:
+            for src, o in zip(srcs, outs):
+                self.gather_rows(src, rows, out=o[:m])
+                if o.shape[0] > m:
+                    o[m:].zero_()
+            return [o[:m] for o in outs]
+        for lo in range(0, len(srcs), PM_MAX_GATHER):
+            ps, po = srcs[lo:lo + PM_MAX_GATHER], outs[lo:lo + PM_MAX_GATHER]
+            k = len(ps)
+            self._count("gather_rows_multi")
+            rc = self.pm["gather_rows_multi"]((_vp * k)(*[_ptr(x) for x in ps]), (_i32 * k)(*[x.shape[1] for x in ps]), k,
+                                              _ptr(rows), m, (_vp * k)(*[_ptr(x) for x in po]),
+                                              (_i64 * k)(*[x.shape[0] for x in po]), self.stream(rows.device))
+            self._check_pm(rc, "gather_rows_multi")
+        return [o[:m] for o in outs]
+
     def gather_rows(self, src: torch.Tensor, rows: torch.Tensor, out: Optional[torch.Tensor] = None) -> torch.Tensor:
         if src.element_size() != 4:
             raise TypeError("gather_rows serves 4-byte element types")
diff --git a/pasco_amd/me/core.py b/pasco_amd/me/core.py
--- a/pasco_amd/me/core.py
+++ b/pasco_amd/me/core.py
@@ -48,7 +48,7 @@
 
 
 class _CoordMap:
-    __slots__ = ("coords", "_tkeys", "_tvals", "n", "_build")
+    __slots__ = ("coords", "_tkeys", "_tvals", "n", "_build", "parent")
 
     def __init__(self, coords, tkeys, tvals, build=None):
         self.coords = coords
@@ -56,6 +56,7 @@
         self._tvals = tvals
         self._build = build
         self.n = coords.shape[0]
+        self.parent = None
 
     def _table(self):
         if self._tkeys is None:
@@ -228,8 +229,34 @@
         m = self._maps[in_key]
         be = self.backend()
         children = be.coords_expand(m.coords, ts_out[0])
-        keep = be.mask_compact(keep_of(children).contiguous())
-        return self.insert_unique(be.gather_rows(children, keep), ts_out)
+        (_, _, coords), = be.prune_rows_many([(keep_of(children).contiguous(), children)])
+        return self.insert_unique(coords, ts_out)
+
+    def _insert_pruned(self, coords, in_key: CoordinateMapKey, keep, rank_of) -> CoordinateMapKey:
+        out_key = self.insert_unique(coords, in_key.tensor_stride)
+        if rank_of is not None:
+            self._maps[out_key].parent = (in_key, keep, rank_of)
+        return out_key
+
+    def _restricted_table(self, key: CoordinateMapKey, ks, dl):
+        be = self.backend()
+        if not be.pm.get("nbr_restrict"):
+            return None
+        chain, k = [], key
+        while True:
+            m = self._maps.get(k)
+            if m is None or m.parent is None or m.parent[0] not in self._maps:
+                return None
+            chain.append(k)
+            k = m.parent[0]
+            nbr = self._kmap_cache.get((k, k, ks, dl, False))
+            if nbr is not None:
+                break
+        for k in reversed(chain):
+            _, keep, rank_of = self._maps[k].parent
+            nbr = be.nbr_restrict(nbr, keep, rank_of)
+            self._kmap_cache[(k, k, ks, dl, False)] = nbr
+        return nbr
 
     def prune(self, in_key: CoordinateMapKey, mask: torch.Tensor):
         m = self._maps[in_key]
@@ -238,9 +265,8 @@
         if last is not None and last[0] == in_key and last[1] is mask and last[2] == tensor_version(mask):
             return last[3], last[4]
         be = self.backend()
-        keep = be.mask_compact(mask.contiguous())
-        coords = be.gather_rows(m.coords, keep)
-        out_key = self.insert_unique(coords, in_key.tensor_stride)
+        (keep, rank_of, coords), = be.prune_rows_many([(mask.contiguous(), m.coords)])
+        out_key = self._insert_pruned(coords, in_key, keep, rank_of)
         self.__dict__["_last_prune"] = (in_key, mask, tensor_version(mask), out_key, keep)
         return out_key, keep
 
@@ -254,11 +280,9 @@
             if k not in uniq:
                 uniq[k] = len(order)
                 order.append((in_key, mask))
-        keeps = be.mask_compact_many([mask.contiguous() for _, mask in order])
-        done = []
-        for (in_key, mask), keep in zip(order, keeps):
-            coords = be.gather_rows(self._maps[in_key].coords, keep)
-            done.append((self.insert_unique(coords, in_key.tensor_stride), keep))
+        parts = be.prune_rows_many([(mask.contiguous(), self._maps[in_key].coords) for in_key, mask in order])
+        done = [(self._insert_pruned(coords, in_key, keep, rank_of), keep)
+                for (in_key, _), (keep, rank_of, coords) in zip(order, parts)]
         return [done[uniq[(in_key, id(mask), tensor_version(mask))]] for in_key, mask in jobs]
 
     def union(self, key_a: CoordinateMapKey, key_b: CoordinateMapKey):
@@ -284,7 +308,9 @@
             k = len(offs)
             same = in_key == out_key and not transposed and k % 2 == 1 and k > 1 and all(
                 tuple(offs[i]) == tuple(-v for v in offs[k - 1 - i]) for i in range(k // 2 + 1))
-            nbr = self.backend().nbr_build(mo.coords, mi.tkeys, mi.tvals, offs, same_map=same)
+            nbr = self._restricted_table(in_key, ks, dl) if same else None
+            if nbr is None:
+                nbr = self.backend().nbr_build(mo.coords, mi.tkeys, mi.tvals, offs, same_map=same)
             self._kmap_cache[ck] = nbr
         return nbr
 
```

Measured after the change: 48.20. -1.2%, worse.
